# facebook/winterfell

Measured on NVIDIA H100. Metric: prover_ms, lower is better.
Workload: dtype u64

## Files before the change

### winterfell_b200/csrc/capi.cu

```cuda
#include <cuda_runtime.h>
#include <stdarg.h>
#include <stdio.h>

#include <algorithm>
#include <map>
#include <set>
#include <string>
#include <thread>
#include <utility>
#include <vector>

#include "internal.hpp"
#include "alg_hash.cuh"

void wf_mark(wf_ctx* ctx, const char* name) {
    if (!ctx->profiling) return;
    cudaEvent_t e;
    if (cudaEventCreate(&e) != cudaSuccess) return;
    cudaEventRecord(e, ctx->st);
    ctx->marks.push_back({name, e});
}
int wf_fail(wf_ctx* ctx, int code, const char* fmt, ...) {
    char buf[512];
    va_list ap;
    va_start(ap, fmt);
    vsnprintf(buf, sizeof(buf), fmt, ap);
    va_end(ap);
    if (ctx) ctx->err = buf;
    return code;
}
static inline void wf_use_device(wf_ctx* ctx) {
    int cur = -1;
    if (cudaGetDevice(&cur) != cudaSuccess || cur != ctx->device) cudaSetDevice(ctx->device);
}
int wf_dev_alloc(wf_ctx* ctx, size_t bytes, void** out) {
    wf_use_device(ctx);
    bytes = (bytes + 255) & ~(size_t)255;
    if (bytes == 0) bytes = 256;
    auto it = ctx->pool.find(bytes);
    if (it != ctx->pool.end()) {
        *out = it->second;
        ctx->pool.erase(it);
        ctx->live[*out] = bytes;
        return WF_OK;
    }
    void* p = nullptr;
    cudaError_t e = cudaMalloc(&p, bytes);
    if (e != cudaSuccess) {
        for (auto& kv : ctx->pool) cudaFree(kv.second);
        ctx->pool.clear();
        e = cudaMalloc(&p, bytes);
        if (e != cudaSuccess) return wf_fail(ctx, WF_ERR_CUDA, "cudaMalloc(%zu): %s", bytes, cudaGetErrorString(e));
    }
    ctx->live[p] = bytes;
    *out = p;
    return WF_OK;
}
void wf_dev_free(wf_ctx* ctx, void* p) {
    if (!p) return;
    auto it = ctx->live.find(p);
    if (it == ctx->live.end()) return;
    ctx->pool.insert({it->second, p});
    ctx->live.erase(it);
}
int wf_mat_alloc(wf_ctx* ctx, size_t rows, u32 cols, wf_mat** out) { return wf_mat_alloc_w(ctx, rows, cols, seg_width_for(cols), out); }
int wf_mat_alloc_w(wf_ctx* ctx, size_t rows, u32 cols, int W, wf_mat** out) {
    wf_mat* m = new wf_mat();
    m->m.rows = rows;
    m->m.cols = cols;
    m->m.W = W;
    m->m.seg_stride = rows * m->m.W;
    void* p;
    int r = wf_dev_alloc(ctx, m->m.words() * 8, &p);
    if (r != WF_OK) { delete m; return r; }
    m->m.base = (u64*)p;
    *out = m;
    return WF_OK;
}

__global__ void pow_table_kernel(u64* out, u64 base, u64 scale, size_t count) {
    size_t i = (size_t)blockIdx.x * blockDim.x + threadIdx.x;
    if (i < count) out[i] = gl_mul(scale, gl_pow(base, i));
}
__global__ void pow_table2_kernel(u64* out, const u64* bases, size_t count, size_t nbases) {
    size_t i = (size_t)blockIdx.x * blockDim.x + threadIdx.x;
    if (i < count * nbases) out[i] = gl_pow(bases[i / count], i % count);
}

int wf_get_twiddles(wf_ctx* ctx, u32 log_n, const u64** out) {
    auto it = ctx->tw.find(log_n);
    if (it != ctx->tw.end()) { *out = it->second; return WF_OK; }
    if (log_n < 1 || log_n > 32) return wf_fail(ctx, WF_ERR_INVALID, "no 2^%u-th root of unity", log_n);
    size_t half = log_n >= 1 ? ((size_t)1 << (log_n - 1)) : 1;
    void* p;
    cudaError_t e = cudaMalloc(&p, std::max(half * 8, (size_t)16));
    if (e != cudaSuccess) return wf_fail(ctx, WF_ERR_CUDA, "cudaMalloc twiddles: %s", cudaGetErrorString(e));
    pow_table_kernel<<<(unsigned)((half + 255) / 256), 256, 0, ctx->st>>>((u64*)p, gl_root_of_unity(log_n), 1, half);
    ctx->launches++;
    CK(cudaGetLastError());
    ctx->tw[log_n] = (u64*)p;
    *out = (u64*)p;
    return WF_OK;
}

static int get_pow_table(wf_ctx* ctx, u32 log_order, u32 log_count, const u64** out) {
    auto key = std::make_pair(log_order, log_count);
    auto it = ctx->pow_tab.find(key);
    if (it != ctx->pow_tab.end()) { *out = it->second; return WF_OK; }
    size_t cnt = (size_t)1 << log_count;
    void* p;
    cudaError_t e = cudaMalloc(&p, std::max(cnt * 8, (size_t)16));
    if (e != cudaSuccess) return wf_fail(ctx, WF_ERR_CUDA, "cudaMalloc power table: %s", cudaGetErrorString(e));
    pow_table_kernel<<<(unsigned)((cnt + 255) / 256), 256, 0, ctx->st>>>((u64*)p, log_order ? gl_root_of_unity(log_order) : 1, 1, cnt);
    ctx->launches++;
    CK(cudaGetLastError());
    ctx->pow_tab[key] = (u64*)p;
    *out = (u64*)p;
    return WF_OK;
}
static int get_round_tw(wf_ctx* ctx, u32 logS, const u64** out) {
    auto it = ctx->round_tw.find(logS);
    if (it != ctx->round_tw.end()) { *out = it->second; return WF_OK; }
    void* p;
    cudaError_t e = cudaMalloc(&p, ntt2_tw_entries((int)logS) * 8);
    if (e != cudaSuccess) return wf_fail(ctx, WF_ERR_CUDA, "cudaMalloc round twiddles: %s", cudaGetErrorString(e));
    CK(ntt2_build_tw((int)logS, (u64*)p, ctx->st));
    ctx->launches++;
    ctx->round_tw[logS] = (u64*)p;
    *out = (u64*)p;
    return WF_OK;
}
static int launch_pass(wf_ctx* ctx, int mode, NttPassParams& p, u32 n_segments, u32 n_batch) {
    wf_use_device(ctx);
    if (p.logS >= NTT2_MIN_LOGS) {
        CKI(get_round_tw(ctx, (u32)p.logS, &p.sub_tw));
        if (p.has_post) {
            p.tw_split = p.logM / 2;
            CKI(get_pow_table(ctx, p.logM, p.tw_split, &p.tw_lo));
            CKI(get_pow_table(ctx, p.logM - p.tw_split, p.logM - p.tw_split, &p.tw_hi));
        }
        p.vec_in = (p.W >= 2 || mode == NTT_STRIDED) ? 1 : 0;
        p.vec_out = (p.W >= 2 || (mode == NTT_STRIDED && !p.y_in_out)) ? 1 : 0;
        CK(ntt2_launch_pass(mode, p, n_segments, n_batch, ctx->st));
    } else {
        CKI(wf_get_twiddles(ctx, std::max((u32)p.logS, 1u), &p.sub_tw));
        if (p.has_post) CKI(wf_get_twiddles(ctx, p.logM, &p.master));
        CK(ntt_launch_pass(mode, p, n_segments, n_batch, ctx->st));
    }
    ctx->launches++;
    return WF_OK;
}

static void split_log(u32 log_n, u32* logR, u32* logC) {
    if (log_n <= NTT_MAX_LOGS) { *logR = 0; *logC = log_n; return; }
    u32 r = (log_n + 1) / 2;
    if (r > NTT_MAX_LOGS) r = NTT_MAX_LOGS;
    *logR = r;
    *logC = log_n - r;
}

static int get_lde_tables(wf_ctx* ctx, u32 log_n, u32 log_b, u32 logR, LdeTables* out) {
    auto key = std::make_pair(log_n | (logR << 8), log_b);
    auto it = ctx->lde_tabs.find(key);
    if (it != ctx->lde_tabs.end()) { *out = it->second; return WF_OK; }
    const u32 logC = log_n - logR;
    size_t b = (size_t)1 << log_b, R = (size_t)1 << logR, C = (size_t)1 << logC;
    u64 g = gl_root_of_unity(log_n + log_b);
    std::vector<u64> bases(b);
    size_t cnt = logR == 0 ? C : R;
    for (size_t k = 0; k < b; k++) {
        u64 sk = gl_mul(GL_GENERATOR, gl_pow(g, k));
        bases[k] = logR == 0 ? sk : gl_pow(sk, C);
    }
    LdeTables t{nullptr, nullptr};
    void *p, *pb;
    CK(cudaMalloc(&p, b * cnt * 8));
    CK(cudaMalloc(&pb, b * 8));
    CK(cudaMemcpyAsync(pb, bases.data(), b * 8, cudaMemcpyHostToDevice, ctx->st));
    pow_table2_kernel<<<(unsigned)((b * cnt + 255) / 256), 256, 0, ctx->st>>>((u64*)p, (u64*)pb, cnt, b);
    ctx->launches++;
    CK(cudaGetLastError());
    CK(cudaStreamSynchronize(ctx->st));
    cudaFree(pb);
    t.pre = (u64*)p;
    if (logR != 0) {
        void* q;
        CK(cudaMalloc(&q, C * 8));
        pow_table_kernel<<<(unsigned)((C + 255) / 256), 256, 0, ctx->st>>>((u64*)q, GL_GENERATOR, 1, C);
        ctx->launches++;
        CK(cudaGetLastError());
        t.pow7 = (u64*)q;
    }
    ctx->lde_tabs[key] = t;
    *out = t;
    return WF_OK;
}

static void pass_defaults(NttPassParams& p, const SegMatrix& in, const SegMatrix& out) {
    memset(&p, 0, sizeof(p));
    p.in = in.base;
    p.out = out.base;
    p.in_seg_stride = in.seg_stride;
    p.out_seg_stride = out.seg_stride;
    p.W = in.W;
    p.out_W = (u32)out.W;
    p.out_row_mul = 1;
    p.cconst = 1;
}
static int split3(wf_ctx* ctx, u32 log_n, u32* lr, u32* lc, u32* lr2, u32* lc2) {
    *lr = (log_n + 2) / 3;
    *lc = log_n - *lr;
    split_log(*lc, lr2, lc2);
    if (*lr2 == 0 || *lc2 > NTT_MAX_LOGS || *lr > NTT_MAX_LOGS)
        return wf_fail(ctx, WF_ERR_UNSUPPORTED, "transform of 2^%u points exceeds the three-pass limit", log_n);
    return WF_OK;
}

static int run_ntt(wf_ctx* ctx, const SegMatrix& in, SegMatrix& out, const SegMatrix* tmp, u32 log_n, int inverse) {
    u32 logR, logC;
    split_log(log_n, &logR, &logC);
    u64 inv_n = gl_inv(((u64)1 << log_n) % GL_P);
    NttPassParams p;
    if (logC > NTT_MAX_LOGS) {
        if (!tmp) return wf_fail(ctx, WF_ERR_STATE, "run_ntt: scratch matrix required");
        u32 lr, lc, lr2, lc2;
        CKI(split3(ctx, log_n, &lr, &lc, &lr2, &lc2));
        pass_defaults(p, in, *tmp);
        p.logS = (int)lr; p.logR = lr; p.logC = lc; p.inverse = inverse;
        p.has_post = 1; p.logM = log_n; p.a_mul = 1; p.b_mul = 0; p.cconst = inverse ? inv_n : 1;
        CKI(launch_pass(ctx, NTT_STRIDED, p, in.nseg(), 1));
        pass_defaults(p, *tmp, *tmp);
        p.in_batch_stride = p.out_batch_stride = ((size_t)1 << lc) * in.W;
        p.logS = (int)lr2; p.logR = lr2; p.logC = lc2; p.inverse = inverse;
        p.has_post = 1; p.logM = lc; p.a_mul = 1; p.b_mul = 0;
        CKI(launch_pass(ctx, NTT_STRIDED, p, in.nseg(), 1u << lr));
        pass_defaults(p, *tmp, out);
        p.in_batch_stride = ((size_t)1 << lc) * in.W;
        p.logS = (int)lc2; p.logR = lr2; p.logC = lc2; p.inverse = inverse;
        p.out_row_mul = 1u << lr; p.out_row_add = 1;
        CKI(launch_pass(ctx, NTT_CONTIG, p, in.nseg(), 1u << lr));
        return WF_OK;
    }
    if (logR == 0) {
        pass_defaults(p, in, out);
        p.logS = (int)logC; p.logR = 0; p.logC = logC; p.inverse = inverse;
        if (inverse) p.cconst = inv_n;
        return launch_pass(ctx, NTT_CONTIG, p, in.nseg(), 1);
    }
    if (!tmp) return wf_fail(ctx, WF_ERR_STATE, "run_ntt: scratch matrix required");
    pass_defaults(p, in, *tmp);
    p.logS = (int)logR; p.logR = logR; p.logC = logC; p.inverse = inverse;
    p.has_post = 1; p.logM = log_n; p.a_mul = 1; p.b_mul = 0; p.cconst = inverse ? inv_n : 1;
    CKI(launch_pass(ctx, NTT_STRIDED, p, in.nseg(), 1));
    pass_defaults(p, *tmp, out);
    p.logS = (int)logC; p.logR = logR; p.logC = logC; p.inverse = inverse;
    return launch_pass(ctx, NTT_CONTIG, p, in.nseg(), 1);
}

static int run_lde(wf_ctx* ctx, const SegMatrix& polys, SegMatrix& out, u32 log_n, u32 log_b, u32 out_col0 = 0, u32 k0 = 0, u32 k1 = 0,
                   u32 row_mul = 0, u32 row_add = 1) {
    u32 logR, logC;
    split_log(log_n, &logR, &logC);
    u32 b = 1u << log_b;
    if (k1 == 0) k1 = b;
    if (row_mul == 0) { row_mul = b; row_add = 1; }
    LdeTables tabs;
    NttPassParams p;
    if (logC > NTT_MAX_LOGS) {
        u32 lr, lc, lr2, lc2;
        CKI(split3(ctx, log_n, &lr, &lc, &lr2, &lc2));
        CKI(get_lde_tables(ctx, log_n, log_b, lr, &tabs));
        SegMatrix y = polys;
        void* yp;
        CKI(wf_dev_alloc(ctx, polys.words() * 8, &yp));
        y.base = (u64*)yp;
        int rc = WF_OK;
        for (u32 k = k0; k < k1 && rc == WF_OK; k++) {
            pass_defaults(p, polys, y);
            p.logS = (int)lr; p.logR = lr; p.logC = lc;
            p.pre_tab = tabs.pre + ((size_t)k << lr); p.pre_batch_stride = 0;
            p.has_post = 1; p.logM = log_n + log_b; p.a_mul = b; p.b_mul = 1; p.batch0 = k;
            p.ctab = tabs.pow7;
            rc = launch_pass(ctx, NTT_STRIDED, p, polys.nseg(), 1);
            if (rc != WF_OK) break;
            pass_defaults(p, y, y);
            p.in_batch_stride = p.out_batch_stride = ((size_t)1 << lc) * polys.W;
            p.logS = (int)lr2; p.logR = lr2; p.logC = lc2;
            p.has_post = 1; p.logM = lc; p.a_mul = 1; p.b_mul = 0;
            rc = launch_pass(ctx, NTT_STRIDED, p, polys.nseg(), 1u << lr);
            if (rc != WF_OK) break;
            pass_defaults(p, y, out);
            p.in_batch_stride = ((size_t)1 << lc) * polys.W;
            p.logS = (int)lc2; p.logR = lr2; p.logC = lc2;
            p.out_row_mul = row_mul << lr; p.out_row_add = row_mul; p.out_col0 = out_col0;
            p.out = out.base + (size_t)(k - k0) * row_add * out.W;
            rc = launch_pass(ctx, NTT_CONTIG, p, polys.nseg(), 1u << lr);
        }
        wf_dev_free(ctx, yp);
        return rc;
    }
    CKI(get_lde_tables(ctx, log_n, log_b, logR, &tabs));
    if (logR == 0) {
        pass_defaults(p, polys, out);
        p.logS = (int)logC; p.logR = 0; p.logC = logC;
        p.pre_tab = tabs.pre + ((size_t)k0 << log_n); p.pre_batch_stride = (size_t)1 << log_n;
        p.out_row_mul = row_mul; p.out_row_add = row_add; p.out_col0 = out_col0;
        return launch_pass(ctx, NTT_CONTIG, p, polys.nseg(), k1 - k0);
    }
    pass_defaults(p, polys, out);
    p.logS = (int)logR; p.logR = logR; p.logC = logC;
    p.pre_tab = tabs.pre + ((size_t)k0 << logR); p.pre_batch_stride = (size_t)1 << logR;
    p.has_post = 1; p.logM = log_n + log_b; p.a_mul = b; p.b_mul = 1; p.batch0 = k0;
    p.ctab = tabs.pow7;
    p.y_in_out = 1; p.out_row_mul = row_mul; p.out_row_add = row_add; p.out_col0 = out_col0;
    CKI(launch_pass(ctx, NTT_STRIDED, p, polys.nseg(), k1 - k0));
    pass_defaults(p, polys, out);
    p.in = out.base;
    p.in_seg_stride = out.seg_stride;
    p.logS = (int)logC; p.logR = logR; p.logC = logC;
    p.y_in_out = 1; p.out_row_mul = row_mul; p.out_row_add = row_add; p.out_col0 = out_col0;
    return launch_pass(ctx, NTT_CONTIG, p, polys.nseg(), k1 - k0);
}

template <int K>
__device__ __forceinline__ void field_shift_store(u64 a, u64* out, size_t n, size_t i, int slot) { out[(4 + slot) * n + i] = gl_mul_2exp<K>(a); }
__global__ void field_ops_kernel(const u64* a, const u64* b, size_t n, u64* out) {
    size_t i = (size_t)blockIdx.x * blockDim.x + threadIdx.x;
    if (i >= n) return;
    u64 x = a[i], y = b[i];
    out[i] = gl_mul(x, y);
    out[n + i] = gl_add(x, y);
    out[2 * n + i] = gl_sub(x, y);
    out[3 * n + i] = x ? gl_inv(x) : 0;
    u64 s = x, d = y;
    gl_butterfly(s, d);
    if (s != out[n + i] || d != out[2 * n + i]) out[n + i] = ~0ULL;
    field_shift_store<1>(x, out, n, i, 0);   field_shift_store<3>(x, out, n, i, 1);   field_shift_store<6>(x, out, n, i, 2);
    field_shift_store<12>(x, out, n, i, 3);  field_shift_store<24>(x, out, n, i, 4);  field_shift_store<31>(x, out, n, i, 5);
    field_shift_store<32>(x, out, n, i, 6);  field_shift_store<33>(x, out, n, i, 7);  field_shift_store<48>(x, out, n, i, 8);
    field_shift_store<63>(x, out, n, i, 9);  field_shift_store<64>(x, out, n, i, 10); field_shift_store<65>(x, out, n, i, 11);
    field_shift_store<72>(x, out, n, i, 12); field_shift_store<80>(x, out, n, i, 13); field_shift_store<84>(x, out, n, i, 14);
    field_shift_store<90>(x, out, n, i, 15); field_shift_store<95>(x, out, n, i, 16); field_shift_store<96>(x, out, n, i, 17);
}
template <int... K>
__device__ __forceinline__ void field_shifts_all(u64 x, u64* out, size_t n, size_t i, std::integer_sequence<int, K...>) {
    ((out[(size_t)K * n + i] = gl_mul_2exp<K>(x)), ...);
}
__global__ void field_shifts_kernel(const u64* a, size_t n, u64* out) {
    size_t i = (size_t)blockIdx.x * blockDim.x + threadIdx.x;
    if (i >= n) return;
    field_shifts_all(a[i], out, n, i, std::make_integer_sequence<int, 97>{});
}

__global__ void rescue_weak_kernel(const u64* a, const u64* b, size_t n, u64* out) {
    size_t i = (size_t)blockIdx.x * blockDim.x + threadIdx.x;
    if (i >= n) return;
    out[i] = gl_mul_weak(a[i], b[i]);
    out[n + i] = gl_sqr_weak(a[i]);
    out[2 * n + i] = rp64_exp7(a[i]);
}
template <int G>
__global__ void rescue_inv7_kernel(const u64* a, size_t n, u64* out) {
    size_t t = (size_t)blockIdx.x * blockDim.x + threadIdx.x;
    if (t >= n / G) return;
    u64 s[G];
#pragma unroll
    for (int e = 0; e < G; e++) s[e] = a[t * G + e];
    rp64_inv7_group<G>(s);
#pragma unroll
    for (int e = 0; e < G; e++) out[t * G + e] = s[e];
}
__global__ void rescue_mds_kernel(const u64* a, size_t n, u64* out12, u64* out8) {
    size_t t = (size_t)blockIdx.x * blockDim.x + threadIdx.x;
    if (t < n / 12) {
        u64 s[12];
        for (int e = 0; e < 12; e++) s[e] = a[t * 12 + e];
        rp64_mds(s);
        for (int e = 0; e < 12; e++) out12[t * 12 + e] = s[e];
    }
    if (t < n / 8) {
        u64 s[8];
        for (int e = 0; e < 8; e++) s[e] = a[t * 8 + e];
        rpj_mds(s);
        for (int e = 0; e < 8; e++) out8[t * 8 + e] = s[e];
    }
}
template <int HASH, int W>
__global__ void rescue_permute_kernel(const u64* in, const u64* values, size_t n, u64* out) {
    size_t i = (size_t)blockIdx.x * blockDim.x + threadIdx.x;
    if (i >= n) return;
    u64 s[W];
#pragma unroll
    for (int e = 0; e < W; e++) s[e] = in[i * W + e];
    u64 m[4], mi[4];
    alg_merge<HASH>(s, m);
    alg_merge_with_int<HASH>(s, values[i], mi);
    if (HASH == WF_HASH_RP64_256) rp64_permute(s);
    else rpj_permute(s);
#pragma unroll
    for (int e = 0; e < W; e++) out[i * W + e] = s[e];
#pragma unroll
    for (int e = 0; e < 4; e++) { out[n * W + i * 4 + e] = m[e]; out[n * (W + 4) + i * 4 + e] = mi[e]; }
}

template <int D>
__global__ void ext_ops_kernel(const u64* a, const u64* b, size_t n, u64* out) {
    size_t i = (size_t)blockIdx.x * blockDim.x + threadIdx.x;
    if (i >= n) return;
    GlExt<D> x, y;
#pragma unroll
    for (int q = 0; q < D; q++) { x.v[q] = a[i * D + q]; y.v[q] = b[i * D + q]; }
    const GlExt<D> r[6] = {ext_mul(x, y), ext_inv(x), ext_frobenius(x), ext_mul_base(x, y.v[0]), ext_add(x, y), ext_sub(x, y)};
#pragma unroll
    for (int k = 0; k < 6; k++)
#pragma unroll
        for (int q = 0; q < D; q++) out[((size_t)k * n + i) * D + q] = r[k].v[q];
}

__global__ void acc_ops_kernel(const u64* x, const u64* y, u32 k, size_t n, u64* out) {
    size_t i = (size_t)blockIdx.x * blockDim.x + threadIdx.x;
    if (i >= n) return;
    GlAcc a = acc_zero();
    for (u32 j = 0; j < k; j++) acc_mad(a, x[i * k + j], y[i * k + j]);
    u64* o = out + i * 6;
    o[0] = a.w0; o[1] = a.w1; o[2] = a.w2; o[3] = a.w3; o[4] = a.w4;
    o[5] = acc_reduce(a);
}

template <int K>
static u64 m2e(u64 x) { return gl_mul_2exp<K>(x); }

extern "C" {

const char* wf_version(void) { return "winterfell_b200 0.1 (sm_90a)"; }

int wf_ctx_create(wf_ctx** out, int device, void* stream) {
    if (!out) return WF_ERR_INVALID;
    *out = nullptr;
    int n = 0;
    cudaError_t e = cudaGetDeviceCount(&n);
    if (e != cudaSuccess || n == 0) return WF_ERR_CUDA;
    if (device < 0 || device >= n) return WF_ERR_INVALID;
    if (cudaSetDevice(device) != cudaSuccess) return WF_ERR_CUDA;
    wf_ctx* ctx = new wf_ctx();
    ctx->device = device;
    ctx->st = (cudaStream_t)stream;
    ctx->launches = 0;
    ctx->pinned = nullptr;
    ctx->pinned_bytes = 0;
    ctx->profiling = false;
    *out = ctx;
    return WF_OK;
}
void wf_ctx_destroy(wf_ctx* ctx) {
    if (!ctx) return;
    cudaSetDevice(ctx->device);
    cudaStreamSynchronize(ctx->st);
    for (auto& kv : ctx->pool) cudaFree(kv.second);
    for (auto& kv : ctx->live) cudaFree(kv.first);
    for (auto& kv : ctx->tw) cudaFree(kv.second);
    for (auto& kv : ctx->lde_tabs) { cudaFree(kv.second.pre); if (kv.second.pow7) cudaFree(kv.second.pow7); }
    if (ctx->pinned) cudaFreeHost(ctx->pinned);
    for (auto& kv : ctx->ipc_opened) cudaIpcCloseMemHandle(kv.second);
    for (auto& kv : ctx->jit_cache) if (kv.second.first) cudaLibraryUnload((cudaLibrary_t)kv.second.first);
    for (int i = 0; i < 4; i++) if (ctx->push_st[i]) { cudaStreamSynchronize(ctx->push_st[i]); cudaStreamDestroy(ctx->push_st[i]); }
    for (int i = 0; i < 16; i++) if (ctx->push_ev[i]) cudaEventDestroy(ctx->push_ev[i]);
    if (ctx->copy_st) {
        cudaStreamSynchronize(ctx->copy_st);
        for (int i = 0; i < 2; i++) { cudaEventDestroy(ctx->ev_up[i]); cudaEventDestroy(ctx->ev_used[i]); }
        cudaEventDestroy(ctx->ev_start);
        cudaStreamDestroy(ctx->copy_st);
    }
    delete ctx;
}
int wf_ctx_set_profiling(wf_ctx* ctx, int on) {
    if (!ctx) return WF_ERR_INVALID;
    ctx->profiling = on != 0;
    for (auto& m : ctx->marks) cudaEventDestroy(m.second);
    ctx->marks.clear();
    return WF_OK;
}
int wf_ctx_stage_times(wf_ctx* ctx, char* names, size_t names_cap, float* ms, size_t* count) {
    if (!ctx || !names || !ms || !count) return WF_ERR_INVALID;
    CK(cudaStreamSynchronize(ctx->st));
    size_t n = ctx->marks.size() > 0 ? ctx->marks.size() - 1 : 0, used = 0;
    if (n > *count) n = *count;
    names[0] = 0;
    for (size_t i = 0; i < n; i++) {
        CK(cudaEventElapsedTime(&ms[i], ctx->marks[i].second, ctx->marks[i + 1].second));
        const std::string& nm = ctx->marks[i + 1].first;
        if (used + nm.size() + 2 < names_cap) { memcpy(names + used, nm.c_str(), nm.size()); used += nm.size(); names[used++] = ','; names[used] = 0; }
    }
    *count = n;
    for (auto& m : ctx->marks) cudaEventDestroy(m.second);
    ctx->marks.clear();
    return WF_OK;
}
const char* wf_last_error(const wf_ctx* ctx) { return ctx ? ctx->err.c_str() : "no context (is a CUDA device present?)"; }
int wf_ctx_sync(wf_ctx* ctx) { wf_use_device(ctx); CK(cudaStreamSynchronize(ctx->st)); return WF_OK; }
uint64_t wf_ctx_launch_count(const wf_ctx* ctx) { return ctx->launches; }
int wf_ctx_mem_stats(const wf_ctx* ctx, uint64_t* live_buffers, uint64_t* live_bytes, uint64_t* pooled_bytes) {
    if (!ctx) return WF_ERR_INVALID;
    uint64_t lb = 0, pb = 0;
    for (auto& kv : ctx->live) lb += kv.second;
    for (auto& kv : ctx->pool) pb += kv.first;
    if (live_buffers) *live_buffers = ctx->live.size();
    if (live_bytes) *live_bytes = lb;
    if (pooled_bytes) *pooled_bytes = pb;
    return WF_OK;
}
// ... 261 lines not shown
            ctx->launches++;
            SegMatrix pv = polys->m;
            pv.base = polys->m.base + (size_t)k * polys->m.seg_stride;
            pv.cols = cw;
            SegMatrix tv = trv;
            tv.base = (u64*)tmp;
            CKI(run_ntt(ctx, trv, pv, &tv, log_n, 1));
            SegMatrix ov = lde->m;
            ov.base = lde->m.base + (size_t)(c0 / Wout) * lde->m.seg_stride;
            ov.cols = cw;
            CKI(extend(pv, ov, c0 % Wout, k + 1 == nchunks));
        }
        return WF_OK;
    };
    int rc = body();
    if (rc != WF_OK) {
        cudaStreamSynchronize(ctx->copy_st);
        release(true);
        return rc;
    }
    release(false);
    *polys_out = polys;
    *lde_out = lde;
    return WF_OK;
}

int wf_mat_interpolate_with_offset(wf_ctx* ctx, const wf_mat* evals, uint64_t domain_offset, wf_mat** polys) {
    if (domain_offset == 0 || domain_offset >= GL_P) return wf_fail(ctx, WF_ERR_INVALID, "bad domain offset");
    wf_mat* p;
    CKI(mat_transform(ctx, evals, 1, &p));
    CK(layout_scale_rows_by_powers(p->m, gl_inv(domain_offset), ctx->st));
    ctx->launches++;
    *polys = p;
    return WF_OK;
}

static int tree_alloc(wf_ctx* ctx, int hash_id, size_t nleaves, wf_tree** out) {
    if (nleaves < 2 || (nleaves & (nleaves - 1))) return wf_fail(ctx, WF_ERR_INVALID, "number of leaves must be a power of two >= 2");
    wf_tree* t = new wf_tree();
    t->hash_id = hash_id;
    t->nleaves = nleaves;
    void *a, *b;
    int r = wf_dev_alloc(ctx, nleaves * 32, &a);
    if (r != WF_OK) { delete t; return r; }
    r = wf_dev_alloc(ctx, nleaves * 32, &b);
    if (r != WF_OK) { wf_dev_free(ctx, a); delete t; return r; }
    t->leaves = (u64*)a;
    t->nodes = (u64*)b;
    *out = t;
    return WF_OK;
}
static u32 merkle_launches(size_t nleaves) {
    u32 l = 0;
    size_t m = nleaves / 2;
    while (m > (1u << 13)) { l++; m >>= 1; }
    for (;;) {
        l++;
        if (m <= 256) break;
        m = (m >> 8) >> 1;
        if (m == 0) break;
    }
    return l;
}
int wf_commit_rows_partitioned(wf_ctx* ctx, int hash_id, const wf_mat* m, uint32_t partition_size, wf_tree** out) {
    if (!ctx || !m || !out) return wf_fail(ctx, WF_ERR_INVALID, "bad arguments");
    if (!WF_HASH_IS_KNOWN(hash_id)) return wf_fail(ctx, WF_ERR_UNSUPPORTED, "unknown hash %d", hash_id);
    if (partition_size != 0 && partition_size != m->m.cols && (m->m.cols + partition_size - 1) / partition_size > 16)
        return wf_fail(ctx, WF_ERR_INVALID, "more than 16 partitions");
    wf_tree* t;
    CKI(tree_alloc(ctx, hash_id, m->m.rows, &t));
    CK(commit_hash_rows(hash_id, m->m, t->leaves, ctx->st, partition_size));
    CK(commit_merkle_nodes(hash_id, t->leaves, t->nleaves, t->nodes, ctx->st));
    ctx->launches += 1 + merkle_launches(t->nleaves);
    *out = t;
    return WF_OK;
}
int wf_commit_rows(wf_ctx* ctx, int hash_id, const wf_mat* m, wf_tree** out) {
    if (!ctx || !m || !out) return wf_fail(ctx, WF_ERR_INVALID, "bad arguments");
    if (!WF_HASH_IS_KNOWN(hash_id)) return wf_fail(ctx, WF_ERR_UNSUPPORTED, "unknown hash %d", hash_id);
    wf_tree* t;
    CKI(tree_alloc(ctx, hash_id, m->m.rows, &t));
    CK(commit_hash_rows(hash_id, m->m, t->leaves, ctx->st));
    CK(commit_merkle_nodes(hash_id, t->leaves, t->nleaves, t->nodes, ctx->st));
    ctx->launches += 1 + merkle_launches(t->nleaves);
    *out = t;
    return WF_OK;
}
int wf_tree_from_leaves(wf_ctx* ctx, int hash_id, const uint8_t* leaves, size_t nleaves, int on_device, wf_tree** out) {
    if (!ctx || !leaves || !out) return wf_fail(ctx, WF_ERR_INVALID, "bad arguments");
    wf_tree* t;
    CKI(tree_alloc(ctx, hash_id, nleaves, &t));
    CK(cudaMemcpyAsync(t->leaves, leaves, nleaves * 32, on_device ? cudaMemcpyDeviceToDevice : cudaMemcpyHostToDevice, ctx->st));
    CK(commit_merkle_nodes(hash_id, t->leaves, nleaves, t->nodes, ctx->st));
    ctx->launches += merkle_launches(nleaves);
    if (!on_device) CK(cudaStreamSynchronize(ctx->st));
    *out = t;
    return WF_OK;
}
int wf_tree_free(wf_ctx* ctx, wf_tree* t) {
    if (!t) return WF_OK;
    wf_dev_free(ctx, t->leaves);
    wf_dev_free(ctx, t->nodes);
    delete t;
    return WF_OK;
}
size_t wf_tree_num_leaves(const wf_tree* t) { return t->nleaves; }
int wf_tree_root(wf_ctx* ctx, const wf_tree* t, uint8_t root[32]) {
    if (!ctx || !t || !root) return wf_fail(ctx, WF_ERR_INVALID, "bad arguments");
    CK(cudaMemcpyAsync(root, t->nodes + 4, 32, cudaMemcpyDeviceToHost, ctx->st));
    CK(cudaStreamSynchronize(ctx->st));
    return WF_OK;
}
int wf_tree_to_host(wf_ctx* ctx, const wf_tree* t, uint8_t* leaves, uint8_t* nodes) {
    if (!ctx || !t) return wf_fail(ctx, WF_ERR_INVALID, "bad arguments");
    if (leaves) CK(cudaMemcpyAsync(leaves, t->leaves, t->nleaves * 32, cudaMemcpyDeviceToHost, ctx->st));
    if (nodes) CK(cudaMemcpyAsync(nodes, t->nodes, t->nleaves * 32, cudaMemcpyDeviceToHost, ctx->st));
    CK(cudaStreamSynchronize(ctx->st));
    return WF_OK;
}

}

int wf_open_plan(wf_ctx* ctx, size_t n, const uint64_t* positions, size_t k, OpenPlan& pl) {
    pl.depth = log2_ceil(n);
    if (k == 0) return wf_fail(ctx, WF_ERR_INVALID, "no positions");
    std::map<size_t, size_t> index_map;
    for (size_t i = 0; i < k; i++) {
        if (positions[i] >= n) return wf_fail(ctx, WF_ERR_INVALID, "leaf index out of bounds");
        index_map[positions[i]] = i;
    }
    if (index_map.size() != k) return wf_fail(ctx, WF_ERR_INVALID, "duplicate leaf index");
    std::set<size_t> norm;
    for (size_t i = 0; i < k; i++) norm.insert(positions[i] & ~(size_t)1);
    pl.want.clear();
    pl.vec_slots.clear();
    pl.leaf_slot.assign(k, 0);
    std::vector<size_t> next;
    for (size_t index : norm) {
        std::vector<size_t> slots;
        for (size_t i = index; i < index + 2; i++) {
            auto it = index_map.find(i);
            pl.want.push_back(n + i);
            if (it != index_map.end()) pl.leaf_slot[it->second] = pl.want.size() - 1;
            else slots.push_back(pl.want.size() - 1);
        }
        pl.vec_slots.push_back(slots);
        next.push_back((index + n) >> 1);
    }
    for (u32 lvl = 1; lvl < pl.depth; lvl++) {
        std::vector<size_t> idx = next;
        next.clear();
        size_t i = 0;
        while (i < idx.size()) {
            size_t sib = idx[i] ^ 1;
            if (i + 1 < idx.size() && idx[i + 1] == sib) i += 1;
            else { pl.want.push_back(sib); pl.vec_slots[i].push_back(pl.want.size() - 1); }
            next.push_back(sib >> 1);
            i += 1;
        }
    }
    return WF_OK;
}
void wf_open_finish(const OpenPlan& pl, const uint8_t* got, uint8_t* leaves_out, ByteVec& proof) {
    if (leaves_out)
        for (size_t i = 0; i < pl.leaf_slot.size(); i++) memcpy(leaves_out + i * 32, got + pl.leaf_slot[i] * 32, 32);
    proof.u8_((u8)pl.depth);
    proof.usize(pl.vec_slots.size());
    for (auto& v : pl.vec_slots) {
        proof.usize(v.size());
        for (size_t s : v) proof.bytes(got + s * 32, pl.digest_bytes);
    }
}

int pinned_reserve(wf_ctx* ctx, size_t bytes) {
    if (ctx->pinned_bytes >= bytes) return WF_OK;
    if (ctx->pinned) cudaFreeHost(ctx->pinned);
    ctx->pinned = nullptr;
    ctx->pinned_bytes = 0;
    bytes = std::max(bytes * 2, (size_t)1 << 20);
    CK(cudaMallocHost(&ctx->pinned, bytes));
    ctx->pinned_bytes = bytes;
    return WF_OK;
}

size_t GatherBatch::add_rows(const SegMatrix& m, const std::vector<u64>& pos) {
    rows.push_back({m, pos, 0, 0});
    return rows.size() - 1;
}
int GatherBatch::add_opening(wf_ctx* ctx, const wf_tree* t, const std::vector<u64>& pos, size_t* id) {
    digs.emplace_back();
    digs.back().t = t;
    CKI(wf_open_plan(ctx, t->nleaves, pos.data(), pos.size(), digs.back().plan));
    digs.back().plan.digest_bytes = WF_DIGEST_BYTES(t->hash_id);
    digs.back().idx = digs.back().plan.want;
    *id = digs.size() - 1;
    return WF_OK;
}
int GatherBatch::add_opening_sharded(wf_ctx* ctx, const wf_tree* t, size_t n_global, int world, int rank, const std::vector<u64>& pos,
                                     size_t* id, std::vector<std::pair<size_t, u64>>* top_slots) {
    digs.emplace_back();
    DigJob& j = digs.back();
    j.t = t;
    CKI(wf_open_plan(ctx, n_global, pos.data(), pos.size(), j.plan));
    if (t) j.plan.digest_bytes = WF_DIGEST_BYTES(t->hash_id);
    const size_t n_local = n_global / (size_t)world;
    const u32 log_w = log2_ceil((size_t)world);
    j.idx.assign(j.plan.want.size(), ~(u64)0);
    for (size_t s = 0; s < j.plan.want.size(); s++) {
        const u64 e = j.plan.want[s];
        if (e >= n_global) {
            const u64 leaf = e - n_global;
            if ((int)(leaf / n_local) == rank) j.idx[s] = n_local + leaf % n_local;
        } else if (e < (u64)world) {
            if (top_slots) top_slots->push_back({s, e});
        } else {
            u32 depth = 63 - (u32)__builtin_clzll(e);
            const u32 rel = depth - log_w;
            const u64 owner = (e >> rel) - (u64)world;
            if ((int)owner == rank) j.idx[s] = ((u64)1 << rel) | (e & (((u64)1 << rel) - 1));
        }
    }
    *id = digs.size() - 1;
    return WF_OK;
}
int GatherBatch::run(wf_ctx* ctx) {
    wf_use_device(ctx);
    size_t idx_words = 0, out_words = 0;
    for (auto& j : rows) { j.idx_off = idx_words; j.out_off = out_words; idx_words += j.pos.size(); out_words += j.pos.size() * j.m.cols; }
    for (auto& j : digs) { j.idx_off = idx_words; j.out_off = out_words; idx_words += j.plan.want.size(); out_words += j.plan.want.size() * 4; }
    if (idx_words == 0) return WF_OK;
    CKI(pinned_reserve(ctx, (idx_words + out_words) * 8));
    u64* h_idx = (u64*)ctx->pinned;
    u64* h_out = h_idx + idx_words;
    for (auto& j : rows) memcpy(h_idx + j.idx_off, j.pos.data(), j.pos.size() * 8);
    for (auto& j : digs) memcpy(h_idx + j.idx_off, j.idx.data(), j.idx.size() * 8);
    void *d_idx, *d_out;
    CKI(wf_dev_alloc(ctx, idx_words * 8, &d_idx));
    CKI(wf_dev_alloc(ctx, out_words * 8, &d_out));
    CK(cudaMemcpyAsync(d_idx, h_idx, idx_words * 8, cudaMemcpyHostToDevice, ctx->st));
    for (auto& j : rows) {
        CK(layout_gather_rows(j.m, (const u64*)d_idx + j.idx_off, j.pos.size(), (u64*)d_out + j.out_off, 0, ctx->st));
        ctx->launches++;
    }
    for (auto& j : digs) {
        CK(layout_gather_digests(j.t->nodes, j.t->leaves, j.t->nleaves, (const u64*)d_idx + j.idx_off, j.plan.want.size(),
                                 (u64*)d_out + j.out_off, ctx->st));
        ctx->launches++;
    }
    if (comm && comm->world > 1 && comm->all_reduce_sum(comm->user, d_out, out_words) != 0)
        return wf_fail(ctx, WF_ERR_STATE, "all_reduce_sum callback failed");
    CK(cudaMemcpyAsync(h_out, d_out, out_words * 8, cudaMemcpyDeviceToHost, ctx->st));
    CK(cudaStreamSynchronize(ctx->st));
    wf_dev_free(ctx, d_idx);
    wf_dev_free(ctx, d_out);
    result = h_out;
    return WF_OK;
}

int wf_tree_open_many_bytes(wf_ctx* ctx, const wf_tree* t, const uint64_t* positions, size_t k, uint8_t* leaves_out,
                            ByteVec& proof) {
    GatherBatch gb;
    size_t id;
    CKI(gb.add_opening(ctx, t, std::vector<u64>(positions, positions + k), &id));
    CKI(gb.run(ctx));
    wf_open_finish(gb.digs[id].plan, gb.digest_result(id), leaves_out, proof);
    return WF_OK;
}
extern "C" {
int wf_tree_open_many(wf_ctx* ctx, const wf_tree* t, const uint64_t* positions, size_t k, uint8_t* leaves_out,
                      uint8_t* proof, size_t* proof_len) {
    if (!ctx || !t || !positions || !leaves_out || !proof || !proof_len) return wf_fail(ctx, WF_ERR_INVALID, "bad arguments");
    ByteVec bv;
    CKI(wf_tree_open_many_bytes(ctx, t, positions, k, leaves_out, bv));
    if (bv.v.size() > *proof_len) return wf_fail(ctx, WF_ERR_INVALID, "proof buffer too small (%zu needed)", bv.v.size());
    memcpy(proof, bv.v.data(), bv.v.size());
    *proof_len = bv.v.size();
    return WF_OK;
}

}
int wf_fri_layer_tree(wf_ctx* ctx, int hash_id, const u64* vals, size_t len, int d, int ld, int nf, wf_tree** out) {
    const size_t m = len / (size_t)nf;
    wf_tree* t;
    CKI(tree_alloc(ctx, hash_id, m, &t));
    CK(fri_hash_layer(hash_id, vals, len, d, ld, nf, t->leaves, ctx->st));
    CK(commit_merkle_nodes(hash_id, t->leaves, m, t->nodes, ctx->st));
    ctx->launches += 1 + merkle_launches(m);
    *out = t;
    return WF_OK;
}
extern "C" {
int wf_fri_free(wf_ctx* ctx, wf_fri* f) {
    if (!f) return WF_OK;
    for (auto& l : f->layers) { wf_dev_free(ctx, l.evals); wf_tree_free(ctx, l.tree); }
    delete f;
    return WF_OK;
}

}
struct FriBuild {
    wf_ctx* ctx;
    wf_fri* f;
    wf_tree* t = nullptr;
    DevScratch tmp;
    FriBuild(wf_ctx* c, wf_fri* fr) : ctx(c), f(fr), tmp(c) {}
    ~FriBuild() { if (t) wf_tree_free(ctx, t); if (f) wf_fri_free(ctx, f); }
};
extern "C" {
int wf_fri_build_layers(wf_ctx* ctx, int hash_id, const wf_mat* evals, int d, uint32_t folding, uint32_t rem_max_deg,
                        uint32_t blowup, wf_fri_commit_fn commit, wf_fri_draw_fn draw_alpha, void* user, wf_fri** out) {
    if (!ctx || !evals || !commit || !draw_alpha || !out) return wf_fail(ctx, WF_ERR_INVALID, "bad arguments");
    if (d < 1 || d > 3 || (int)evals->m.cols != d) return wf_fail(ctx, WF_ERR_INVALID, "evaluations must have ext_degree base columns");
    if (folding != 2 && folding != 4 && folding != 8 && folding != 16) return wf_fail(ctx, WF_ERR_UNSUPPORTED, "folding factor %u", folding);
    size_t len = evals->m.rows;
    u32 logL;
    if (log2_exact(len, &logL)) return wf_fail(ctx, WF_ERR_INVALID, "domain size must be a power of two");
    wf_fri* f = new wf_fri();
    FriBuild g(ctx, f);
    f->hash_id = hash_id; f->d = d; f->folding = folding; f->blowup = blowup;
    f->ld = evals->m.W;
    const int ld = f->ld;
    void* cur;
    CKI(g.tmp.alloc(len * ld * 8, &cur));
    CK(cudaMemcpyAsync(cur, evals->m.base, len * ld * 8, cudaMemcpyDeviceToDevice, ctx->st));
    size_t max_rem = (size_t)(rem_max_deg + 1) * blowup;
    while (len > max_rem) {
        size_t m = len / folding;
        wf_tree* t;
        CKI(tree_alloc(ctx, hash_id, m, &t));
        g.t = t;
        CK(fri_hash_layer(hash_id, (u64*)cur, len, d, ld, (int)folding, t->leaves, ctx->st));
        CK(commit_merkle_nodes(hash_id, t->leaves, m, t->nodes, ctx->st));
        ctx->launches += 1 + merkle_launches(m);
        uint8_t root[32];
        CK(cudaMemcpyAsync(root, t->nodes + 4, 32, cudaMemcpyDeviceToHost, ctx->st));
        CK(cudaStreamSynchronize(ctx->st));
        commit(user, root);
        u64 alpha[3] = {0, 0, 0};
        draw_alpha(user, alpha);
        const u64* master;
        CKI(wf_get_twiddles(ctx, log2_ceil(len), &master));
        void* nxt;
        CKI(g.tmp.alloc(m * ld * 8, &nxt));
        if (ld > d) CK(cudaMemsetAsync(nxt, 0, m * ld * 8, ctx->st));
        CK(fri_fold_layer((u64*)cur, len, d, ld, (int)folding, alpha, master, (u64*)nxt, ld, ctx->st));
        ctx->launches++;
        f->layers.push_back(FriLayer{(u64*)g.tmp.keep(cur), len, t});
        g.t = nullptr;
        cur = nxt;
        len = m;
    }
    std::vector<u64> raw(len * ld), v(len * d);
    CK(cudaMemcpyAsync(raw.data(), cur, len * ld * 8, cudaMemcpyDeviceToHost, ctx->st));
    CK(cudaStreamSynchronize(ctx->st));
    g.tmp.free(cur);
    for (size_t i = 0; i < len; i++)
        for (int c = 0; c < d; c++) v[i * d + c] = raw[i * ld + c];
    wf_host_dft(v, len, d, true, GL_GENERATOR);
    size_t rsize = len / blowup;
    f->remainder.resize(rsize * d);
    for (size_t i = 0; i < rsize; i++)
        for (int c = 0; c < d; c++) f->remainder[i * d + c] = v[(rsize - 1 - i) * d + c];
    Digest rc = hh_hash_elements(hash_id, f->remainder.data(), f->remainder.size());
    commit(user, rc.b);
    g.f = nullptr;
    *out = f;
    return WF_OK;
}

}
int wf_fri_build_layers_coin(wf_ctx* ctx, int hash_id, const wf_mat* evals, int d, uint32_t folding, uint32_t rem_max_deg,
                             uint32_t blowup, PublicCoin& coin, std::vector<Digest>& commitments, wf_fri** out) {
    if (!ctx || !evals || !out) return wf_fail(ctx, WF_ERR_INVALID, "bad arguments");
    if (d < 1 || d > 3 || (int)evals->m.cols != d) return wf_fail(ctx, WF_ERR_INVALID, "evaluations must have ext_degree base columns");
    if (folding != 2 && folding != 4 && folding != 8 && folding != 16) return wf_fail(ctx, WF_ERR_UNSUPPORTED, "folding factor %u", folding);
    size_t len = evals->m.rows;
    u32 logL;
    if (log2_exact(len, &logL)) return wf_fail(ctx, WF_ERR_INVALID, "domain size must be a power of two");
    wf_fri* f = new wf_fri();
    FriBuild g(ctx, f);
    f->hash_id = hash_id; f->d = d; f->folding = folding; f->blowup = blowup;
    f->ld = evals->m.W;
    const int ld = f->ld;
    const size_t max_rem = (size_t)(rem_max_deg + 1) * blowup;
    size_t nlayers = 0;
    for (size_t l = len; l > max_rem; l /= folding) nlayers++;
    void *cur, *dstate, *dalpha, *dlog;
    CKI(g.tmp.alloc(len * ld * 8, &cur));
    CK(cudaMemcpyAsync(cur, evals->m.base, len * ld * 8, cudaMemcpyDeviceToDevice, ctx->st));
    CKI(g.tmp.alloc(8 * 8, &dstate));
    CKI(g.tmp.alloc(8 * 8, &dalpha));
    CKI(g.tmp.alloc(std::max<size_t>(nlayers, 1) * 8 * 8, &dlog));
    u64 seed_words[4];
    memcpy(seed_words, coin.seed.b, 32);
    CK(cudaMemcpyAsync(dstate, seed_words, 32, cudaMemcpyHostToDevice, ctx->st));
    size_t layer = 0;
    while (len > max_rem) {
        size_t m = len / folding;
        wf_tree* t;
        CKI(tree_alloc(ctx, hash_id, m, &t));
        g.t = t;
        CK(fri_hash_layer(hash_id, (u64*)cur, len, d, ld, (int)folding, t->leaves, ctx->st));
        CK(commit_merkle_nodes(hash_id, t->leaves, m, t->nodes, ctx->st));
        CK(fri_coin_step(hash_id, (u64*)dstate, t->nodes + 4, d, (u64*)dalpha, (u64*)dlog + 8 * layer, ctx->st));
        ctx->launches += 2 + merkle_launches(m);
        const u64* master;
        CKI(wf_get_twiddles(ctx, log2_ceil(len), &master));
        void* nxt;
        CKI(g.tmp.alloc(m * ld * 8, &nxt));
        if (ld > d) CK(cudaMemsetAsync(nxt, 0, m * ld * 8, ctx->st));
        CK(fri_fold_layer((u64*)cur, len, d, ld, (int)folding, nullptr, master, (u64*)nxt, ld, ctx->st, (const u64*)dalpha));
        ctx->launches++;
        f->layers.push_back(FriLayer{(u64*)g.tmp.keep(cur), len, t});
        g.t = nullptr;
        cur = nxt;
        len = m;
        layer++;
    }
    std::vector<u64> raw(len * ld), v(len * d), log(std::max<size_t>(nlayers, 1) * 8);
    CK(cudaMemcpyAsync(raw.data(), cur, len * ld * 8, cudaMemcpyDeviceToHost, ctx->st));
    if (nlayers) CK(cudaMemcpyAsync(log.data(), dlog, nlayers * 8 * 8, cudaMemcpyDeviceToHost, ctx->st));
    CK(cudaStreamSynchronize(ctx->st));
    g.tmp.free(cur);
    g.tmp.free(dstate); g.tmp.free(dalpha); g.tmp.free(dlog);
    for (size_t l = 0; l < nlayers; l++) {
        Digest root;
        memcpy(root.b, &log[8 * l], 32);
        commitments.push_back(root);
        coin.reseed(root);
        u64 alpha[3] = {0, 0, 0};
        bool ok = coin.draw(d, alpha) && log[8 * l + 7] == 1;
        for (int k = 0; k < d; k++) ok = ok && alpha[k] == log[8 * l + 4 + k];
        if (!ok) return wf_fail(ctx, WF_ERR_STATE, "device and host FRI transcripts diverged at layer %zu", l);
    }
    for (size_t i = 0; i < len; i++)
        for (int c = 0; c < d; c++) v[i * d + c] = raw[i * ld + c];
    wf_host_dft(v, len, d, true, GL_GENERATOR);
    size_t rsize = len / blowup;
    f->remainder.resize(rsize * d);
    for (size_t i = 0; i < rsize; i++)
        for (int c = 0; c < d; c++) f->remainder[i * d + c] = v[(rsize - 1 - i) * d + c];
    Digest rc = hh_hash_elements(hash_id, f->remainder.data(), f->remainder.size());
    commitments.push_back(rc);
    coin.reseed(rc);
    g.f = nullptr;
    *out = f;
    return WF_OK;
}
extern "C" {

struct DefaultChannel {
    PublicCoin coin;
    int d;
    std::vector<Digest> commitments;
};
int wf_fri_build_layers_default_channel(wf_ctx* ctx, int hash_id, const wf_mat* evals, int d, uint32_t folding,
                                        uint32_t rem_max_deg, uint32_t blowup, uint8_t* roots_out, size_t roots_cap,
                                        wf_fri** out) {
    DefaultChannel ch{PublicCoin(hash_id, nullptr, 0), d, {}};
    CKI(wf_fri_build_layers_coin(ctx, hash_id, evals, d, folding, rem_max_deg, blowup, ch.coin, ch.commitments, out));
    if (roots_out) {
        if (roots_cap < ch.commitments.size() * 32) return wf_fail(ctx, WF_ERR_INVALID, "roots buffer too small");
        for (size_t i = 0; i < ch.commitments.size(); i++) memcpy(roots_out + 32 * i, ch.commitments[i].b, 32);
    }
    return WF_OK;
}
uint32_t wf_fri_num_layers(const wf_fri* f) { return (uint32_t)f->layers.size(); }
size_t wf_fri_remainder(const wf_fri* f, uint64_t* coeffs, size_t cap_words) {
    if (coeffs && cap_words >= f->remainder.size()) memcpy(coeffs, f->remainder.data(), f->remainder.size() * 8);
    return f->remainder.size() / f->d;
}

}
int wf_fri_queue_proof(wf_ctx* ctx, wf_fri* f, const std::vector<u64>& positions, GatherBatch& gb, FriProofPlan& plan) {
    std::vector<u64> pos = positions;
    for (auto& L : f->layers) {
        size_t m = L.len / f->folding;
        pos = fold_positions(pos, m);
        std::vector<u64> gpos(pos.size() * f->folding);
        for (size_t i = 0; i < pos.size(); i++)
            for (u32 j = 0; j < f->folding; j++) gpos[i * f->folding + j] = pos[i] + (u64)j * m;
        SegMatrix lm;
        lm.base = L.evals; lm.rows = L.len; lm.cols = (u32)f->d; lm.W = f->ld; lm.seg_stride = L.len * f->ld;
        plan.row_ids.push_back(gb.add_rows(lm, gpos));
        size_t id;
        CKI(gb.add_opening(ctx, L.tree, pos, &id));
        plan.dig_ids.push_back(id);
        plan.nq.push_back(pos.size());
    }
    return WF_OK;
}
void wf_fri_finish_proof(const wf_fri* f, const GatherBatch& gb, const FriProofPlan& plan, ByteVec& bv, const FriProofPlan* before) {
    auto layer = [&](const FriProofPlan& p, size_t l) {
        const size_t nvals = p.nq[l] * f->folding * f->d;
        ByteVec paths;
        wf_open_finish(gb.digs[p.dig_ids[l]].plan, gb.digest_result(p.dig_ids[l]), nullptr, paths);
        bv.u32_((u32)(nvals * 8));
        bv.bytes(gb.row_result(p.row_ids[l]), nvals * 8);
        bv.u32_((u32)paths.v.size());
        bv.bytes(paths.v.data(), paths.v.size());
    };
    const size_t nb = before ? before->nq.size() : 0;
    bv.u8_((u8)(nb + f->layers.size()));
    for (size_t l = 0; l < nb; l++) layer(*before, l);
    for (size_t l = 0; l < f->layers.size(); l++) layer(plan, l);
    bv.u16_((uint16_t)(f->remainder.size() * 8));
    bv.bytes(f->remainder.data(), f->remainder.size() * 8);
    bv.u8_(0);
}
extern "C" {
int wf_fri_build_proof(wf_ctx* ctx, wf_fri* f, const uint64_t* positions, size_t k, uint8_t* out, size_t* len) {
    if (!ctx || !f || !positions || !out || !len) return wf_fail(ctx, WF_ERR_INVALID, "bad arguments");
    GatherBatch gb;
    FriProofPlan plan;
    CKI(wf_fri_queue_proof(ctx, f, std::vector<u64>(positions, positions + k), gb, plan));
    CKI(gb.run(ctx));
    ByteVec bv;
    wf_fri_finish_proof(f, gb, plan, bv);
    if (bv.v.size() > *len) return wf_fail(ctx, WF_ERR_INVALID, "proof buffer too small (%zu needed)", bv.v.size());
    memcpy(out, bv.v.data(), bv.v.size());
    *len = bv.v.size();
    return WF_OK;
}

int wf_ntt_dev(wf_ctx* ctx, uint64_t* d_data, uint32_t log_n, uint32_t cols, int inverse) {
    if (!ctx || !d_data || cols == 0 || log_n < 1) return wf_fail(ctx, WF_ERR_INVALID, "bad arguments");
    wf_mat *m, *o;
    CKI(wf_mat_from_device_columns(ctx, d_data, cols, (size_t)1 << log_n, &m));
    int r = mat_transform(ctx, m, inverse, &o);
    wf_mat_free(ctx, m);
    if (r != WF_OK) return r;
    r = wf_mat_to_columns(ctx, o, d_data, 0, 0);
    wf_mat_free(ctx, o);
    return r;
}
int wf_hash_rows_dev(wf_ctx* ctx, int hash_id, const uint64_t* d_rows, size_t nrows, uint32_t cols, uint8_t* d_digests) {
    if (!ctx || !d_rows || !d_digests || cols == 0) return wf_fail(ctx, WF_ERR_INVALID, "bad arguments");
    wf_mat* m;
    CKI(wf_mat_alloc(ctx, nrows, cols, &m));
    CK(layout_rows_to_seg(d_rows, m->m, ctx->st));
    CK(commit_hash_rows(hash_id, m->m, (u64*)d_digests, ctx->st));
    ctx->launches += 2;
    wf_mat_free(ctx, m);
    return WF_OK;
}
int wf_merkle_dev(wf_ctx* ctx, int hash_id, const uint8_t* d_leaves, size_t nleaves, uint8_t* d_nodes) {
    if (!ctx || !d_leaves || !d_nodes) return wf_fail(ctx, WF_ERR_INVALID, "bad arguments");
    if (nleaves < 2 || (nleaves & (nleaves - 1))) return wf_fail(ctx, WF_ERR_INVALID, "number of leaves must be a power of two >= 2");
    CK(commit_merkle_nodes(hash_id, (const u64*)d_leaves, nleaves, (u64*)d_nodes, ctx->st));
    ctx->launches += merkle_launches(nleaves);
    return WF_OK;
}
int wf_field_ops_dev(wf_ctx* ctx, const uint64_t* d_a, const uint64_t* d_b, size_t n, uint64_t* d_out) {
    if (!ctx || !d_a || !d_b || !d_out || n == 0) return wf_fail(ctx, WF_ERR_INVALID, "bad arguments");
    field_ops_kernel<<<(unsigned)((n + 127) / 128), 128, 0, ctx->st>>>(d_a, d_b, n, d_out);
    ctx->launches++;
    CK(cudaGetLastError());
    return WF_OK;
}
int wf_field_shifts_dev(wf_ctx* ctx, const uint64_t* d_a, size_t n, uint64_t* d_out) {
    if (!ctx || !d_a || !d_out || n == 0) return wf_fail(ctx, WF_ERR_INVALID, "bad arguments");
    field_shifts_kernel<<<(unsigned)((n + 127) / 128), 128, 0, ctx->st>>>(d_a, n, d_out);
    ctx->launches++;
    CK(cudaGetLastError());
    return WF_OK;
}
int wf_rescue_ops_dev(wf_ctx* ctx, const uint64_t* d_a, const uint64_t* d_b, size_t n, uint64_t* d_out) {
    if (!ctx || !d_a || !d_b || !d_out || n == 0 || n % 24) return wf_fail(ctx, WF_ERR_INVALID, "bad arguments");
    const unsigned blocks = (unsigned)((n + 127) / 128);
    rescue_weak_kernel<<<blocks, 128, 0, ctx->st>>>(d_a, d_b, n, d_out);
    rescue_inv7_kernel<1><<<blocks, 128, 0, ctx->st>>>(d_a, n, d_out + 3 * n);
    rescue_inv7_kernel<2><<<blocks, 128, 0, ctx->st>>>(d_a, n, d_out + 4 * n);
    rescue_inv7_kernel<3><<<blocks, 128, 0, ctx->st>>>(d_a, n, d_out + 5 * n);
    rescue_inv7_kernel<4><<<blocks, 128, 0, ctx->st>>>(d_a, n, d_out + 6 * n);
    rescue_inv7_kernel<6><<<blocks, 128, 0, ctx->st>>>(d_a, n, d_out + 7 * n);
    rescue_mds_kernel<<<blocks, 128, 0, ctx->st>>>(d_a, n, d_out + 8 * n, d_out + 9 * n);
    ctx->launches += 7;
    CK(cudaGetLastError());
    return WF_OK;
}
int wf_rescue_permute_dev(wf_ctx* ctx, int hash_id, const uint64_t* d_states, const uint64_t* d_values, size_t n, uint64_t* d_out) {
    if (!ctx || !d_states || !d_values || !d_out || n == 0) return wf_fail(ctx, WF_ERR_INVALID, "bad arguments");
    const unsigned blocks = (unsigned)((n + 127) / 128);
    if (hash_id == WF_HASH_RP64_256) rescue_permute_kernel<WF_HASH_RP64_256, 12><<<blocks, 128, 0, ctx->st>>>(d_states, d_values, n, d_out);
    else if (hash_id == WF_HASH_RPJIVE64_256) rescue_permute_kernel<WF_HASH_RPJIVE64_256, 8><<<blocks, 128, 0, ctx->st>>>(d_states, d_values, n, d_out);
    else return wf_fail(ctx, WF_ERR_INVALID, "hash %d has no Rescue permutation", hash_id);
    ctx->launches++;
    CK(cudaGetLastError());
    return WF_OK;
}
int wf_ext_ops_dev(wf_ctx* ctx, uint32_t ext, const uint64_t* d_a, const uint64_t* d_b, size_t n, uint64_t* d_out) {
    if (!ctx || !d_a || !d_b || !d_out || n == 0 || (ext != 2 && ext != 3)) return wf_fail(ctx, WF_ERR_INVALID, "bad arguments");
    const unsigned blocks = (unsigned)((n + 127) / 128);
    if (ext == 2) ext_ops_kernel<2><<<blocks, 128, 0, ctx->st>>>(d_a, d_b, n, d_out);
    else ext_ops_kernel<3><<<blocks, 128, 0, ctx->st>>>(d_a, d_b, n, d_out);
    ctx->launches++;
    CK(cudaGetLastError());
    return WF_OK;
}
int wf_acc_ops_dev(wf_ctx* ctx, const uint64_t* d_x, const uint64_t* d_y, uint32_t k, size_t n, uint64_t* d_out) {
    if (!ctx || !d_x || !d_y || !d_out || n == 0 || k == 0 || k >= (1u << 31)) return wf_fail(ctx, WF_ERR_INVALID, "bad arguments");
    acc_ops_kernel<<<(unsigned)((n + 127) / 128), 128, 0, ctx->st>>>(d_x, d_y, k, n, d_out);
    ctx->launches++;
    CK(cudaGetLastError());
    return WF_OK;
}
int wf_fri_fold_dev(wf_ctx* ctx, const uint64_t* d_evals, size_t len, int d, uint32_t folding, const uint64_t* alpha,
                    uint64_t* d_next) {
    if (!ctx || !d_evals || !alpha || !d_next || d < 1 || d > 3) return wf_fail(ctx, WF_ERR_INVALID, "bad arguments");
    u32 ll;
    if (log2_exact(len, &ll) || len < folding) return wf_fail(ctx, WF_ERR_INVALID, "bad length");
    const u64* master;
    CKI(wf_get_twiddles(ctx, std::max(ll, 1u), &master));
    CK(fri_fold_layer(d_evals, len, d, d, (int)folding, alpha, master, d_next, d, ctx->st));
    ctx->launches++;
    return WF_OK;
}

int wf_host_hash_elements(int hash_id, const uint64_t* elems, size_t n, uint8_t out[32]) {
    Digest d = hh_hash_elements(hash_id, elems, n);
    memcpy(out, d.b, 32);
    return WF_OK;
}
int wf_host_merge(int hash_id, const uint8_t two[64], uint8_t out[32]) {
    Digest a, b;
    memcpy(a.b, two, 32);
    memcpy(b.b, two + 32, 32);
    Digest d = hh_merge(hash_id, a, b);
    memcpy(out, d.b, 32);
    return WF_OK;
}
int wf_host_merge_with_int(int hash_id, const uint8_t seed[32], uint64_t value, uint8_t out[32]) {
    Digest s;
    memcpy(s.b, seed, 32);
    Digest d = hh_merge_with_int(hash_id, s, value);
    memcpy(out, d.b, 32);
    return WF_OK;
}
uint64_t wf_host_mul(uint64_t a, uint64_t b) { return gl_mul(a, b); }
uint64_t wf_host_mul_2exp(uint64_t x, uint32_t k) {
    switch (k) {
        case 0: return m2e<0>(x); case 3: return m2e<3>(x); case 6: return m2e<6>(x); case 12: return m2e<12>(x);
        case 24: return m2e<24>(x); case 36: return m2e<36>(x); case 48: return m2e<48>(x); case 60: return m2e<60>(x);
        case 63: return m2e<63>(x); case 64: return m2e<64>(x); case 65: return m2e<65>(x); case 72: return m2e<72>(x);
        case 84: return m2e<84>(x); case 95: return m2e<95>(x); case 96: return m2e<96>(x);
        default: return gl_mul(x, gl_pow(2, k));
    }
}
uint64_t wf_host_mont_to_canonical(uint64_t m) { return gl_from_mont(m); }
uint64_t wf_host_canonical_to_mont(uint64_t x) { return gl_to_mont(x); }
size_t wf_host_write_usize(uint64_t value, uint8_t out[9]) {
    ByteVec b;
    b.usize(value);
    memcpy(out, b.v.data(), b.v.size());
    return b.v.size();
}
int wf_host_build_fib_trace(uint32_t k, size_t n, uint64_t* cols, uint64_t* results) {
    if (!cols || !results || k == 0 || n == 0) return WF_ERR_INVALID;
    auto pair = [&](uint32_t j) {
        u64 a = j + 1, b = j + 1;
        u64 *ca = cols + (size_t)(2 * j) * n, *cb = ca + n;
        for (size_t i = 0; i < n; i++) {
            ca[i] = a;
            cb[i] = b;
            a = gl_add_host(a, b);
            b = gl_add_host(b, a);
        }
        results[j] = cb[n - 1];
    };
    const unsigned nt = std::max(1u, std::min(std::min(k, 16u), std::thread::hardware_concurrency()));
    std::vector<std::thread> th;
    for (unsigned t = 0; t < nt; t++) th.emplace_back([&, t]() { for (uint32_t j = t; j < k; j += nt) pair(j); });
    for (auto& x : th) x.join();
    return WF_OK;
}
long wf_host_sharded_opening_plan(size_t n_global, int world, int rank, const uint64_t* positions, size_t k, uint64_t* want,
                                  uint64_t* idx, size_t cap) {
    if (!positions || !want || !idx || world < 1 || (world & (world - 1)) || n_global % (size_t)world) return -1;
    GatherBatch gb;
    size_t id;
    std::vector<std::pair<size_t, u64>> top;
    if (gb.add_opening_sharded(nullptr, nullptr, n_global, world, rank, std::vector<u64>(positions, positions + k), &id, &top) != WF_OK) return -1;
    const auto& j = gb.digs[id];
    if (j.idx.size() > cap) return -1;
    for (size_t i = 0; i < j.idx.size(); i++) { want[i] = j.plan.want[i]; idx[i] = j.idx[i]; }
    for (auto& t : top) idx[t.first] = ~(u64)0 - 1;
    return (long)j.idx.size();
}
int wf_host_coin_draw(int hash_id, const uint64_t* seed_elems, size_t n_seed, const uint8_t* reseed32, int d, size_t count,
                      uint64_t* out) {
    if (d < 1 || d > 3 || !out) return -1;
    PublicCoin coin(hash_id, seed_elems, n_seed);
    if (reseed32) { Digest dg; memcpy(dg.b, reseed32, 32); coin.reseed(dg); }
    for (size_t i = 0; i < count; i++) if (!coin.draw(d, out + i * d)) return -1;
    return 0;
}

}
```

### winterfell_b200/csrc/fri.cu

```cuda
#include "fri.cuh"
#include "internal.hpp"

#include "blake3.cuh"
#include "commit.cuh"
#include "minidft.cuh"
#include "alg_hash.cuh"

__global__ void __launch_bounds__(256) fri_hash_blake3_kernel(const u64* __restrict__ ev, size_t m, int d, int ld, int nf,
                                                              uint4* __restrict__ digests, u32 dw) {
    size_t i = (size_t)blockIdx.x * blockDim.x + threadIdx.x;
    if (i >= m) return;
    const u32 ne = (u32)(nf * d);
    const u32 nblk = (ne + 7) / 8;
    u32 cv[8];
    b3_iv(cv);
    for (u32 b = 0; b < nblk; b++) {
        u32 msg[16];
#pragma unroll
        for (int k = 0; k < 8; k++) {
            u32 e = b * 8 + k;
            u64 v = 0;
            if (e < ne) {
                u32 kk = e / d, comp = e % d;
                v = ev[(i + (size_t)kk * m) * ld + comp];
            }
            msg[2 * k] = (u32)v;
            msg[2 * k + 1] = (u32)(v >> 32);
        }
        u32 bl = min(64u, (ne - b * 8) * 8);
        u32 fl = (b == 0 ? B3_CHUNK_START : 0) | (b == nblk - 1 ? (B3_CHUNK_END | B3_ROOT) : 0);
        b3_compress(cv, msg, 0, bl, fl, b3_runtime_one());
    }
    if (dw == 6) { cv[6] = 0; cv[7] = 0; }
    digests[2 * i] = make_uint4(cv[0], cv[1], cv[2], cv[3]);
    digests[2 * i + 1] = make_uint4(cv[4], cv[5], cv[6], cv[7]);
}

template <int HASH>
__global__ void __launch_bounds__(128) fri_hash_alg_kernel(const u64* __restrict__ ev, size_t m, int d, int ld, int nf,
                                                           u64* __restrict__ digests) {
    size_t i = (size_t)blockIdx.x * blockDim.x + threadIdx.x;
    if (i >= m) return;
    const u32 ne = (u32)(nf * d);
    AlgSponge<HASH> sp;
    sp.init(ne);
    for (u32 e = 0; e < ne; e++) {
        u32 kk = e / d, comp = e % d;
        sp.absorb(ev[(i + (size_t)kk * m) * ld + comp]);
    }
    u64 o[4];
    sp.finish(o);
#pragma unroll
    for (int k = 0; k < 4; k++) digests[i * 4 + k] = o[k];
}

__host__ __device__ constexpr u32 cbrev(u32 v, int bits) {
    u32 r = 0;
    for (int i = 0; i < bits; i++) r |= ((v >> i) & 1u) << (bits - 1 - i);
    return r;
}

template <int D, int LOGNF>
__global__ void __launch_bounds__(256) fri_fold_kernel(const u64* __restrict__ ev, size_t m, int ld, GlExt<D> alpha,
                                                       const u64* __restrict__ d_alpha, const u64* __restrict__ master,
                                                       u32 logL, u64* __restrict__ next, int next_ld, size_t i0) {
    constexpr int NF = 1 << LOGNF;
    size_t i = (size_t)blockIdx.x * blockDim.x + threadIdx.x;
    if (i >= m) return;
    if (d_alpha) {
#pragma unroll
        for (int c = 0; c < D; c++) alpha.v[c] = d_alpha[c];
    }
    u64 x[D][NF];
#pragma unroll
    for (int k = 0; k < NF; k++)
#pragma unroll
        for (int c = 0; c < D; c++) x[c][k] = ev[(i + (size_t)k * m) * ld + c];
#pragma unroll
    for (int c = 0; c < D; c++) mini_dft<LOGNF>(x[c]);
    const u32 L = 1u << logL;
    u32 e = (L - (u32)(i + i0)) & (L - 1);
    u64 winv = (e & (L >> 1)) ? gl_neg(master[e & ((L >> 1) - 1)]) : master[e & ((L >> 1) - 1)];
    u64 xinv = gl_mul(winv, 2635249152773512046ULL);
    GlExt<D> beta = ext_mul_base(alpha, xinv);
    GlExt<D> acc;
    {
        constexpr u32 pos = cbrev(1u, LOGNF);
#pragma unroll
        for (int c = 0; c < D; c++) acc.v[c] = x[c][pos];
    }
#pragma unroll
    for (int j = NF - 2; j >= 0; j--) {
        const u32 pos = cbrev((u32)((NF - j) % NF), LOGNF);
        GlExt<D> cj;
#pragma unroll
        for (int c = 0; c < D; c++) cj.v[c] = x[c][pos];
        acc = ext_add(ext_mul(acc, beta), cj);
    }
    const u64 inv_nf = GL_P - ((GL_P - 1) >> LOGNF);
    acc = ext_mul_base(acc, inv_nf);
#pragma unroll
    for (int c = 0; c < D; c++) next[i * next_ld + c] = acc.v[c];
}

cudaError_t fri_hash_layer(int hash_id, const u64* evals, size_t len, int d, int ld, int nf, u64* digests,
                           cudaStream_t st) {
    size_t m = len / nf;
    if (WF_HASH_IS_BLAKE3(hash_id))
        fri_hash_blake3_kernel<<<(unsigned)((m + 255) / 256), 256, 0, st>>>(evals, m, d, ld, nf,
                                                                            reinterpret_cast<uint4*>(digests), WF_DIGEST_WORDS32(hash_id));
    else if (hash_id == WF_HASH_RP64_256)
        fri_hash_alg_kernel<WF_HASH_RP64_256><<<(unsigned)((m + 127) / 128), 128, 0, st>>>(evals, m, d, ld, nf, digests);
    else if (hash_id == WF_HASH_SHA3_256)
        fri_hash_alg_kernel<WF_HASH_SHA3_256><<<(unsigned)((m + 127) / 128), 128, 0, st>>>(evals, m, d, ld, nf, digests);
    else
        fri_hash_alg_kernel<WF_HASH_RPJIVE64_256><<<(unsigned)((m + 127) / 128), 128, 0, st>>>(evals, m, d, ld, nf, digests);
    return cudaGetLastError();
}

template <int D>
static cudaError_t fold_dispatch(const u64* evals, size_t len, int ld, int nf, const u64* alpha, const u64* d_alpha,
                                 const u64* master, u64* next, int next_ld, cudaStream_t st, size_t i0, u32 logL_global) {
    size_t m = len / nf;
    const u32 logL = logL_global ? logL_global : log2_ceil(len);
    GlExt<D> a;
    for (int c = 0; c < D; c++) a.v[c] = alpha ? alpha[c] : 0;
    unsigned blocks = (unsigned)((m + 255) / 256);
    switch (nf) {
        case 2: fri_fold_kernel<D, 1><<<blocks, 256, 0, st>>>(evals, m, ld, a, d_alpha, master, logL, next, next_ld, i0); break;
        case 4: fri_fold_kernel<D, 2><<<blocks, 256, 0, st>>>(evals, m, ld, a, d_alpha, master, logL, next, next_ld, i0); break;
        case 8: fri_fold_kernel<D, 3><<<blocks, 256, 0, st>>>(evals, m, ld, a, d_alpha, master, logL, next, next_ld, i0); break;
        case 16: fri_fold_kernel<D, 4><<<blocks, 256, 0, st>>>(evals, m, ld, a, d_alpha, master, logL, next, next_ld, i0); break;
        default: return cudaErrorInvalidValue;
    }
    return cudaGetLastError();
}

cudaError_t fri_fold_layer(const u64* evals, size_t len, int d, int ld, int nf, const u64* alpha, const u64* master,
                           u64* next, int next_ld, cudaStream_t st, const u64* d_alpha, size_t i0, u32 logL_global) {
    switch (d) {
        case 1: return fold_dispatch<1>(evals, len, ld, nf, alpha, d_alpha, master, next, next_ld, st, i0, logL_global);
        case 2: return fold_dispatch<2>(evals, len, ld, nf, alpha, d_alpha, master, next, next_ld, st, i0, logL_global);
        case 3: return fold_dispatch<3>(evals, len, ld, nf, alpha, d_alpha, master, next, next_ld, st, i0, logL_global);
        default: return cudaErrorInvalidValue;
    }
}

template <int HASH>
__device__ __forceinline__ void coin_merge(const u64 a[4], const u64 b[4], u64 out[4]) {
    if (WF_HASH_IS_BLAKE3(HASH)) {
        u32 wa[8], wb[8], cv[8];
#pragma unroll
        for (int i = 0; i < 4; i++) { wa[2 * i] = (u32)a[i]; wa[2 * i + 1] = (u32)(a[i] >> 32); wb[2 * i] = (u32)b[i]; wb[2 * i + 1] = (u32)(b[i] >> 32); }
        b3_merge_words<WF_DIGEST_WORDS32(HASH)>(wa, wb, cv);
#pragma unroll
        for (int i = 0; i < 4; i++) out[i] = (u64)cv[2 * i] | ((u64)cv[2 * i + 1] << 32);
    } else {
        u64 in[8];
#pragma unroll
        for (int i = 0; i < 4; i++) { in[i] = a[i]; in[4 + i] = b[i]; }
        alg_merge<HASH>(in, out);
    }
}
template <int HASH>
__device__ __forceinline__ void coin_merge_with_int(const u64 seed[4], u64 value, u64 out[4]) {
    if (WF_HASH_IS_BLAKE3(HASH)) {
        u32 ws[8], cv[8];
#pragma unroll
        for (int i = 0; i < 4; i++) { ws[2 * i] = (u32)seed[i]; ws[2 * i + 1] = (u32)(seed[i] >> 32); }
        b3_merge_with_int_words<WF_DIGEST_WORDS32(HASH)>(ws, value, cv);
#pragma unroll
        for (int i = 0; i < 4; i++) out[i] = (u64)cv[2 * i] | ((u64)cv[2 * i + 1] << 32);
    } else {
        alg_merge_with_int<HASH>(seed, value, out);
    }
}
template <int HASH>
__global__ void fri_coin_kernel(u64* state, const u64* root, int d, u64* alpha_out, u64* log_entry) {
    if (threadIdx.x != 0 || blockIdx.x != 0) return;
    u64 seed[4], r[4], v[4];
    for (int i = 0; i < 4; i++) { seed[i] = state[i]; r[i] = root[i]; }
    coin_merge<HASH>(seed, r, seed);
    u64 counter = 0;
    bool ok = false;
    for (int t = 0; t < 1000 && !ok; t++) {
        counter += 1;
        coin_merge_with_int<HASH>(seed, counter, v);
        ok = true;
        for (int k = 0; k < d; k++) ok = ok && v[k] < GL_P;
    }
    for (int i = 0; i < 4; i++) { state[i] = seed[i]; log_entry[i] = r[i]; }
    state[4] = counter;
    for (int k = 0; k < 3; k++) { u64 a = (ok && k < d) ? v[k] : 0; alpha_out[k] = a; log_entry[4 + k] = a; }
    log_entry[7] = ok ? 1 : 0;
}
cudaError_t fri_coin_step(int hash_id, u64* state, const u64* root, int d, u64* alpha_out, u64* log_entry, cudaStream_t st) {
    if (hash_id == WF_HASH_BLAKE3_256) fri_coin_kernel<WF_HASH_BLAKE3_256><<<1, 32, 0, st>>>(state, root, d, alpha_out, log_entry);
    else if (hash_id == WF_HASH_BLAKE3_192) fri_coin_kernel<WF_HASH_BLAKE3_192><<<1, 32, 0, st>>>(state, root, d, alpha_out, log_entry);
    else if (hash_id == WF_HASH_RP64_256) fri_coin_kernel<WF_HASH_RP64_256><<<1, 32, 0, st>>>(state, root, d, alpha_out, log_entry);
    else if (hash_id == WF_HASH_SHA3_256) fri_coin_kernel<WF_HASH_SHA3_256><<<1, 32, 0, st>>>(state, root, d, alpha_out, log_entry);
    else fri_coin_kernel<WF_HASH_RPJIVE64_256><<<1, 32, 0, st>>>(state, root, d, alpha_out, log_entry);
    return cudaGetLastError();
}
```

### winterfell_b200/csrc/fri.cuh

```cuda
#pragma once
#include <cuda_runtime.h>

#include "gl64.cuh"

cudaError_t fri_hash_layer(int hash_id, const u64* evals, size_t len, int d, int ld, int nf, u64* digests,
                           cudaStream_t st);
cudaError_t fri_fold_layer(const u64* evals, size_t len, int d, int ld, int nf, const u64* alpha,
                           const u64* master, u64* next, int next_ld, cudaStream_t st, const u64* d_alpha = nullptr,
                           size_t i0 = 0, u32 logL_global = 0);
cudaError_t fri_coin_step(int hash_id, u64* state, const u64* root, int d, u64* alpha_out, u64* log_entry, cudaStream_t st);
```

### winterfell_b200/csrc/internal.hpp

```cpp
#pragma once
#include <cuda_runtime.h>

#include <algorithm>
#include <map>
#include <set>
#include <string>
#include <functional>
#include <vector>

#include "../../include/winterfell_b200.h"
#include "commit.cuh"
#include "fri.cuh"
#include "host_transcript.hpp"
#include "layout.cuh"
#include "ntt.cuh"

struct LdeTables {
    u64* pre;
    u64* pow7;
};

struct wf_ctx {
    int device;
    cudaStream_t st;
    std::string err;
    uint64_t launches;
    std::multimap<size_t, void*> pool;
    std::map<void*, size_t> live;
    std::map<u32, u64*> tw;
    std::map<u32, u64*> round_tw;
    std::map<std::pair<u32, u32>, u64*> pow_tab;
    std::map<std::pair<u32, u32>, LdeTables> lde_tabs;
    void* pinned;
    size_t pinned_bytes;
    cudaStream_t copy_st = nullptr;
    cudaEvent_t ev_up[2], ev_used[2], ev_start;
    std::map<std::string, void*> ipc_opened;
    cudaStream_t push_st[4] = {nullptr, nullptr, nullptr, nullptr};
    cudaEvent_t push_ev[16] = {};
    std::map<std::string, std::pair<void*, void*>> jit_cache;
    bool jit_enabled = true;
    bool validate = false;
    uint64_t jit_compiled = 0, jit_hits = 0, jit_fallbacks = 0;
    bool profiling;
    std::vector<std::pair<std::string, cudaEvent_t>> marks;
};
void wf_mark(wf_ctx* ctx, const char* name);

struct wf_mat {
    SegMatrix m;
};
struct wf_tree {
    int hash_id;
    size_t nleaves;
    u64* leaves;
    u64* nodes;
};

static inline u32 log2_ceil(size_t n) { return n <= 1 ? 0 : 64 - (u32)__builtin_clzll((unsigned long long)(n - 1)); }

static inline void wf_host_dft(std::vector<u64>& v, size_t n, int d, bool inverse, u64 offset) {
    const u32 log_n = log2_ceil(n);
    u64 w0 = n > 1 ? gl_root_of_unity(log_n) : 1;
    if (inverse) w0 = gl_inv(w0);
    if (!inverse && offset != 1) {
        u64 f = 1;
        for (size_t i = 0; i < n; i++) { for (int c = 0; c < d; c++) v[i * d + c] = gl_mul(v[i * d + c], f); f = gl_mul(f, offset); }
    }
    for (size_t i = 0; i < n; i++) {
        size_t j = 0;
        for (u32 b = 0; b < log_n; b++) j |= ((i >> b) & 1) << (log_n - 1 - b);
        if (j > i) for (int c = 0; c < d; c++) std::swap(v[i * d + c], v[j * d + c]);
    }
    for (size_t len = 2; len <= n; len <<= 1) {
        u64 wl = gl_pow(w0, n / len);
        for (size_t s = 0; s < n; s += len) {
            u64 w = 1;
            for (size_t i = 0; i < len / 2; i++) {
                for (int c = 0; c < d; c++) {
                    u64 a = v[(s + i) * d + c], b = gl_mul(v[(s + i + len / 2) * d + c], w);
                    v[(s + i) * d + c] = gl_add(a, b);
                    v[(s + i + len / 2) * d + c] = gl_sub(a, b);
                }
                w = gl_mul(w, wl);
            }
        }
    }
    if (inverse) {
        u64 scale = gl_inv((u64)n % GL_P), oinv = gl_inv(offset);
        for (size_t i = 0; i < n; i++) {
            for (int c = 0; c < d; c++) v[i * d + c] = gl_mul(v[i * d + c], scale);
            scale = gl_mul(scale, oinv);
        }
    }
}

int wf_fail(wf_ctx* ctx, int code, const char* fmt, ...);
int pinned_reserve(wf_ctx* ctx, size_t bytes);
std::string wf_jit_source(int D, u32 w, u32 nper, u32 nregs, const std::vector<u32>& prog, const std::vector<u64>& consts, u32 aw, u32 nr,
                          u32 naregs, const std::vector<u32>& aprog);
int wf_jit_compile(const std::string& src, std::vector<char>& cubin, std::string& log);
int wf_jit_get_kernel(wf_ctx* ctx, const std::string& src, cudaKernel_t* kernel);
int wf_dev_alloc(wf_ctx* ctx, size_t bytes, void** out);
void wf_dev_free(wf_ctx* ctx, void* p);
struct AuxBuildCol {
    u32 kind = 0;
    u64 init[3] = {0, 0, 0};
    u32 num_regs = 0;
    std::vector<u32> prog;
};
struct AuxBuildHost {
    u32 aw = 0;
    std::vector<u64> consts;
    std::vector<AuxBuildCol> cols;
};
const char* wf_aux_build_parse(const u64* d, size_t len, u32 w, u32 aw, u32 np, u32 nr, AuxBuildHost& out);
int wf_aux_build_run(wf_ctx* ctx, const AuxBuildHost& b, const wf_mat* main, u32 w, const std::vector<std::vector<u64>>& periodic,
                     const u64* rnd, u32 nr, int D, wf_mat** out);
struct DevScratch {
    wf_ctx* ctx;
    std::vector<void*> bufs;
    explicit DevScratch(wf_ctx* c) : ctx(c) {}
    DevScratch(const DevScratch&) = delete;
    DevScratch& operator=(const DevScratch&) = delete;
    ~DevScratch() { for (void* p : bufs) if (p) wf_dev_free(ctx, p); }
    int alloc(size_t bytes, void** out) {
        int r = wf_dev_alloc(ctx, bytes, out);
        if (r == WF_OK) bufs.push_back(*out);
        return r;
    }
    void forget(void* p) { for (void*& q : bufs) if (q == p) { q = nullptr; return; } }
    void free(void* p) { if (!p) return; forget(p); wf_dev_free(ctx, p); }
    void* keep(void* p) { forget(p); return p; }
};
int wf_mat_alloc(wf_ctx* ctx, size_t rows, u32 cols, wf_mat** out);
int wf_mat_alloc_w(wf_ctx* ctx, size_t rows, u32 cols, int W, wf_mat** out);
extern "C" int wf_trace_lde_cosetwise(wf_ctx* ctx, const uint64_t* const* cols, const uint64_t* d_cols, uint32_t ncols, size_t nrows, int mont,
                           uint32_t log_blowup, wf_mat** polys_out, wf_mat** lde_out, bool coset_major,
                           const std::function<int(u32)>* after_coset);
extern "C" int wf_mat_lde_cosets(wf_ctx* ctx, const wf_mat* polys, uint32_t log_blowup, uint32_t k0, uint32_t k1, wf_mat* lde);
extern "C" int wf_mat_lde_from_coset(wf_ctx* ctx, const wf_mat* polys, uint32_t log_blowup, uint32_t k0, wf_mat* lde);
struct PublicCoin;
struct Digest;
struct wf_fri;
int wf_fri_build_layers_coin(wf_ctx* ctx, int hash_id, const wf_mat* evals, int d, uint32_t folding, uint32_t rem_max_deg,
                             uint32_t blowup, PublicCoin& coin, std::vector<Digest>& commitments, wf_fri** out);
int wf_get_twiddles(wf_ctx* ctx, u32 log_n, const u64** out);
struct wf_tree;
int wf_fri_layer_tree(wf_ctx* ctx, int hash_id, const u64* vals, size_t len, int d, int ld, int nf, wf_tree** out);
struct OpenPlan {
    u32 depth;
    u32 digest_bytes = 32;
    std::vector<u64> want;
    std::vector<std::vector<size_t>> vec_slots;
    std::vector<size_t> leaf_slot;
};
int wf_open_plan(wf_ctx* ctx, size_t n, const uint64_t* positions, size_t k, OpenPlan& pl);
void wf_open_finish(const OpenPlan& pl, const uint8_t* got, uint8_t* leaves_out, ByteVec& proof);
struct GatherBatch {
    struct RowJob { SegMatrix m; std::vector<u64> pos; size_t idx_off, out_off; };
    struct DigJob { const wf_tree* t; OpenPlan plan; std::vector<u64> idx; size_t idx_off, out_off; };
    std::vector<RowJob> rows;
    std::vector<DigJob> digs;
    const wf_comm* comm = nullptr;
    u64* result = nullptr;
    size_t add_rows(const SegMatrix& m, const std::vector<u64>& pos);
    int add_opening(wf_ctx* ctx, const wf_tree* t, const std::vector<u64>& pos, size_t* id);
    int add_opening_sharded(wf_ctx* ctx, const wf_tree* t, size_t n_global, int world, int rank, const std::vector<u64>& pos,
                            size_t* id, std::vector<std::pair<size_t, u64>>* top_slots);
    int run(wf_ctx* ctx);
    const u64* row_result(size_t id) const { return result + rows[id].out_off; }
    const u8* digest_result(size_t id) const { return (const u8*)(result + digs[id].out_off); }
    u64* digest_words(size_t id) { return result + digs[id].out_off; }
};
struct FriLayer {
    u64* evals;
    size_t len;
    wf_tree* tree;
};
struct wf_fri {
    int hash_id, d, ld;
    u32 folding, blowup;
    std::vector<FriLayer> layers;
    std::vector<u64> remainder;
};

struct FriProofPlan { std::vector<size_t> row_ids, dig_ids; std::vector<size_t> nq; };
int wf_fri_queue_proof(wf_ctx* ctx, wf_fri* f, const std::vector<u64>& positions, GatherBatch& gb, FriProofPlan& plan);
void wf_fri_finish_proof(const wf_fri* f, const GatherBatch& gb, const FriProofPlan& plan, ByteVec& out,
                         const FriProofPlan* before = nullptr);
int wf_tree_open_many_bytes(wf_ctx* ctx, const wf_tree* t, const uint64_t* positions, size_t k, uint8_t* leaves_out,
                            ByteVec& proof);

#define CK(call)                                                                                          \
    do {                                                                                                  \
        cudaError_t _e = (call);                                                                          \
        if (_e != cudaSuccess)                                                                            \
            return wf_fail(ctx, WF_ERR_CUDA, "%s:%d %s: %s", __FILE__, __LINE__, #call, cudaGetErrorString(_e)); \
    } while (0)
#define CKI(call)                   \
    do {                            \
        int _r = (call);            \
        if (_r != WF_OK) return _r; \
    } while (0)
```

### winterfell_b200/csrc/ntt.cuh

```cuda
#pragma once
#include <cuda_runtime.h>
#include <stdint.h>

#include "gl64.cuh"

#define NTT_LANES 8
#ifndef NTT_THREADS
#define NTT_THREADS 512
#endif
#ifndef NTT_LD_BATCH
#define NTT_LD_BATCH 8
#endif
#ifndef NTT_MIN_BLOCKS
#define NTT_MIN_BLOCKS 2
#endif
#define NTT_MAX_LOGS 11

struct NttPassParams {
    const u64* in;
    u64* out;
    size_t in_seg_stride, out_seg_stride;
    size_t in_batch_stride, out_batch_stride;
    int W;
    int logS;
    u32 logR, logC;
    int inverse;
    u32 out_row_mul, out_row_add;
    int y_in_out;
    u32 out_W, out_col0;
    const u64* sub_tw;
    const u64* pre_tab;
    size_t pre_batch_stride;
    int has_post;
    const u64* master;
    u32 logM;
    u32 a_mul, b_mul;
    u32 batch0;
    const u64 *tw_hi, *tw_lo;
    u32 tw_split;
    int vec_in, vec_out;
    const u64* ctab;
    u64 cconst;
};

enum { NTT_STRIDED = 0, NTT_CONTIG = 1 };

size_t ntt_pass_smem_bytes(const NttPassParams& p);
cudaError_t ntt_launch_pass(int mode, const NttPassParams& p, u32 n_segments, u32 n_batch, cudaStream_t st);
#define NTT2_MIN_LOGS 6
cudaError_t ntt2_launch_pass(int mode, const NttPassParams& p, u32 n_segments, u32 n_batch, cudaStream_t st);
size_t ntt2_tw_entries(int logS);
cudaError_t ntt2_build_tw(int logS, u64* d_out, cudaStream_t st);
```

### winterfell_b200/csrc/ntt2.cu

```cuda
#include "minidft.cuh"
#include "ntt.cuh"

#ifndef NTT2_THREADS
#define NTT2_THREADS 256
#endif
#ifndef NTT2_MINB
#define NTT2_MINB 2
#endif
#define NTT2_TILE_ELEMS 8192

template <int LOGS>
struct Plan {
    static constexpr int rounds = LOGS >= 9 ? 3 : 2;
    static constexpr int r0 = (LOGS == 8) ? 4 : 3;
    static constexpr int r1 = (LOGS == 11 || LOGS == 8 || LOGS == 7) ? 4 : 3;
    static constexpr int r2 = LOGS >= 9 ? LOGS - r0 - r1 : 0;
    static_assert(LOGS >= 6 && LOGS <= 11, "plan covers 2^6 .. 2^11");
    static_assert(r0 + r1 + r2 == LOGS && (rounds == 2 || (r2 == 3 || r2 == 4)), "radices must add up");
    static constexpr int lanes = LOGS == 11 ? 4 : 8;
    static constexpr int tw0_entries = 1 << LOGS;
    static constexpr int tw1_entries = rounds == 3 ? (1 << (LOGS - r0)) : 0;
    static constexpr int tw_entries = tw0_entries + tw1_entries;
};
template <int LOGS> __host__ __device__ constexpr int plan_radix(int k) { return k == 0 ? Plan<LOGS>::r0 : (k == 1 ? Plan<LOGS>::r1 : Plan<LOGS>::r2); }
template <int LOGS> __host__ __device__ constexpr int plan_stage(int k) { return k == 0 ? 0 : (k == 1 ? Plan<LOGS>::r0 : Plan<LOGS>::r0 + Plan<LOGS>::r1); }

template <int LK>
__host__ __device__ constexpr u32 swz_const(u32 r) {
    u32 x = r >> LK, h = 0;
    while (x) { h ^= x & ((1u << LK) - 1); x >>= LK; }
    return h;
}
template <int LK>
__host__ __device__ constexpr u32 swz_lo(u32 Q) { return swz_const<LK>(Q) ^ (Q & ((1u << LK) - 1)); }
template <int LK>
__host__ __device__ constexpr u32 swz_hi(u32 Q) { return Q & ~((1u << LK) - 1); }
__host__ __device__ constexpr u32 brev_const(u32 v, int bits) {
    u32 r = 0;
    for (int i = 0; i < bits; i++) r |= ((v >> i) & 1u) << (bits - 1 - i);
    return r;
}
template <int LOGS, int LK, u32 STEP, u32 N, u32 IT = 0, class F>
__device__ __forceinline__ void for_brev_rows(F&& f) {
    if constexpr (IT < N) {
        constexpr u32 c = brev_const(IT * STEP, LOGS);
        f(IT, swz_lo<LK>(c), swz_hi<LK>(c));
        for_brev_rows<LOGS, LK, STEP, N, IT + 1>(f);
    }
}
template <int LK>
__device__ __forceinline__ u32 swz_hash(u32 r) {
    if (LK == 1) return __popc(r >> 1) & 1;
    u32 x = r >> 2;
    x ^= x >> 4;
    x ^= x >> 8;
    x ^= x >> 2;
    return x & 3;
}
template <int LK>
__device__ __forceinline__ u32 prow(u32 r) { return r ^ swz_hash<LK>(r); }

__device__ __forceinline__ void bulk_init(u64* mbar, int tid) {
    if (tid == 0) {
        u32 mb = (u32)__cvta_generic_to_shared(mbar);
        asm volatile("mbarrier.init.shared::cta.b64 [%0], 1;" ::"r"(mb));
        asm volatile("fence.mbarrier_init.release.cluster;" ::: "memory");
    }
}
__device__ __forceinline__ void bulk_expect(u64* mbar, u32 bytes) {
    u32 mb = (u32)__cvta_generic_to_shared(mbar);
    asm volatile("mbarrier.arrive.expect_tx.shared::cta.b64 _, [%0], %1;" ::"r"(mb), "r"(bytes) : "memory");
}
__device__ __forceinline__ void bulk_copy(void* smem_dst, const void* gsrc, u32 bytes, u64* mbar) {
    u32 mb = (u32)__cvta_generic_to_shared(mbar), dst = (u32)__cvta_generic_to_shared(smem_dst);
    asm volatile("cp.async.bulk.shared::cluster.global.mbarrier::complete_tx::bytes [%0], [%1], %2, [%3];" ::"r"(dst), "l"(gsrc), "r"(bytes),
                 "r"(mb)
                 : "memory");
}
__device__ __forceinline__ void bulk_wait(u64* mbar) {
    u32 mb = (u32)__cvta_generic_to_shared(mbar), done = 0;
    while (!done)
        asm volatile("{\n\t.reg .pred p;\n\tmbarrier.try_wait.parity.shared::cta.b64 p, [%1], 0;\n\tselp.u32 %0, 1, 0, p;\n\t}" : "=r"(done) : "r"(mb) : "memory");
}

__device__ __forceinline__ void cp_async16(void* smem_dst, const void* gsrc, bool ok) {
    const u32 dst = (u32)__cvta_generic_to_shared(smem_dst);
    asm volatile("cp.async.cg.shared.global [%0], [%1], 16, %2;" ::"r"(dst), "l"(gsrc), "r"(ok ? 16 : 0) : "memory");
}
__device__ __forceinline__ void cp_async8(void* smem_dst, const void* gsrc, bool ok) {
    const u32 dst = (u32)__cvta_generic_to_shared(smem_dst);
    asm volatile("cp.async.ca.shared.global [%0], [%1], 8, %2;" ::"r"(dst), "l"(gsrc), "r"(ok ? 8 : 0) : "memory");
}
__device__ __forceinline__ void cp_async_commit() { asm volatile("cp.async.commit_group;" ::: "memory"); }
__device__ __forceinline__ void cp_async_wait_all() { asm volatile("cp.async.wait_group 0;" ::: "memory"); }

template <int LOGS, int K>
__device__ __forceinline__ void tile_round(u64* __restrict__ s, const u64* __restrict__ tw, const u64* __restrict__ pre, int tid) {
    constexpr int LANES = Plan<LOGS>::lanes, LK = LANES == 8 ? 1 : 2;
    constexpr int R = plan_radix<LOGS>(K), ST = plan_stage<LOGS>(K);
    constexpr int LOGSPAN = LOGS - ST - R;
    constexpr u32 SPAN = 1u << LOGSPAN;
    constexpr bool LAST = LOGSPAN == 0;
    constexpr u32 TASKS = (1u << LOGS) * LANES / 16;
    if (R == 4) {
#pragma unroll 1
        for (u32 task = tid; task < TASKS; task += NTT2_THREADS) {
            const u32 lane = task % LANES, bf = task / LANES;
            const u32 lo = bf & (SPAN - 1), base = ((bf >> LOGSPAN) << (LOGSPAN + 4)) + lo;
            const u32 bh = base ^ swz_hash<LK>(base);
            u64* pr[1 << LK];
#pragma unroll
            for (int v = 0; v < (1 << LK); v++) pr[v] = s + ((bh ^ v) * LANES + lane);
            u64 x[16];
#pragma unroll
            for (int q = 0; q < 16; q++) x[q] = pr[swz_lo<LK>((u32)q << LOGSPAN)][swz_hi<LK>((u32)q << LOGSPAN) * LANES];
            if (K == 0 && pre) {
#pragma unroll
                for (int q = 0; q < 16; q++) x[q] = gl_mul(x[q], __ldg(pre + base + ((u32)q << LOGSPAN)));
            }
            mini_dft<4>(x);
            if (!LAST) {
                const ulonglong2* t2 = reinterpret_cast<const ulonglong2*>(tw + (size_t)lo * 16);
#pragma unroll
                for (int h = 0; h < 8; h++) {
                    const ulonglong2 w = t2[h];
                    if (h > 0) x[2 * h] = gl_mul(x[2 * h], w.x);
                    x[2 * h + 1] = gl_mul(x[2 * h + 1], w.y);
                }
            }
#pragma unroll
            for (int q = 0; q < 16; q++) pr[swz_lo<LK>((u32)q << LOGSPAN)][swz_hi<LK>((u32)q << LOGSPAN) * LANES] = x[q];
        }
    } else {
        constexpr int LP = LANES / 2;
#pragma unroll 1
        for (u32 task = tid; task < TASKS; task += NTT2_THREADS) {
            const u32 lp = task % LP, bf = task / LP;
            const u32 lo = bf & (SPAN - 1), base = ((bf >> LOGSPAN) << (LOGSPAN + 3)) + lo;
            const u32 bh = base ^ swz_hash<LK>(base);
            ulonglong2* pr[1 << LK];
#pragma unroll
            for (int v = 0; v < (1 << LK); v++) pr[v] = reinterpret_cast<ulonglong2*>(s + ((bh ^ v) * LANES + 2 * lp));
            u64 xa[8], xb[8];
#pragma unroll
            for (int q = 0; q < 8; q++) {
                const ulonglong2 v = pr[swz_lo<LK>((u32)q << LOGSPAN)][swz_hi<LK>((u32)q << LOGSPAN) * (LANES / 2)];
                xa[q] = v.x;
                xb[q] = v.y;
            }
            if (K == 0 && pre) {
#pragma unroll
                for (int q = 0; q < 8; q++) {
                    const u64 f = __ldg(pre + base + ((u32)q << LOGSPAN));
                    xa[q] = gl_mul(xa[q], f);
                    xb[q] = gl_mul(xb[q], f);
                }
            }
            mini_dft<3>(xa);
            mini_dft<3>(xb);
            if (!LAST) {
                const ulonglong2* t2 = reinterpret_cast<const ulonglong2*>(tw + (size_t)lo * 8);
#pragma unroll
                for (int h = 0; h < 4; h++) {
                    const ulonglong2 w = t2[h];
                    if (h > 0) { xa[2 * h] = gl_mul(xa[2 * h], w.x); xb[2 * h] = gl_mul(xb[2 * h], w.x); }
                    xa[2 * h + 1] = gl_mul(xa[2 * h + 1], w.y);
                    xb[2 * h + 1] = gl_mul(xb[2 * h + 1], w.y);
                }
            }
#pragma unroll
            for (int q = 0; q < 8; q++) pr[swz_lo<LK>((u32)q << LOGSPAN)][swz_hi<LK>((u32)q << LOGSPAN) * (LANES / 2)] = make_ulonglong2(xa[q], xb[q]);
        }
    }
}

template <int MODE, int LOGS>
__global__ void __launch_bounds__(NTT2_THREADS, NTT2_MINB) ntt2_pass_kernel(const NttPassParams p) {
    extern __shared__ __align__(16) u64 smem[];
    constexpr int LANES = Plan<LOGS>::lanes, LK = LANES == 8 ? 1 : 2, LP = LANES / 2;
    constexpr u32 S = 1u << LOGS;
    const int tid = threadIdx.x;
    const int W = p.W, logW = 31 - __clz(W);
    const int T = W >= LANES ? 1 : (LANES >> logW);
    const int chunks = W >= LANES ? W / LANES : 1;
    u64* s = smem;
    u64* rtw = s + (size_t)S * LANES;
    u64* ctw = rtw + Plan<LOGS>::tw_entries;
    u64* mbar = ctw + (p.has_post ? (size_t)S * T : 0);

    const bool ymap = p.y_in_out;
    const u32 tc = ymap ? blockIdx.y : blockIdx.x;
    const u32 tile = tc / chunks, q0 = (tc % chunks) * LANES;
    const u32 g = ymap ? blockIdx.z : blockIdx.y, b = ymap ? blockIdx.x : blockIdx.z;
    const u32 R = 1u << p.logR, C = 1u << p.logC;
    const u32 ncols = MODE == NTT_STRIDED ? C : R;

    {
        const u64* in = p.in + (size_t)g * p.in_seg_stride + (size_t)b * p.in_batch_stride;
        const u32 lp = tid % LP;
        const u32 l0 = 2 * lp;
        const u32 t0 = W >= LANES ? 0 : (l0 >> logW), t1 = W >= LANES ? 0 : ((l0 + 1) >> logW);
        const u32 w0 = W >= LANES ? q0 + l0 : (l0 & (W - 1)), w1 = W >= LANES ? q0 + l0 + 1 : ((l0 + 1) & (W - 1));
        const u32 c0 = tile * T + t0, c1 = tile * T + t1;
        const bool ok0 = c0 < ncols, ok1 = c1 < ncols;
        const bool yin = MODE == NTT_CONTIG && ymap;
        const u64 istride = MODE == NTT_STRIDED ? ((u64)W << p.logC) : (yin ? ((u64)p.out_row_mul << p.logR) * p.out_W : (u64)W);
        const u64* a0 = MODE == NTT_STRIDED ? in + (size_t)c0 * W + w0
                        : yin ? in + ((size_t)c0 * p.out_row_mul + (size_t)b * p.out_row_add) * p.out_W + p.out_col0 + w0
                              : in + (((size_t)c0 << p.logC) * W + w0);
        const u64* a1 = MODE == NTT_STRIDED ? in + (size_t)c1 * W + w1
                        : yin ? in + ((size_t)c1 * p.out_row_mul + (size_t)b * p.out_row_add) * p.out_W + p.out_col0 + w1
                              : in + (((size_t)c1 << p.logC) * W + w1);
        if (!ok0) a0 = p.in;
        if (!ok1) a1 = p.in;
        const u64 s0 = ok0 ? istride : 0, s1 = ok1 ? istride : 0;
        const bool vec = p.vec_in;
        constexpr u32 ROWS_PER_IT = NTT2_THREADS / LP;
#pragma unroll 4
        for (u32 i = tid / LP; i < S; i += ROWS_PER_IT) {
            u64* dst = s + prow<LK>(i) * LANES + l0;
            if (vec) {
                cp_async16(dst, a0 + i * s0, ok0);
            } else {
                cp_async8(dst, a0 + i * s0, ok0);
                cp_async8(dst + 1, a1 + i * s1, ok1);
            }
        }
        cp_async_commit();
    }

    bulk_init(mbar, tid);
    __syncthreads();
    if (tid == 0) {
        bulk_expect(mbar, Plan<LOGS>::tw_entries * 8);
        bulk_copy(rtw, p.sub_tw, Plan<LOGS>::tw_entries * 8, mbar);
    }

    if (p.has_post && T == 1) {
        const u32 M = 1u << p.logM, lo_mask = (1u << p.tw_split) - 1, c = tile;
        auto wpow = [&](u64 e64) {
            u32 e = (u32)(e64 & (M - 1));
            if (p.inverse && e) e = M - e;
            return gl_mul(p.tw_hi[e >> p.tw_split], p.tw_lo[e & lo_mask]);
        };
        u64 K = wpow((u64)(p.batch0 + b) * p.b_mul * c);
        if (p.ctab) K = gl_mul(K, p.ctab[c < ncols ? c : 0]);
        if (p.cconst != 1) K = gl_mul(K, p.cconst);
        const u64 step = wpow((u64)NTT2_THREADS * p.a_mul * c);
        u64 x = gl_mul(K, wpow((u64)tid * p.a_mul * c));
        for (u32 j = tid; j < S; j += NTT2_THREADS) {
            ctw[j] = x;
            x = gl_mul(x, step);
        }
    } else if (p.has_post) {
        const u32 M = 1u << p.logM, lo_mask = (1u << p.tw_split) - 1;
        for (u32 idx = tid; idx < S * (u32)T; idx += NTT2_THREADS) {
            const u32 j = idx / T, tt = idx % T, c = tile * T + tt;
            u64 e64 = ((u64)j * p.a_mul + (u64)(p.batch0 + b) * p.b_mul) * c;
            u32 e = (u32)(e64 & (M - 1));
            if (p.inverse && e) e = M - e;
            u64 x = gl_mul(p.tw_hi[e >> p.tw_split], p.tw_lo[e & lo_mask]);
            if (p.ctab) x = gl_mul(x, p.ctab[c < ncols ? c : 0]);
            if (p.cconst != 1) x = gl_mul(x, p.cconst);
            ctw[idx] = x;
        }
    }

    cp_async_wait_all();
    bulk_wait(mbar);
    __syncthreads();

    tile_round<LOGS, 0>(s, rtw, p.pre_tab ? p.pre_tab + (size_t)b * p.pre_batch_stride : nullptr, tid);
    __syncthreads();
    if (Plan<LOGS>::rounds == 3) {
        tile_round<LOGS, 1>(s, rtw + Plan<LOGS>::tw0_entries, nullptr, tid);
        __syncthreads();
        tile_round<LOGS, 2>(s, nullptr, nullptr, tid);
    } else {
        tile_round<LOGS, 1>(s, nullptr, nullptr, tid);
    }
    __syncthreads();

    u64* out = p.out + (size_t)g * p.out_seg_stride + (size_t)b * p.out_batch_stride;
    {
        const u32 lp = tid % LP, l0 = 2 * lp;
        const u32 t0 = W >= LANES ? 0 : (l0 >> logW), t1 = W >= LANES ? 0 : ((l0 + 1) >> logW);
        const u32 w0 = W >= LANES ? q0 + l0 : (l0 & (W - 1)), w1 = W >= LANES ? q0 + l0 + 1 : ((l0 + 1) & (W - 1));
        const u32 c0 = tile * T + t0, c1 = tile * T + t1;
        const bool ok0 = c0 < ncols, ok1 = c1 < ncols;
        u64 *o0, *o1, jstride;
        if (MODE == NTT_STRIDED && ymap) {
            o0 = out + (((size_t)c0 << p.logR) * p.out_row_mul + (size_t)b * p.out_row_add) * p.out_W + p.out_col0 + w0;
            o1 = out + (((size_t)c1 << p.logR) * p.out_row_mul + (size_t)b * p.out_row_add) * p.out_W + p.out_col0 + w1;
            jstride = (u64)p.out_row_mul * p.out_W;
        } else if (MODE == NTT_STRIDED) {
            o0 = out + (size_t)c0 * W + w0;
            o1 = out + (size_t)c1 * W + w1;
            jstride = (u64)W << p.logC;
        } else {
            o0 = out + ((size_t)c0 * p.out_row_mul + (size_t)b * p.out_row_add) * p.out_W + p.out_col0 + w0;
            o1 = out + ((size_t)c1 * p.out_row_mul + (size_t)b * p.out_row_add) * p.out_W + p.out_col0 + w1;
            jstride = ((u64)p.out_row_mul << p.logR) * p.out_W;
        }
        const bool post = p.has_post, scale = !p.has_post && p.cconst != 1, vec = p.vec_out;
        const u32 inv_mask = p.inverse ? (S - 1) : 0;
        constexpr u32 ROWS_PER_IT = NTT2_THREADS / LP;
        if (!p.inverse && vec && T == 1) {
            const u32 j0 = tid / LP, r0 = __brev(j0) >> (32 - LOGS), rh = r0 ^ swz_hash<LK>(r0);
            const ulonglong2* pr[1 << LK];
#pragma unroll
            for (int v = 0; v < (1 << LK); v++) pr[v] = reinterpret_cast<const ulonglong2*>(s + ((rh ^ v) * LANES + l0));
            const u64* cj = ctw + j0;
            u64* oj = o0 + (u64)j0 * jstride;
            const u64 ostep = (u64)ROWS_PER_IT * jstride;
            for_brev_rows<LOGS, LK, ROWS_PER_IT, S / ROWS_PER_IT>([&](u32 it, u32 lo, u32 hi) {
                ulonglong2 v = pr[lo][hi * (LANES / 2)];
                if (post) {
                    const u64 f = cj[it * ROWS_PER_IT];
                    v.x = gl_mul(v.x, f);
                    v.y = gl_mul(v.y, f);
                } else if (scale) {
                    v.x = gl_mul(v.x, p.cconst);
                    v.y = gl_mul(v.y, p.cconst);
                }
                if (ok0) *reinterpret_cast<ulonglong2*>(oj + it * ostep) = v;
            });
            return;
        }
#pragma unroll 4
        for (u32 j = tid / LP; j < S; j += ROWS_PER_IT) {
            const u32 jf = inv_mask ? ((S - j) & inv_mask) : j;
            const u32 r = __brev(jf) >> (32 - LOGS);
            ulonglong2 v = *reinterpret_cast<const ulonglong2*>(s + prow<LK>(r) * LANES + l0);
            if (post) {
                const u64 f0 = ctw[j * T + t0];
                v.x = gl_mul(v.x, f0);
                v.y = gl_mul(v.y, t1 == t0 ? f0 : ctw[j * T + t1]);
            } else if (scale) {
                v.x = gl_mul(v.x, p.cconst);
                v.y = gl_mul(v.y, p.cconst);
            }
            if (vec) {
                if (ok0) *reinterpret_cast<ulonglong2*>(o0 + (u64)j * jstride) = v;
            } else {
                if (ok0) o0[(u64)j * jstride] = v.x;
                if (ok1) o1[(u64)j * jstride] = v.y;
            }
        }
    }
}

template <int LOGS>
__global__ void ntt2_build_tw_kernel(u64* out, u64 w_s) {
    const u32 idx = blockIdx.x * blockDim.x + threadIdx.x;
    if (idx >= (u32)Plan<LOGS>::tw_entries) return;
    int k = idx < (u32)Plan<LOGS>::tw0_entries ? 0 : 1;
    const u32 li = k == 0 ? idx : idx - Plan<LOGS>::tw0_entries;
    const int r = plan_radix<LOGS>(k), st = plan_stage<LOGS>(k);
    const u32 lo = li >> r, qo = li & ((1u << r) - 1);
    const u32 e = (lo * (__brev(qo) >> (32 - r))) << st;
    out[idx] = gl_pow(w_s, e);
}

template <int LOGS>
static size_t smem_bytes_t(const NttPassParams& p) {
    const int lanes = Plan<LOGS>::lanes;
    const size_t S = (size_t)1 << LOGS, T = p.W >= lanes ? 1 : lanes / p.W;
    return (S * lanes + Plan<LOGS>::tw_entries + (p.has_post ? S * T : 0) + 2) * 8;
}
template <int MODE, int LOGS>
static cudaError_t launch_t(const NttPassParams& p, u32 n_segments, u32 n_batch, cudaStream_t st) {
    const int lanes = Plan<LOGS>::lanes;
    const u32 T = p.W >= lanes ? 1 : lanes / p.W, chunks = p.W >= lanes ? p.W / lanes : 1;
    const u32 ncols = MODE == NTT_STRIDED ? (1u << p.logC) : (1u << p.logR);
    const size_t smem = smem_bytes_t<LOGS>(p);
    const u32 tiles = ((ncols + T - 1) / T) * chunks;
    const dim3 grid = p.y_in_out ? dim3(n_batch, tiles, n_segments) : dim3(tiles, n_segments, n_batch);
    cudaError_t e = cudaFuncSetAttribute(ntt2_pass_kernel<MODE, LOGS>, cudaFuncAttributeMaxDynamicSharedMemorySize, (int)smem);
    if (e != cudaSuccess) return e;
    ntt2_pass_kernel<MODE, LOGS><<<grid, NTT2_THREADS, smem, st>>>(p);
    return cudaGetLastError();
}
template <int MODE>
static cudaError_t launch_m(const NttPassParams& p, u32 n_segments, u32 n_batch, cudaStream_t st) {
    switch (p.logS) {
        case 6: return launch_t<MODE, 6>(p, n_segments, n_batch, st);
        case 7: return launch_t<MODE, 7>(p, n_segments, n_batch, st);
        case 8: return launch_t<MODE, 8>(p, n_segments, n_batch, st);
        case 9: return launch_t<MODE, 9>(p, n_segments, n_batch, st);
        case 10: return launch_t<MODE, 10>(p, n_segments, n_batch, st);
        case 11: return launch_t<MODE, 11>(p, n_segments, n_batch, st);
    }
    return cudaErrorInvalidValue;
}
cudaError_t ntt2_launch_pass(int mode, const NttPassParams& p, u32 n_segments, u32 n_batch, cudaStream_t st) {
    return mode == NTT_STRIDED ? launch_m<NTT_STRIDED>(p, n_segments, n_batch, st) : launch_m<NTT_CONTIG>(p, n_segments, n_batch, st);
}
size_t ntt2_tw_entries(int logS) {
    switch (logS) {
        case 6: return Plan<6>::tw_entries; case 7: return Plan<7>::tw_entries; case 8: return Plan<8>::tw_entries;
        case 9: return Plan<9>::tw_entries; case 10: return Plan<10>::tw_entries; case 11: return Plan<11>::tw_entries;
    }
    return 0;
}
cudaError_t ntt2_build_tw(int logS, u64* d_out, cudaStream_t st) {
    const u64 w = gl_root_of_unity((u32)logS);
    const unsigned nb = (unsigned)((ntt2_tw_entries(logS) + 255) / 256);
    switch (logS) {
        case 6: ntt2_build_tw_kernel<6><<<nb, 256, 0, st>>>(d_out, w); break;
        case 7: ntt2_build_tw_kernel<7><<<nb, 256, 0, st>>>(d_out, w); break;
        case 8: ntt2_build_tw_kernel<8><<<nb, 256, 0, st>>>(d_out, w); break;
        case 9: ntt2_build_tw_kernel<9><<<nb, 256, 0, st>>>(d_out, w); break;
        case 10: ntt2_build_tw_kernel<10><<<nb, 256, 0, st>>>(d_out, w); break;
        case 11: ntt2_build_tw_kernel<11><<<nb, 256, 0, st>>>(d_out, w); break;
        default: return cudaErrorInvalidValue;
    }
    return cudaGetLastError();
}
```

### winterfell_b200/csrc/prover.cu

```cuda
#include <algorithm>
#include <chrono>

#include "internal.hpp"
#include "air_host.hpp"
#include "blake3.cuh"
#include "alg_hash.cuh"

#include "constraints_generic.cuh"

#ifndef FIB_ROWS_D3
#define FIB_ROWS_D3 2
#endif
struct FibEvalParams {
    SegMatrix lde;
    SegMatrix out;
    u32 k, log_n, log_blowup, log_ce_blowup;
    const u64* coef;
    u64 K0[3], K1[3];
    const u64* tw_ce;
    u64 zt[8];
    u64 last;
    size_t row0, ce_rows;
    u32 log_step;
};
// ... 896 lines not shown
        } else if (aw) {
            generic_constraints_kernel<D, true><<<blocks, 128, 0, ctx->st>>>(p);
        } else {
            generic_constraints_kernel<D, false><<<blocks, 128, 0, ctx->st>>>(p);
        }
        ctx->launches++;
        CK(cudaGetLastError());
    }
    CK(cudaStreamSynchronize(ctx->st));
    stage.comp = nullptr;
    *out = comp;
    return WF_OK;
}

static size_t comp_subcoset_rows(size_t n, u32 kc) {
    size_t m = n;
    while (m < n * kc) m <<= 1;
    return m;
}
int composition_polys(wf_ctx* ctx, const wf_mat* comp, u32 log_n, int D, u32 kc, wf_mat** polys_out) {
    const size_t n = (size_t)1 << log_n;
    if (comp->m.rows < n * kc || (int)comp->m.cols != D) return wf_fail(ctx, WF_ERR_INVALID, "composition trace shape");
    wf_mat *ccoefs, *cpolys;
    const size_t m = comp_subcoset_rows(n, kc);
    if (m < comp->m.rows && comp->m.nseg() == 1) {
        wf_mat* sub;
        CKI(wf_mat_alloc_w(ctx, m, comp->m.cols, comp->m.W, &sub));
        const size_t rb = (size_t)comp->m.W * 8, stride = comp->m.rows / m;
        cudaError_t e = cudaMemcpy2DAsync(sub->m.base, rb, comp->m.base, stride * rb, rb, m, cudaMemcpyDeviceToDevice, ctx->st);
        int rc = e == cudaSuccess ? wf_mat_interpolate_with_offset(ctx, sub, GL_GENERATOR, &ccoefs)
                                  : wf_fail(ctx, WF_ERR_CUDA, "composition sub-coset copy: %s", cudaGetErrorString(e));
        wf_mat_free(ctx, sub);
        if (rc != WF_OK) return rc;
    } else {
        CKI(wf_mat_interpolate_with_offset(ctx, comp, GL_GENERATOR, &ccoefs));
    }
    if (kc == 1 && ccoefs->m.rows == n) {
        wf_mark(ctx, "composition_interpolate");
        *polys_out = ccoefs;
        return WF_OK;
    }
    CKI(wf_mat_alloc(ctx, n, kc * D, &cpolys));
    if (cpolys->m.W > (int)(kc * D)) CK(cudaMemsetAsync(cpolys->m.base, 0, cpolys->m.words() * 8, ctx->st));
    comp_split_kernel<<<(unsigned)((n * kc * D + 255) / 256), 256, 0, ctx->st>>>(ccoefs->m, n, kc, D, cpolys->m);
    ctx->launches++;
    CK(cudaGetLastError());
    wf_mat_free(ctx, ccoefs);
    wf_mark(ctx, "composition_interpolate");
    *polys_out = cpolys;
    return WF_OK;
}
static int composition_lde(wf_ctx* ctx, const wf_mat* comp, const wf_mat* cpolys, u32 log_n, u32 log_b, u32 kc, wf_mat** lde_out) {
    const size_t n = (size_t)1 << log_n;
    if (kc != 1 || comp->m.rows != n || comp->m.nseg() != 1 || comp->m.W != cpolys->m.W || cpolys->m.nseg() != 1)
        return wf_mat_lde(ctx, cpolys, log_b, lde_out);
    if (log_b > 7 || log_n + log_b > 32) return wf_fail(ctx, WF_ERR_INVALID, "bad blowup");
    const u32 b = 1u << log_b;
    wf_mat* clde;
    CKI(wf_mat_alloc(ctx, n << log_b, cpolys->m.cols, &clde));
    coset0_rows_kernel<<<(unsigned)((n * comp->m.W + 255) / 256), 256, 0, ctx->st>>>(comp->m.base, n, comp->m.W, b, clde->m.base);
    ctx->launches++;
    const cudaError_t e = cudaGetLastError();
    int r = e == cudaSuccess ? wf_mat_lde_from_coset(ctx, cpolys, log_b, 1, clde)
                             : wf_fail(ctx, WF_ERR_CUDA, "composition coset 0 copy: %s", cudaGetErrorString(e));
    if (r != WF_OK) { wf_mat_free(ctx, clde); return r; }
    *lde_out = clde;
    return WF_OK;
}
int composition_commit(wf_ctx* ctx, int h, const wf_mat* comp, u32 log_n, u32 log_b, int D, u32 kc, wf_mat** polys_out,
                       wf_mat** lde_out, wf_tree** tree_out, u32 partition_words = 0) {
    wf_mat *cpolys = nullptr, *clde = nullptr;
    CKI(composition_polys(ctx, comp, log_n, D, kc, &cpolys));
    int r = composition_lde(ctx, comp, cpolys, log_n, log_b, kc, &clde);
    if (r == WF_OK) {
        wf_mark(ctx, "composition_lde");
        if (tree_out) r = wf_commit_rows_partitioned(ctx, h, clde, partition_words, tree_out);
    }
    if (r != WF_OK) { wf_mat_free(ctx, cpolys); wf_mat_free(ctx, clde); return r; }
    *polys_out = cpolys;
    *lde_out = clde;
    return WF_OK;
}

template <int D>
int deep_compose(wf_ctx* ctx, const wf_mat* lde, const wf_mat* alde, const wf_mat* clde, u32 kc, u32 log_N,
                 const std::vector<GlExt<D>>& dc, const GlExt<D>& z, const GlExt<D>& zg, const GlExt<D>& Sz, const GlExt<D>& Szg,
                 wf_mat** out, size_t row0 = 0, size_t nrows = 0) {
    const u32 c = lde->m.cols, aw = alde ? alde->m.cols / D : 0, ct = c + aw;
    const size_t N = nrows ? nrows : ((size_t)1 << log_N);
    for (const GlExt<D>* w : {&z, &zg}) {
        bool base = true;
        for (int q = 1; q < D; q++) base = base && w->v[q] == 0;
        if (base && gl_sqr_n(gl_mul(w->v[0], 2635249152773512046ULL), (int)log_N) == 1)
            return wf_fail(ctx, WF_ERR_INVALID, "DEEP point %s lies on the LDE domain: its denominators vanish", w == &z ? "z" : "z*g");
    }
    DeepPoint<D> pz, pzg;
    if (!deep_point<D>(z, pz) || !deep_point<D>(zg, pzg)) return wf_fail(ctx, WF_ERR_STATE, "conjugates of the out-of-domain point are inconsistent");
    u64 *d_dt, *d_dq, *d_da;
    CKI(upload_ext<D>(ctx, dc, 0, ct + kc, &d_dt));
    d_da = d_dt + (size_t)c * D;
    d_dq = d_dt + (size_t)ct * D;
    wf_mat* deep;
    CKI(wf_mat_alloc(ctx, N, D, &deep));
    DeepParams p;
    p.trace = lde->m; p.cons = clde->m; p.out = deep->m; p.c = c; p.kc = kc; p.log_N = log_N;
    p.row0 = row0; p.nrows = nrows;
    p.tcc = d_dt; p.ccc = d_dq; p.acc = d_da; p.aw = aw;
    p.aux = aw ? alde->m : lde->m;
    CKI(wf_get_twiddles(ctx, log_N, &p.tw_N));
    const size_t coef_bytes = (size_t)(c + aw + kc) * D * 8;
    deep_sum_kernel<D><<<(unsigned)((N + DEEP_SUM_THREADS - 1) / DEEP_SUM_THREADS), DEEP_SUM_THREADS, coef_bytes, ctx->st>>>(p);
    const size_t rows_per_thread = DEEP_ROWS;
    size_t threads = (N + rows_per_thread - 1) / rows_per_thread;
    deep_div_kernel<D><<<(unsigned)((threads + 255) / 256), 256, 0, ctx->st>>>(p, pz, pzg, Sz, Szg);
    ctx->launches += 2;
    CK(cudaGetLastError());
    wf_dev_free(ctx, d_dt);
    *out = deep;
    return WF_OK;
}

template <int D>
int deep_compose_polys(wf_ctx* ctx, const wf_mat* polys, const wf_mat* apolys, const wf_mat* cpolys, u32 kc, u32 log_b,
                       const std::vector<GlExt<D>>& dc, const GlExt<D>& z, const GlExt<D>& zg, wf_mat** out) {
    const u32 c = polys->m.cols, aw = apolys ? apolys->m.cols / D : 0, ct = c + aw;
    const size_t n = polys->m.rows, ntiles = (n + SYN_TILE - 1) / SYN_TILE;
    const u32 log_n = log2_ceil(n);
    DevScratch tmp(ctx);
    u64* d_dt;
    CKI(upload_ext<D>(ctx, dc, 0, ct + kc, &d_dt));
    tmp.bufs.push_back(d_dt);
    void* d_agg;
    CKI(tmp.alloc(ntiles * 2 * D * 8, &d_agg));
    wf_mat* quot;
    CKI(wf_mat_alloc(ctx, n, D, &quot));
    DeepParams p{};
    p.trace = polys->m; p.cons = cpolys->m; p.out = quot->m; p.c = c; p.kc = kc; p.log_N = log_n;
    p.tcc = d_dt; p.acc = d_dt + (size_t)c * D; p.ccc = d_dt + (size_t)ct * D; p.aw = aw;
    p.aux = aw ? apolys->m : polys->m;
    deep_sum_kernel<D><<<(unsigned)((n + DEEP_SUM_THREADS - 1) / DEEP_SUM_THREADS), DEEP_SUM_THREADS, (size_t)(ct + kc) * D * 8, ctx->st>>>(p);
    SynDivParams<D> sp;
    sp.b[0] = z; sp.b[1] = zg;
    for (int pt = 0; pt < 2; pt++) { sp.b_items[pt] = ext_pow(sp.b[pt], SYN_ITEMS); sp.b_tile[pt] = ext_pow(sp.b[pt], SYN_TILE); }
    syn_div_reduce<D><<<(unsigned)ntiles, SYN_THREADS, 0, ctx->st>>>(quot->m.base, n, sp, (u64*)d_agg);
    syn_div_carry<D><<<1, SYN_THREADS, 0, ctx->st>>>((u64*)d_agg, ntiles, sp);
    syn_div_apply<D><<<(unsigned)ntiles, SYN_THREADS, 0, ctx->st>>>(quot->m.base, n, sp, (const u64*)d_agg);
    ctx->launches += 4;
    const cudaError_t e = cudaGetLastError();
    const int r = e == cudaSuccess ? wf_mat_lde(ctx, quot, log_b, out) : wf_fail(ctx, WF_ERR_CUDA, "DEEP quotient launch: %s", cudaGetErrorString(e));
    wf_mat_free(ctx, quot);
    return r;
}

static int validation_result(wf_ctx* ctx, int r, const TraceReport& rep) {
    if (r != WF_OK) return r;
    return rep.kind == WF_VALID ? WF_OK : wf_fail(ctx, WF_ERR_INVALID, "%s", rep.msg.c_str());
}

struct ProofScope {
    wf_ctx* ctx;
    std::vector<wf_mat**> mats;
    std::vector<wf_tree**> trees;
    wf_fri** fri = nullptr;
    explicit ProofScope(wf_ctx* c) : ctx(c) {}
    void own(std::initializer_list<wf_mat**> l) { mats.insert(mats.end(), l); }
    void own(std::initializer_list<wf_tree**> l) { trees.insert(trees.end(), l); }
    void drop(wf_mat*& m) { wf_mat_free(ctx, m); m = nullptr; }
    ~ProofScope() {
        if (fri && *fri) wf_fri_free(ctx, *fri);
        for (wf_mat** m : mats) if (*m) wf_mat_free(ctx, *m);
        for (wf_tree** t : trees) if (*t) wf_tree_free(ctx, *t);
    }
};

template <int D>
int prove_air(wf_ctx* ctx, const AirHost& air_in, const uint64_t* const* trace_cols, const uint64_t* d_trace, int mont, u32 log_n,
              const Options& o, wf_aux_builder_fn aux_builder, void* aux_user, std::vector<u8>& proof_out,
              wf_aux_assertions_fn aux_assertions = nullptr, const AuxBuildHost* aux_build = nullptr) {
    AirHost air_dyn;
    if (aux_assertions) air_dyn = air_in;
    const AirHost& air = aux_assertions ? air_dyn : air_in;
    const int h = o.hash_id;
    const size_t n = (size_t)1 << log_n;
    const u32 log_b = log2_ceil(o.blowup);
    const size_t N = n << log_b;
    const u32 c = air.w, kc = air.num_comp_cols(n), log_ceb = air.log_ce_blowup();
    const u32 aw = air.aw;
    if (aw && !aux_builder && !aux_build) return wf_fail(ctx, WF_ERR_INVALID, "multi-segment AIR needs an aux trace builder");
    const bool validate = ctx->validate && !air.is_fib;
    if (log_ceb > log_b) return wf_fail(ctx, WF_ERR_INVALID, "blowup factor too small for the constraint degrees");
    for (auto& col : air.periodic) if (col.size() > n) return wf_fail(ctx, WF_ERR_INVALID, "periodic column longer than the trace");
    CKI(validate_degrees(ctx, air.all_degrees(), n));
    CKI(validate_assertions(ctx, air.aux_asserts, n, 3, "aux assertion"));
    CKI(validate_assertions(ctx, air.asserts, n, 1, "assertion"));
    Channel ch(h, context_seed(air, n, o));

    wf_mat *trace = nullptr, *polys = nullptr, *lde = nullptr, *atrace = nullptr, *apolys = nullptr, *alde = nullptr, *comp = nullptr,
           *cpolys = nullptr, *clde = nullptr, *deep = nullptr;
    wf_tree *ttree = nullptr, *atree = nullptr, *ctree = nullptr;
    wf_fri* fri = nullptr;
    ProofScope scope(ctx);
    scope.own({&trace, &polys, &lde, &atrace, &apolys, &alde, &comp, &cpolys, &clde, &deep});
    scope.own({&ttree, &atree, &ctree});
    scope.fri = &fri;
    wf_mark(ctx, "start");
    if (d_trace) {
        CKI(wf_mat_from_device_columns(ctx, d_trace, c, n, &trace));
        wf_mark(ctx, "trace_upload_layout");
        CKI(wf_mat_interpolate(ctx, trace, &polys));
        if (!aux_build && !validate) scope.drop(trace);
        wf_mark(ctx, "trace_interpolate");
        CKI(wf_mat_lde(ctx, polys, log_b, &lde));
    } else {
        CKI(wf_trace_lde_from_host(ctx, trace_cols, c, n, mont, log_b, &polys, &lde));
    }
    wf_mark(ctx, "trace_lde");
    CKI(wf_commit_rows_partitioned(ctx, h, lde, o.part_words(c, 1), &ttree));
    u8 root[32];
    CKI(wf_tree_root(ctx, ttree, root));
    wf_mark(ctx, "trace_commit");
    ch.commit(root);

    std::vector<u64> rnd_flat;
    if (aw) {
        for (u32 i = 0; i < air.nr; i++) { GlExt<D> e = draw_ext<D>(ch.coin); for (int q = 0; q < D; q++) rnd_flat.push_back(e.v[q]); }
        std::vector<u64> rnd_user = rnd_flat;
        if (mont) for (u64& v : rnd_user) v = gl_mul(v, 0xFFFFFFFFULL);
        std::vector<u64> aux_host;
        if (aux_build) {
            if (!trace) CKI(wf_mat_evaluate(ctx, polys, &trace));
            CKI(wf_aux_build_run(ctx, *aux_build, trace, c, air.periodic, rnd_flat.data(), air.nr, D, &atrace));
            if (!validate) scope.drop(trace);
            wf_mark(ctx, "aux_build");
        } else {
            aux_host.resize((size_t)aw * n * D);
            if (aux_builder(aux_user, rnd_user.data(), aux_host.data()) != 0) return wf_fail(ctx, WF_ERR_INVALID, "aux trace builder failed");
        }
        if (aux_assertions) {
            std::vector<u64> vals = get_aux_assertion_words(air_dyn, D, mont);
            if (aux_assertions(aux_user, rnd_user.data(), vals.data()) != 0) return wf_fail(ctx, WF_ERR_INVALID, "aux assertion callback failed");
            if (!set_aux_assertion_words(air_dyn, vals.data(), D, mont))
                return wf_fail(ctx, WF_ERR_INVALID, "aux assertion value is not a canonical field element");
        }
        if (!aux_build) {
            std::vector<const u64*> cols(aw);
            for (u32 j = 0; j < aw; j++) cols[j] = &aux_host[(size_t)j * n * D];
            CKI(wf_mat_from_host_columns(ctx, cols.data(), aw, n, D, mont, &atrace));
        }
        CKI(wf_mat_interpolate(ctx, atrace, &apolys));
        if (!validate) scope.drop(atrace);
        CKI(wf_mat_lde(ctx, apolys, log_b, &alde));
        CKI(wf_commit_rows_partitioned(ctx, h, alde, o.part_words(aw, D), &atree));
        CKI(wf_tree_root(ctx, atree, root));
        wf_mark(ctx, "aux_commit");
        ch.commit(root);
    }
    if (validate) {
        if (!trace) CKI(wf_mat_evaluate(ctx, polys, &trace));
        TraceReport rep;
        CKI(validation_result(ctx, wf_check_trace(ctx, air, trace, atrace, rnd_flat.data(), log_n, D, rep), rep));
        scope.drop(trace);
        scope.drop(atrace);
    }

    std::vector<GlExt<D>> cc = draw_coeffs<D>(ch.coin, o.batch_c, air.num_constraints());
    const size_t m = comp_subcoset_rows(n, kc);
    const u32 log_step = m < (n << log_ceb) ? log_n + log_ceb - log2_ceil(m) : 0;
    CKI(eval_constraints<D>(ctx, air, lde, alde, cc, rnd_flat, log_n, log_b, &comp, 0, 0, log_step));
    if (validate) {
        TraceReport rep;
        CKI(validation_result(ctx, wf_check_degrees(ctx, air, lde, alde, rnd_flat.data(), log_n, log_b, D, rep), rep));
    }
    wf_mark(ctx, "constraint_eval");
    CKI(composition_commit(ctx, h, comp, log_n, log_b, D, kc, &cpolys, &clde, &ctree, o.part_words(kc, D)));
    scope.drop(comp);
    CKI(wf_tree_root(ctx, ctree, root));
    wf_mark(ctx, "composition_commit");
    ch.commit(root);

    GlExt<D> z = draw_ext<D>(ch.coin);
    GlExt<D> zg = ext_mul_base(z, gl_root_of_unity(log_n));
    std::vector<std::vector<GlExt<D>>> ood;
    {
        std::vector<const wf_mat*> mats = {polys, cpolys};
        if (aw) mats.push_back(apolys);
        CKI(ood_eval<D>(ctx, mats, z, zg, ood));
    }
    std::vector<GlExt<D>>&t_cur = ood[0], &t_nxt = ood[1];
    std::vector<GlExt<D>> q_cur = ext_from_components<D>(ood[2]), q_nxt = ext_from_components<D>(ood[3]);
    if (aw) {
        auto a_cur = ext_from_components<D>(ood[4]), a_nxt = ext_from_components<D>(ood[5]);
        t_cur.insert(t_cur.end(), a_cur.begin(), a_cur.end());
        t_nxt.insert(t_nxt.end(), a_nxt.begin(), a_nxt.end());
    }
    const u32 ct = c + aw;
    ByteVec ood_t, ood_q;
    ch.coin.reseed(ood_frames<D>(h, t_cur, t_nxt, q_cur, q_nxt, &ood_t, &ood_q));
    wf_mark(ctx, "ood_frames");
    std::vector<GlExt<D>> dc = draw_coeffs<D>(ch.coin, o.batch_d, ct + kc);
    CKI(deep_compose_polys<D>(ctx, polys, apolys, cpolys, kc, log_b, dc, z, zg, &deep));
    wf_mark(ctx, "deep_composition");
    {
        std::vector<Digest> fri_roots;
        CKI(wf_fri_build_layers_coin(ctx, h, deep, D, o.folding, o.rem_max_deg, o.blowup, ch.coin, fri_roots, &fri));
        for (auto& r : fri_roots) ch.commitments.bytes(r.b, WF_DIGEST_BYTES(h));
    }
    scope.drop(deep);
    wf_mark(ctx, "fri_layers");
    u64 nonce;
    CKI(grind_on_device(ctx, h, ch.coin.seed, o.grinding, &nonce));
    if (ch.coin.check_leading_zeros(nonce) < o.grinding) return wf_fail(ctx, WF_ERR_STATE, "grinding self-check failed");
    std::vector<u64> pos;
    if (!query_positions(ch.coin, o.num_queries, N, nonce, pos)) return wf_fail(ctx, WF_ERR_STATE, "failed to draw query positions");
    wf_mark(ctx, "grinding");
    ByteVec w;
    write_context(w, air, log_n, o);
    w.u8_((u8)pos.size());
    w.u16_((uint16_t)ch.commitments.v.size());
    w.bytes(ch.commitments.v.data(), ch.commitments.v.size());
    GatherBatch gb;
    FriProofPlan fplan;
    size_t tr_rows = gb.add_rows(lde->m, pos), cr_rows = gb.add_rows(clde->m, pos), tr_dig, cr_dig;
    size_t ar_rows = 0, ar_dig = 0;
    if (aw) ar_rows = gb.add_rows(alde->m, pos);
    CKI(gb.add_opening(ctx, ttree, pos, &tr_dig));
    CKI(gb.add_opening(ctx, ctree, pos, &cr_dig));
    if (aw) CKI(gb.add_opening(ctx, atree, pos, &ar_dig));
    CKI(wf_fri_queue_proof(ctx, fri, pos, gb, fplan));
    CKI(gb.run(ctx));
    write_queries(gb, tr_rows, tr_dig, pos.size() * c, w);
    if (aw) write_queries(gb, ar_rows, ar_dig, pos.size() * aw * D, w);
    write_queries(gb, cr_rows, cr_dig, pos.size() * kc * D, w);
    w.u16_((uint16_t)ood_t.v.size()); w.bytes(ood_t.v.data(), ood_t.v.size());
    w.u16_((uint16_t)ood_q.v.size()); w.bytes(ood_q.v.data(), ood_q.v.size());
    wf_fri_finish_proof(fri, gb, fplan, w);
    w.u64_(nonce);
    wf_mark(ctx, "queries_and_proof");
    proof_out.swap(w.v);
    return WF_OK;
}

__global__ void __launch_bounds__(256) coset_interleave_kernel(SegMatrix src, SegMatrix dst, size_t rows_j, u32 b) {
    const size_t idx = (size_t)blockIdx.x * blockDim.x + threadIdx.x;
    const int W = dst.W;
    if (idx >= dst.rows * (size_t)W) return;
    const size_t row = idx / W;
    const u32 w = (u32)(idx % W), g = blockIdx.y;
    const size_t j = row / b, k = row % b;
    dst.base[(size_t)g * dst.seg_stride + idx] = src.base[(size_t)g * src.seg_stride + (k * rows_j + j) * W + w];
}

struct ShardCtx {
    wf_ctx* ctx;
    const wf_comm* cm;
    int G, r;
    double bytes_sent = 0, bytes_overlapped = 0, ncoll = 0, ms_small = 0;
    bool forked = false;
    int fork() {
        if (cm->fork) { if (cm->fork(cm->user) != 0) return wf_fail(ctx, WF_ERR_STATE, "fork callback failed"); forked = true; }
        return WF_OK;
    }
    int join() {
        if (forked) { forked = false; if (cm->join(cm->user) != 0) return wf_fail(ctx, WF_ERR_STATE, "join callback failed"); }
        return WF_OK;
    }
    std::vector<std::pair<cudaEvent_t, cudaEvent_t>> ev;
    ~ShardCtx() { for (auto& e : ev) { cudaEventDestroy(e.first); cudaEventDestroy(e.second); } }
    int exchange(const std::vector<int>& sp, const std::vector<const void*>& sv, const std::vector<int>& rp, const std::vector<void*>& rv,
                 size_t bytes) {
        cudaEvent_t a = nullptr, b = nullptr;
        if (!forked) {
            CK(cudaEventCreate(&a));
            CK(cudaEventCreate(&b));
            ev.push_back({a, b});
            CK(cudaEventRecord(a, ctx->st));
        }
        if (cm->exchange(cm->user, sp.size(), sp.data(), sv.data(), rp.size(), rp.data(), rv.data(), bytes) != 0)
            return wf_fail(ctx, WF_ERR_STATE, "exchange callback failed");
        if (!forked) CK(cudaEventRecord(b, ctx->st));
        (forked ? bytes_overlapped : bytes_sent) += (double)bytes * (double)sp.size();
        ncoll += 1;
        return WF_OK;
    }
    int all_gather_dev(const void* mine, void* all, size_t bytes) {
        std::vector<int> sp, rp;
        std::vector<const void*> sv;
        std::vector<void*> rv;
        for (int q = 0; q < G; q++) {
            if (q == r) continue;
            sp.push_back(q); sv.push_back(mine);
            rp.push_back(q); rv.push_back((u8*)all + (size_t)q * bytes);
        }
        if ((const u8*)mine != (u8*)all + (size_t)r * bytes)
            CK(cudaMemcpyAsync((u8*)all + (size_t)r * bytes, mine, bytes, cudaMemcpyDeviceToDevice, ctx->st));
        return exchange(sp, sv, rp, rv, bytes);
    }
    int gather_host(const void* send, void* recv, size_t bytes) {
        cudaEvent_t a, b;
        (void)a; (void)b;
        const auto t0 = std::chrono::steady_clock::now();
        if (cm->all_gather_host(cm->user, send, recv, bytes) != 0) return wf_fail(ctx, WF_ERR_STATE, "all_gather_host callback failed");
        ms_small += std::chrono::duration<double, std::milli>(std::chrono::steady_clock::now() - t0).count();
        ncoll += 1;
        return WF_OK;
    }
    int map_peers(void* local_base, std::vector<void*>& out) {
        out.assign(G, nullptr);
        if (const char* e = getenv("WF_PEER_PUSH")) if (atoi(e) == 0) return WF_ERR_UNSUPPORTED;
        cudaIpcMemHandle_t h;
        memset(&h, 0, sizeof(h));
        int ok = cudaIpcGetMemHandle(&h, local_base) == cudaSuccess ? 1 : 0;
        if (!ok) cudaGetLastError();
        struct Msg { cudaIpcMemHandle_t h; int ok; int pad; } mine{h, ok, 0};
        std::vector<Msg> all(G);
        CKI(gather_host(&mine, all.data(), sizeof(Msg)));
        for (int q = 0; q < G; q++) ok &= all[q].ok;
        if (!ok) return WF_ERR_UNSUPPORTED;
        int opened = 1;
        for (int q = 0; q < G; q++) {
            if (q == r) { out[q] = local_base; continue; }
            std::string key((const char*)&all[q].h, sizeof(cudaIpcMemHandle_t));
            auto it = ctx->ipc_opened.find(key);
            if (it != ctx->ipc_opened.end()) { out[q] = it->second; continue; }
            void* pp = nullptr;
            if (cudaIpcOpenMemHandle(&pp, all[q].h, cudaIpcMemLazyEnablePeerAccess) != cudaSuccess) { cudaGetLastError(); opened = 0; continue; }
            ctx->ipc_opened[key] = pp;
            out[q] = pp;
        }
        std::vector<int> flags(G);
        CKI(gather_host(&opened, flags.data(), sizeof(int)));
        for (int q = 0; q < G; q++) if (!flags[q]) return WF_ERR_UNSUPPORTED;
        return WF_OK;
    }
    int host_barrier() {
        int one = 1;
        std::vector<int> all(G);
        return gather_host(&one, all.data(), sizeof(int));
    }
    double exchange_ms() {
        double t = 0;
        for (auto& e : ev) { float ms = 0; if (cudaEventElapsedTime(&ms, e.first, e.second) == cudaSuccess) t += ms; }
        return t;
    }
};

struct ShardTree {
    wf_tree* local = nullptr;
    size_t n_global = 0;
    std::vector<Digest> top;
};
static int shard_tree_finish(ShardCtx& sc, int h, ShardTree& t, Digest* root) {
    wf_ctx* ctx = sc.ctx;
    Digest mine;
    CKI(wf_tree_root(ctx, t.local, mine.b));
    std::vector<Digest> all(sc.G);
    CKI(sc.gather_host(mine.b, all.data(), 32));
    t.top.assign(2 * sc.G, Digest{});
    for (int q = 0; q < sc.G; q++) t.top[sc.G + q] = all[q];
    for (int i = sc.G - 1; i >= 1; i--) t.top[i] = hh_merge(h, t.top[2 * i], t.top[2 * i + 1]);
    *root = t.top[1];
    return WF_OK;
}

static void shard_segments(u32 w, u32 G, u32 r, u32& seg0, u32& nseg) {
    const u32 S = (w + 7) / 8, base = S / G, extra = S % G;
    seg0 = r * base + std::min(r, extra);
    nseg = base + (r < extra ? 1u : 0u);
}
static void shard_columns(u32 w, u32 G, u32 r, u32& first, u32& count) {
    u32 s0, ns;
    shard_segments(w, G, r, s0, ns);
    first = std::min(w, s0 * 8);
    count = std::min(w, (s0 + ns) * 8) - first;
}

static int exchange_halo(ShardCtx& sc, const SegMatrix& m, size_t b) {
    wf_ctx* ctx = sc.ctx;
    DevScratch tmp(ctx);
    void *pk, *pk2;
    const size_t hb = b * m.W * 8;
    const u32 nsg = m.nseg();
    CKI(tmp.alloc(hb * nsg, &pk));
    CKI(tmp.alloc(hb * nsg, &pk2));
    CK(cudaMemcpy2DAsync(pk, hb, m.base, m.seg_stride * 8, hb, nsg, cudaMemcpyDeviceToDevice, ctx->st));
    CKI(sc.exchange({(sc.r + sc.G - 1) % sc.G}, {pk}, {(sc.r + 1) % sc.G}, {pk2}, hb * nsg));
    CK(cudaMemcpy2DAsync(m.base + m.rows * m.W, m.seg_stride * 8, pk2, hb, hb, nsg, cudaMemcpyDeviceToDevice, ctx->st));
    return WF_OK;
}

static int shard_lde_rows(ShardCtx& sc, const wf_mat* polys, u32 log_b, bool halo, wf_mat** out, wf_mat& view) {
    wf_ctx* ctx = sc.ctx;
    const int G = sc.G, r = sc.r;
    const size_t n = polys->m.rows, b = (size_t)1 << log_b, rows_per = (n << log_b) / (size_t)G;
    const int W = polys->m.W;
    const u32 cols = polys->m.cols;
    if (b % (size_t)G != 0) {
        wf_mat *full = nullptr, *rows = nullptr;
        CKI(wf_mat_lde(ctx, polys, log_b, &full));
        if (!halo) {
            *out = full;
            view.m = full->m;
            view.m.base += (size_t)r * rows_per * full->m.W;
            view.m.rows = rows_per;
            return WF_OK;
        }
        int rc = wf_mat_alloc_w(ctx, rows_per + b, cols, full->m.W, &rows);
        if (rc == WF_OK) {
            rows->m.rows = rows_per;
            const size_t rb = (size_t)full->m.W * 8, sp = full->m.seg_stride * 8, dp = rows->m.seg_stride * 8;
            const u32 nsg = full->m.nseg();
            cudaError_t e = cudaMemcpy2DAsync(rows->m.base, dp, full->m.base + (size_t)r * rows_per * full->m.W, sp, rows_per * rb, nsg,
                                              cudaMemcpyDeviceToDevice, ctx->st);
            if (e == cudaSuccess)
                e = cudaMemcpy2DAsync(rows->m.base + rows_per * full->m.W, dp, full->m.base + (size_t)((r + 1) % G) * rows_per * full->m.W, sp,
                                      b * rb, nsg, cudaMemcpyDeviceToDevice, ctx->st);
            if (e != cudaSuccess) rc = wf_fail(ctx, WF_ERR_CUDA, "row shard copy: %s", cudaGetErrorString(e));
        }
        wf_mat_free(ctx, full);
        if (rc != WF_OK) { wf_mat_free(ctx, rows); return rc; }
        *out = rows;
        view.m = rows->m;
        return WF_OK;
    }
    const u32 kpr = (u32)(b / (size_t)G);
    const size_t nj = n / (size_t)G;
    wf_mat *ccos = nullptr, *stage = nullptr, *lde = nullptr;
    int rc = wf_mat_alloc_w(ctx, (size_t)kpr * n, cols, W, &ccos);
    if (rc == WF_OK) rc = wf_mat_lde_cosets(ctx, polys, log_b, (u32)r * kpr, (u32)(r + 1) * kpr, ccos);
    if (rc == WF_OK) rc = wf_mat_alloc_w(ctx, rows_per, cols, W, &stage);
    if (rc == WF_OK) rc = wf_mat_alloc_w(ctx, rows_per + (halo ? b : 0), cols, W, &lde);
    if (rc == WF_OK) {
        lde->m.rows = rows_per;
        const size_t blk = nj * W;
        std::vector<int> sp, rp;
        std::vector<const void*> sv;
        std::vector<void*> rv;
        for (u32 sg = 0; sg < ccos->m.nseg(); sg++) {
            const u64* cb = ccos->m.base + (size_t)sg * ccos->m.seg_stride;
            u64* sb = stage->m.base + (size_t)sg * stage->m.seg_stride;
            for (u32 kl = 0; kl < kpr; kl++)
                for (int q = 0; q < G; q++) {
                    const u64* src = cb + ((size_t)kl * n + (size_t)q * nj) * W;
                    if (q == r) CK(cudaMemcpyAsync(sb + ((size_t)r * kpr + kl) * blk, src, blk * 8, cudaMemcpyDeviceToDevice, ctx->st));
                    else { sp.push_back(q); sv.push_back(src); }
                }
            for (u32 k = 0; k < (u32)b; k++) {
                const int owner = (int)(k / kpr);
                if (owner != r) { rp.push_back(owner); rv.push_back(sb + (size_t)k * blk); }
            }
        }
        rc = sc.exchange(sp, sv, rp, rv, blk * 8);
        if (rc == WF_OK) {
            dim3 grid((unsigned)((rows_per * W + 255) / 256), lde->m.nseg());
            coset_interleave_kernel<<<grid, 256, 0, ctx->st>>>(stage->m, lde->m, nj, (u32)b);
            ctx->launches++;
            if (cudaGetLastError() != cudaSuccess) rc = wf_fail(ctx, WF_ERR_CUDA, "coset_interleave_kernel launch failed");
        }
    }
    wf_mat_free(ctx, ccos);
    wf_mat_free(ctx, stage);
    if (rc == WF_OK && halo) rc = exchange_halo(sc, lde->m, b);
    if (rc != WF_OK) { wf_mat_free(ctx, lde); return rc; }
    *out = lde;
    view.m = lde->m;
    return WF_OK;
}


template <int D>
static int sharded_check_trace(ShardCtx& sc, const AirHost& air, const wf_mat* polys, const wf_mat* mtrace, const wf_mat* atrace,
                               const std::vector<u64>& rnd, u32 log_n, const std::vector<u32>& seg0, const std::vector<u32>& segs) {
    wf_ctx* ctx = sc.ctx;
    const int G = sc.G, r = sc.r;
    const size_t n = (size_t)1 << log_n, nt = n / (size_t)G;
    const u32 fs = seg0[r], nsl = segs[r];
    const u32 col0 = std::min(air.w, fs * 8), cl = std::min(air.w, (fs + nsl) * 8) - col0;
    wf_mat *own = nullptr, *rows = nullptr;
    struct Free { wf_ctx* c; wf_mat** a; wf_mat** b; ~Free() { wf_mat_free(c, *a); wf_mat_free(c, *b); } } fr{ctx, &own, &rows};
    TraceCheckPart part;
    part.acol0 = col0;
    part.s0 = (size_t)r * nt;
    part.s1 = std::min((size_t)(r + 1) * nt, n - air.exemptions);
    if (mtrace) {
        part.amain = mtrace->m;
        part.amain.base += (size_t)fs * mtrace->m.seg_stride;
        part.amain.cols = cl;
        part.main = mtrace;
        part.aux = atrace;
    } else {
        CKI(wf_mat_alloc_w(ctx, n, cl, 8, &own));
        if (cl) {
            wf_mat* ev;
            CKI(wf_mat_evaluate(ctx, polys, &ev));
            const cudaError_t e = layout_select_cols(ev->m, 0, own->m, ctx->st);
            ctx->launches++;
            wf_mat_free(ctx, ev);
            CK(e);
        }
        part.amain = own->m;
        CKI(wf_mat_alloc_w(ctx, nt + 1, air.w, 8, &rows));
        rows->m.rows = nt;
        std::vector<int> sp, rp;
        std::vector<const void*> sv;
        std::vector<void*> rv;
        for (int q = 0; q < G; q++) {
            for (u32 sg = 0; sg < nsl; sg++) {
                const u64* src = own->m.base + (size_t)sg * own->m.seg_stride + (size_t)q * nt * 8;
// ... 45 lines not shown
                const u64* src = loc->m.base + (size_t)(cs0[q] + sg) * loc->m.seg_stride;
                if (q == r) CK(cudaMemcpyAsync(mine->m.base + (size_t)sg * mine->m.seg_stride + (size_t)r * ce_per * 8, src, ce_per * 64,
                                               cudaMemcpyDeviceToDevice, ctx->st));
                else { sp.push_back(q); sv.push_back(src); }
            }
            for (u32 sg = 0; q != r && sg < cns[r]; sg++) { rp.push_back(q); rv.push_back(mine->m.base + (size_t)sg * mine->m.seg_stride + (size_t)q * ce_per * 8); }
        }
        CKI(sc.exchange(sp, sv, rp, rv, ce_per * 64));
    }
    wf_mat_free(ctx, loc);
    loc = nullptr;
    std::vector<u64> d1;
    if (cnt) CKI(wf_column_degrees(ctx, mine, d1));
    d1.resize(blk, 0);
    std::vector<u64> all((size_t)blk * G), deg1(ncols);
    CKI(sc.gather_host(d1.data(), all.data(), (size_t)blk * 8));
    for (int q = 0; q < G; q++)
        for (u32 j = cs0[q] * 8; j < std::min(ncols, (cs0[q] + cns[q]) * 8); j++) deg1[j] = all[(size_t)q * blk + j - cs0[q] * 8];
    TraceReport rep;
    wf_degree_verdict(air, alde != nullptr, D, log_n, deg1, rep);
    return validation_result(ctx, WF_OK, rep);
}

template <int D>
int prove_sharded(wf_ctx* ctx, const wf_comm* cm, const AirHost& air_in, const AuxBuildHost* aux_build, wf_aux_assertions_fn aux_assertions,
                  void* aux_user, const uint64_t* const* local_cols, const uint64_t* d_local, int mont, u32 log_n, const Options& o,
                  std::vector<u8>& proof_out, double* stats) {
    AirHost air_dyn;
    if (aux_assertions) air_dyn = air_in;
    const AirHost& air = aux_assertions ? air_dyn : air_in;
    ShardCtx sc{ctx, cm, cm->world, cm->rank};
    const int G = sc.G, r = sc.r;
    const int h = o.hash_id;
    const size_t n = (size_t)1 << log_n;
    const u32 log_b = log2_ceil(o.blowup);
    const size_t N = n << log_b, b = o.blowup;
    const u32 c = air.w, aw = air.aw, nsg = (c + 7) / 8;
    const size_t rows_per = N / (size_t)G;
    if (G < 2 || (G & (G - 1)) || r < 0 || r >= G) return wf_fail(ctx, WF_ERR_INVALID, "world size must be a power of two >= 2");
    if (aw && !aux_build) return wf_fail(ctx, WF_ERR_INVALID, "multi-segment AIR needs an aux build description");
    std::vector<u32> seg0(G), segs(G), col0(G), ncol(G);
    for (int q = 0; q < G; q++) {
        shard_segments(c, (u32)G, (u32)q, seg0[q], segs[q]);
        shard_columns(c, (u32)G, (u32)q, col0[q], ncol[q]);
    }
    const u32 cl = ncol[r], fs = seg0[r], nsl = segs[r];
    const u32 maxcl = *std::max_element(ncol.begin(), ncol.end());
    const u32 kc = air.num_comp_cols(n), log_ceb = air.log_ce_blowup();
    const size_t ce = n << log_ceb, ce_per = ce / (size_t)G;
    if (rows_per < 64 * b || ce_per < 64) return wf_fail(ctx, WF_ERR_UNSUPPORTED, "trace too short to shard over %d ranks", G);
    const bool validate = ctx->validate && !air.is_fib;
    Channel ch(h, context_seed(air, n, o));

    wf_mat *polys = nullptr, *lde = nullptr, *shard = nullptr, *mtrace = nullptr, *atrace = nullptr, *apolys = nullptr, *arows = nullptr,
           *comp_l = nullptr, *comp = nullptr, *cpolys = nullptr, *clde = nullptr, *deep = nullptr, *fri_in = nullptr, *tstage = nullptr;
    ShardTree ttree, atree, ctree;
    wf_fri* fri = nullptr;
    ProofScope scope(ctx);
    scope.own({&polys, &lde, &shard, &mtrace, &atrace, &apolys, &arows, &comp_l, &comp, &cpolys, &clde, &deep, &fri_in, &tstage});
    scope.own({&ttree.local, &atree.local, &ctree.local});
    scope.fri = &fri;
    struct SLayer { u64* vals; size_t m_l, m_g; ShardTree tree; };
    std::vector<SLayer> slayers;
    std::vector<void*> owned;
    struct Cleanup {
        wf_ctx* ctx; std::vector<SLayer>& sl; std::vector<void*>& ow;
        ~Cleanup() { for (auto& l : sl) wf_tree_free(ctx, l.tree.local); for (void* p : ow) wf_dev_free(ctx, p); }
    } cleanup{ctx, slayers, owned};

    wf_mark(ctx, "start");
    const size_t nj = n / (size_t)G;
    CKI(wf_mat_alloc_w(ctx, rows_per + b, c, 8, &shard));
    shard->m.rows = rows_per;
    wf_mat*& stage = tstage;
    if (cl) CKI(wf_mat_alloc_w(ctx, N, cl, 8, &lde));
    CKI(wf_mat_alloc_w(ctx, rows_per, c, 8, &stage));
    std::vector<void*> peer_stage;
    const bool push = sc.map_peers(stage->m.base, peer_stage) == WF_OK;
    if (push) {
        for (int i = 0; i < 4; i++) if (!ctx->push_st[i]) CK(cudaStreamCreateWithFlags(&ctx->push_st[i], cudaStreamNonBlocking));
        for (int i = 0; i < 16; i++) if (!ctx->push_ev[i]) CK(cudaEventCreateWithFlags(&ctx->push_ev[i], cudaEventDisableTiming));
    }
    auto lde_block = [&](u32 sg, u32 k, int q) {
        return lde->m.base + (size_t)sg * lde->m.seg_stride + ((size_t)k * n + (size_t)q * nj) * 8;
    };
    const std::function<int(u32)> after_coset = [&](u32 k) -> int {
        if (push) {
            cudaEvent_t ev = ctx->push_ev[k % 16];
            CK(cudaEventRecord(ev, ctx->st));
            for (int dq = 1; dq < G; dq++) {
                const int q = (r + dq) % G;
                cudaStream_t ps = ctx->push_st[dq % 4];
                CK(cudaStreamWaitEvent(ps, ev, 0));
                for (u32 sg = 0; sg < nsl; sg++) {
                    u64* dst = (u64*)peer_stage[q] + (size_t)(fs + sg) * stage->m.seg_stride + (size_t)k * nj * 8;
                    CK(cudaMemcpyAsync(dst, lde_block(sg, k, q), nj * 64, cudaMemcpyDeviceToDevice, ps));
                }
            }
            for (u32 sg = 0; sg < nsl; sg++)
                CK(cudaMemcpyAsync(stage->m.base + (size_t)(fs + sg) * stage->m.seg_stride + (size_t)k * nj * 8, lde_block(sg, k, r), nj * 64,
                                   cudaMemcpyDeviceToDevice, ctx->st));
            sc.bytes_overlapped += (double)(G - 1) * nsl * nj * 64;
            return WF_OK;
        }
        std::vector<int> sp, rp;
        std::vector<const void*> sv;
        std::vector<void*> rv;
        for (u32 sg = 0; sg < nsl; sg++)
            for (int q = 0; q < G; q++) {
                u64* dst = stage->m.base + (size_t)(fs + sg) * stage->m.seg_stride + (size_t)k * nj * 8;
                if (q == r) CK(cudaMemcpyAsync(dst, lde_block(sg, k, q), nj * 64, cudaMemcpyDeviceToDevice, ctx->st));
                else { sp.push_back(q); sv.push_back(lde_block(sg, k, q)); }
            }
        for (int q = 0; q < G; q++)
            for (u32 sg = 0; q != r && sg < segs[q]; sg++) {
                rp.push_back(q);
                rv.push_back(stage->m.base + (size_t)(seg0[q] + sg) * stage->m.seg_stride + (size_t)k * nj * 8);
            }
        CKI(sc.fork());
        return sc.exchange(sp, sv, rp, rv, nj * 64);
    };
    if (cl) CKI(wf_trace_lde_cosetwise(ctx, local_cols, d_local, cl, n, mont, log_b, &polys, &lde, true, &after_coset));
    else for (u32 k = 0; k < (u32)b; k++) CKI(after_coset(k));
    wf_mark(ctx, "trace_lde");
    if (push) {
        for (int i = 0; i < 4; i++) CK(cudaStreamSynchronize(ctx->push_st[i]));
        CKI(sc.host_barrier());
        sc.ncoll += 1;
    } else {
        CKI(sc.join());
    }
    {
        SegMatrix dstv = shard->m;
        dim3 grid((unsigned)((rows_per * 8 + 255) / 256), nsg);
        coset_interleave_kernel<<<grid, 256, 0, ctx->st>>>(stage->m, dstv, nj, (u32)b);
        ctx->launches++;
        CK(cudaGetLastError());
    }
    scope.drop(lde);
    scope.drop(stage);
    CKI(exchange_halo(sc, shard->m, b));
    wf_mark(ctx, "trace_exchange");
    Digest root;
    CKI(wf_commit_rows_partitioned(ctx, h, shard, o.part_words(c, 1), &ttree.local));
    ttree.n_global = N;
    CKI(shard_tree_finish(sc, h, ttree, &root));
    wf_mark(ctx, "trace_commit");
    ch.commit(root.b);

    std::vector<u64> rnd_flat;
    wf_mat aview;
    if (aw) {
        for (u32 i = 0; i < air.nr; i++) { GlExt<D> e = draw_ext<D>(ch.coin); for (int q = 0; q < D; q++) rnd_flat.push_back(e.v[q]); }
        CKI(wf_mat_alloc_w(ctx, n, c, 8, &mtrace));
        if (cl) {
            wf_mat* ev;
            CKI(wf_mat_evaluate(ctx, polys, &ev));
            SegMatrix dv = mtrace->m;
            dv.base += (size_t)fs * dv.seg_stride;
            dv.cols = cl;
            const cudaError_t e = layout_select_cols(ev->m, 0, dv, ctx->st);
            ctx->launches++;
            wf_mat_free(ctx, ev);
            CK(e);
        }
        {
            std::vector<int> sp, rp;
            std::vector<const void*> sv;
            std::vector<void*> rv;
            for (int q = 0; q < G; q++) {
                if (q == r) continue;
                for (u32 sg = 0; sg < nsl; sg++) { sp.push_back(q); sv.push_back(mtrace->m.base + (size_t)(fs + sg) * mtrace->m.seg_stride); }
                for (u32 sg = 0; sg < segs[q]; sg++) { rp.push_back(q); rv.push_back(mtrace->m.base + (size_t)(seg0[q] + sg) * mtrace->m.seg_stride); }
            }
            CKI(sc.exchange(sp, sv, rp, rv, n * 64));
        }
        wf_mark(ctx, "main_trace_gather");
        CKI(wf_aux_build_run(ctx, *aux_build, mtrace, c, air.periodic, rnd_flat.data(), air.nr, D, &atrace));
        if (!validate) scope.drop(mtrace);
        wf_mark(ctx, "aux_build");
        if (aux_assertions) {
            std::vector<u64> rnd_user = rnd_flat;
            if (mont) for (u64& v : rnd_user) v = gl_mul(v, 0xFFFFFFFFULL);
            std::vector<u64> vals = get_aux_assertion_words(air_dyn, D, mont);
            if (aux_assertions(aux_user, rnd_user.data(), vals.data()) != 0) return wf_fail(ctx, WF_ERR_INVALID, "aux assertion callback failed");
            if (!set_aux_assertion_words(air_dyn, vals.data(), D, mont))
                return wf_fail(ctx, WF_ERR_INVALID, "aux assertion value is not a canonical field element");
        }
        CKI(wf_mat_interpolate(ctx, atrace, &apolys));
        if (!validate) scope.drop(atrace);
        CKI(shard_lde_rows(sc, apolys, log_b, true, &arows, aview));
        wf_mark(ctx, "aux_lde");
        CKI(wf_commit_rows_partitioned(ctx, h, &aview, o.part_words(aw, D), &atree.local));
        atree.n_global = N;
        CKI(shard_tree_finish(sc, h, atree, &root));
        wf_mark(ctx, "aux_commit");
        ch.commit(root.b);
    }
    if (validate) {
        CKI(sharded_check_trace<D>(sc, air, polys, mtrace, atrace, rnd_flat, log_n, seg0, segs));
        scope.drop(mtrace);
        scope.drop(atrace);
    }
    std::vector<GlExt<D>> cc = draw_coeffs<D>(ch.coin, o.batch_c, air.num_constraints());
    CKI(eval_constraints<D>(ctx, air, shard, aw ? arows : nullptr, cc, rnd_flat, log_n, log_b, &comp_l, (size_t)r * ce_per, ce_per));
    if (validate) CKI(sharded_check_degrees<D>(sc, air, shard, aw ? arows : nullptr, rnd_flat, log_n, log_b));
    wf_mark(ctx, "constraint_eval");
    CKI(wf_mat_alloc(ctx, ce, D, &comp));
    CKI(sc.all_gather_dev(comp_l->m.base, comp->m.base, ce_per * comp->m.W * 8));
    scope.drop(comp_l);
    CKI(composition_polys(ctx, comp, log_n, D, kc, &cpolys));
    scope.drop(comp);
    wf_mat cview;
    CKI(shard_lde_rows(sc, cpolys, log_b, false, &clde, cview));
    wf_mark(ctx, "composition_lde");
    CKI(wf_commit_rows_partitioned(ctx, h, &cview, o.part_words(kc, D), &ctree.local));
    ctree.n_global = N;
    CKI(shard_tree_finish(sc, h, ctree, &root));
    wf_mark(ctx, "composition_commit");
    ch.commit(root.b);
    GlExt<D> z = draw_ext<D>(ch.coin);
    GlExt<D> zg = ext_mul_base(z, gl_root_of_unity(log_n));
    std::vector<std::vector<GlExt<D>>> ood;
    {
        std::vector<const wf_mat*> mats = {cpolys};
        if (aw) mats.push_back(apolys);
        if (cl) mats.push_back(polys);
        CKI(ood_eval<D>(ctx, mats, z, zg, ood));
    }
    const u32 ct = c + aw;
    std::vector<GlExt<D>> t_cur(c), t_nxt(c);
    {
        std::vector<u64> mine((size_t)maxcl * 2 * D, 0), all((size_t)G * maxcl * 2 * D);
        const size_t mi = aw ? 4 : 2;
        for (u32 j = 0; j < cl; j++)
            for (int q = 0; q < D; q++) { mine[((size_t)j * 2) * D + q] = ood[mi][j].v[q]; mine[((size_t)j * 2 + 1) * D + q] = ood[mi + 1][j].v[q]; }
        CKI(sc.gather_host(mine.data(), all.data(), mine.size() * 8));
        for (int s = 0; s < G; s++)
            for (u32 jl = 0; jl < ncol[s]; jl++) {
                const u32 j = col0[s] + jl;
                const u64* v = &all[((size_t)s * maxcl + jl) * 2 * D];
                for (int q = 0; q < D; q++) { t_cur[j].v[q] = v[q]; t_nxt[j].v[q] = v[D + q]; }
            }
    }
    if (aw) {
        auto a_cur = ext_from_components<D>(ood[2]), a_nxt = ext_from_components<D>(ood[3]);
        t_cur.insert(t_cur.end(), a_cur.begin(), a_cur.end());
        t_nxt.insert(t_nxt.end(), a_nxt.begin(), a_nxt.end());
    }
    std::vector<GlExt<D>> q_cur = ext_from_components<D>(ood[0]), q_nxt = ext_from_components<D>(ood[1]);
    ByteVec ood_t, ood_q;
    ch.coin.reseed(ood_frames<D>(h, t_cur, t_nxt, q_cur, q_nxt, &ood_t, &ood_q));
    wf_mark(ctx, "ood_frames");
    std::vector<GlExt<D>> dc = draw_coeffs<D>(ch.coin, o.batch_d, ct + kc);
    GlExt<D> Sz = ext_zero<D>(), Szg = ext_zero<D>();
    for (u32 j = 0; j < ct; j++) { Sz = ext_add(Sz, ext_mul(dc[j], t_cur[j])); Szg = ext_add(Szg, ext_mul(dc[j], t_nxt[j])); }
    for (u32 j = 0; j < kc; j++) { Sz = ext_add(Sz, ext_mul(dc[ct + j], q_cur[j])); Szg = ext_add(Szg, ext_mul(dc[ct + j], q_nxt[j])); }
    CKI(deep_compose<D>(ctx, shard, aw ? &aview : nullptr, &cview, kc, log_n + log_b, dc, z, zg, Sz, Szg, &deep, (size_t)r * rows_per, rows_per));
    wf_mark(ctx, "deep_composition");
    const u32 nf = o.folding;
    const int ld = deep->m.W;
    const size_t max_rem = (size_t)(o.rem_max_deg + 1) * o.blowup;
    u64* cur = deep->m.base;
    size_t L = N;
    u32 min_log = 17;
    if (const char* e = getenv("WF_SHARD_FRI_MIN_LOG")) min_log = (u32)atoi(e);
    while (L > max_rem && L / (size_t)G >= ((size_t)1 << min_log) && (L / nf) % (size_t)G == 0 && L / nf / (size_t)G >= 2) {
        SLayer sl;
        sl.m_g = L / nf;
        sl.m_l = sl.m_g / (size_t)G;
        void* vp;
        CKI(wf_dev_alloc(ctx, (size_t)nf * sl.m_l * ld * 8, &vp));
        owned.push_back(vp);
        sl.vals = (u64*)vp;
        std::vector<int> sp, rp;
        std::vector<const void*> sv;
        std::vector<void*> rv;
        for (u32 t = 0; t < nf; t++) {
            const size_t P = (size_t)nf * r + t;
            const int owner = (int)(P % (size_t)G);
            const size_t q = P / (size_t)G;
            const u64* src = cur + (size_t)t * sl.m_l * ld;
            if (owner == r) CK(cudaMemcpyAsync(sl.vals + q * sl.m_l * ld, src, sl.m_l * ld * 8, cudaMemcpyDeviceToDevice, ctx->st));
            else { sp.push_back(owner); sv.push_back(src); }
        }
        for (u32 q = 0; q < nf; q++) {
            const size_t P = (size_t)q * G + r;
            const int src_rank = (int)(P / nf);
            if (src_rank != r) { rp.push_back(src_rank); rv.push_back(sl.vals + (size_t)q * sl.m_l * ld); }
        }
        CKI(sc.exchange(sp, sv, rp, rv, sl.m_l * ld * 8));
        CKI(wf_fri_layer_tree(ctx, h, sl.vals, (size_t)nf * sl.m_l, D, ld, (int)nf, &sl.tree.local));
        sl.tree.n_global = sl.m_g;
        slayers.push_back(sl);
        CKI(shard_tree_finish(sc, h, slayers.back().tree, &root));
        ch.commit(root.b);
        GlExt<D> alpha = draw_ext<D>(ch.coin);
        const u32 logL = log2_ceil(L);
        const u64* master;
        CKI(wf_get_twiddles(ctx, logL, &master));
        void* nx;
        CKI(wf_dev_alloc(ctx, sl.m_l * ld * 8, &nx));
        owned.push_back(nx);
        if (ld > D) CK(cudaMemsetAsync(nx, 0, sl.m_l * ld * 8, ctx->st));
        u64 av[3] = {0, 0, 0};
        for (int q = 0; q < D; q++) av[q] = alpha.v[q];
        CK(fri_fold_layer(sl.vals, (size_t)nf * sl.m_l, D, ld, (int)nf, av, master, (u64*)nx, ld, ctx->st, nullptr, (size_t)r * sl.m_l, logL));
        ctx->launches++;
        cur = (u64*)nx;
        L = sl.m_g;
    }
    CKI(wf_mat_alloc(ctx, L, D, &fri_in));
    CKI(sc.all_gather_dev(cur, fri_in->m.base, (L / (size_t)G) * ld * 8));
    scope.drop(deep);
    {
        std::vector<Digest> fri_roots;
        CKI(wf_fri_build_layers_coin(ctx, h, fri_in, D, o.folding, o.rem_max_deg, o.blowup, ch.coin, fri_roots, &fri));
        for (auto& rt : fri_roots) ch.commitments.bytes(rt.b, WF_DIGEST_BYTES(h));
    }
    scope.drop(fri_in);
    wf_mark(ctx, "fri_layers");
    u64 nonce;
    CKI(grind_on_device(ctx, h, ch.coin.seed, o.grinding, &nonce));
    if (ch.coin.check_leading_zeros(nonce) < o.grinding) return wf_fail(ctx, WF_ERR_STATE, "grinding self-check failed");
    std::vector<u64> pos;
    if (!query_positions(ch.coin, o.num_queries, N, nonce, pos)) return wf_fail(ctx, WF_ERR_STATE, "failed to draw query positions");
    wf_mark(ctx, "grinding");
    ByteVec w;
    write_context(w, air, log_n, o);
    w.u8_((u8)pos.size());
    w.u16_((uint16_t)ch.commitments.v.size());
    w.bytes(ch.commitments.v.data(), ch.commitments.v.size());
    GatherBatch gb;
    gb.comm = cm;
    const u64 NONE = ~(u64)0;
    auto owned_rows = [&](const std::vector<u64>& p, size_t per) {
        std::vector<u64> l(p.size(), NONE);
        for (size_t i = 0; i < p.size(); i++) if ((int)(p[i] / per) == r) l[i] = p[i] % per;
        return l;
    };
    std::vector<std::pair<size_t, u64>> top_t, top_a, top_c;
    const std::vector<u64> mine = owned_rows(pos, rows_per);
    size_t tr_rows = gb.add_rows(shard->m, mine), cr_rows = gb.add_rows(cview.m, mine), ar_rows = aw ? gb.add_rows(aview.m, mine) : 0;
    size_t tr_dig, cr_dig, ar_dig = 0;
    CKI(gb.add_opening_sharded(ctx, ttree.local, N, G, r, pos, &tr_dig, &top_t));
    CKI(gb.add_opening_sharded(ctx, ctree.local, N, G, r, pos, &cr_dig, &top_c));
    if (aw) CKI(gb.add_opening_sharded(ctx, atree.local, N, G, r, pos, &ar_dig, &top_a));
    FriProofPlan splan;
    std::vector<std::vector<std::pair<size_t, u64>>> top_f(slayers.size());
    std::vector<u64> fpos = pos;
    for (size_t l = 0; l < slayers.size(); l++) {
        const SLayer& sl = slayers[l];
        fpos = fold_positions(fpos, sl.m_g);
        std::vector<u64> gpos(fpos.size() * nf, NONE);
        for (size_t i = 0; i < fpos.size(); i++)
            if ((int)(fpos[i] / sl.m_l) == r)
                for (u32 j = 0; j < nf; j++) gpos[i * nf + j] = (u64)j * sl.m_l + fpos[i] % sl.m_l;
        SegMatrix lm;
        lm.base = sl.vals; lm.rows = (size_t)nf * sl.m_l; lm.cols = (u32)D; lm.W = ld; lm.seg_stride = lm.rows * ld;
        size_t dig_id;
        splan.row_ids.push_back(gb.add_rows(lm, gpos));
        CKI(gb.add_opening_sharded(ctx, sl.tree.local, sl.m_g, G, r, fpos, &dig_id, &top_f[l]));
        splan.dig_ids.push_back(dig_id);
        splan.nq.push_back(fpos.size());
    }
    FriProofPlan fplan;
    {
        const size_t r0 = gb.rows.size(), d0 = gb.digs.size();
        CKI(wf_fri_queue_proof(ctx, fri, fpos, gb, fplan));
        if (r != 0) {
            for (size_t i = r0; i < gb.rows.size(); i++) std::fill(gb.rows[i].pos.begin(), gb.rows[i].pos.end(), NONE);
            for (size_t i = d0; i < gb.digs.size(); i++) std::fill(gb.digs[i].idx.begin(), gb.digs[i].idx.end(), NONE);
        }
    }
    CKI(gb.run(ctx));
    auto patch = [&](size_t dig_id, const std::vector<std::pair<size_t, u64>>& slots, const ShardTree& t) {
        for (auto& se : slots) memcpy(gb.digest_words(dig_id) + se.first * 4, t.top[se.second].b, 32);
    };
    patch(tr_dig, top_t, ttree);
    patch(cr_dig, top_c, ctree);
    if (aw) patch(ar_dig, top_a, atree);
    for (size_t l = 0; l < slayers.size(); l++) patch(splan.dig_ids[l], top_f[l], slayers[l].tree);
    write_queries(gb, tr_rows, tr_dig, pos.size() * c, w);
    if (aw) write_queries(gb, ar_rows, ar_dig, pos.size() * aw * D, w);
    write_queries(gb, cr_rows, cr_dig, pos.size() * kc * D, w);
    w.u16_((uint16_t)ood_t.v.size()); w.bytes(ood_t.v.data(), ood_t.v.size());
    w.u16_((uint16_t)ood_q.v.size()); w.bytes(ood_q.v.data(), ood_q.v.size());
    wf_fri_finish_proof(fri, gb, fplan, w, &splan);
    w.u64_(nonce);
    wf_mark(ctx, "queries_and_proof");
    proof_out.swap(w.v);
    if (stats) {
        CK(cudaStreamSynchronize(ctx->st));
        stats[0] = sc.bytes_sent; stats[1] = sc.exchange_ms(); stats[2] = sc.ncoll + 1; stats[3] = sc.ms_small;
        for (int i = 4; i < 8; i++) stats[i] = 0;
        stats[4] = (double)slayers.size();
        stats[5] = sc.bytes_overlapped;
        stats[6] = push ? 1.0 : 0.0;
    }
    return WF_OK;
}

}

extern "C" int wf_grind(wf_ctx* ctx, int hash_id, const uint8_t seed[32], uint32_t grinding, uint64_t* nonce) {
    if (!ctx || !seed || !nonce || grinding > 40) return wf_fail(ctx, WF_ERR_INVALID, "bad arguments");
    Digest d;
    memcpy(d.b, seed, 32);
    return grind_on_device(ctx, hash_id, d, grinding, nonce);
}

static int parse_options(wf_ctx* ctx, const uint32_t* opts, Options& o) {
    o = options_from_words(opts);
    if (o.num_partitions > 16) return wf_fail(ctx, WF_ERR_INVALID, "at most 16 partitions (air/src/options.rs:413-414)");
    if (!options_in_range(o) || o.ext < 1 || o.ext > 3) return wf_fail(ctx, WF_ERR_INVALID, "bad proof options");
    if (!WF_HASH_IS_KNOWN(o.hash_id)) return wf_fail(ctx, WF_ERR_UNSUPPORTED, "unknown hash %d", o.hash_id);
    return WF_OK;
}
static int prove_bytes(wf_ctx* ctx, const AirHost& air, const uint64_t* const* trace_cols, const uint64_t* d_trace, int mont,
                       uint32_t log_n, const Options& o, std::vector<u8>& out, wf_aux_builder_fn aux_builder, void* aux_user,
                       wf_aux_assertions_fn aux_assertions, const AuxBuildHost* aux_build) {
    switch (o.ext) {
        case 1: return prove_air<1>(ctx, air, trace_cols, d_trace, mont, log_n, o, aux_builder, aux_user, out, aux_assertions, aux_build);
        case 2: return prove_air<2>(ctx, air, trace_cols, d_trace, mont, log_n, o, aux_builder, aux_user, out, aux_assertions, aux_build);
        case 3: return prove_air<3>(ctx, air, trace_cols, d_trace, mont, log_n, o, aux_builder, aux_user, out, aux_assertions, aux_build);
    }
    return wf_fail(ctx, WF_ERR_UNSUPPORTED, "field extension %u", o.ext);
}
static int prove_dispatch(wf_ctx* ctx, const AirHost& air, const uint64_t* const* trace_cols, const uint64_t* d_trace, int mont,
                          uint32_t log_n, const Options& o, uint8_t* proof, size_t* proof_len, wf_aux_builder_fn aux_builder = nullptr,
                          void* aux_user = nullptr, wf_aux_assertions_fn aux_assertions = nullptr, const AuxBuildHost* aux_build = nullptr) {
    std::vector<u8> out;
    CKI(prove_bytes(ctx, air, trace_cols, d_trace, mont, log_n, o, out, aux_builder, aux_user, aux_assertions, aux_build));
    if (out.size() > *proof_len) return wf_fail(ctx, WF_ERR_INVALID, "proof buffer too small (%zu needed)", out.size());
    memcpy(proof, out.data(), out.size());
    *proof_len = out.size();
    return WF_OK;
}
static int prove_fib_entry(wf_ctx* ctx, const uint64_t* const* trace_cols, const uint64_t* d_trace, int mont, uint32_t k,
                           uint32_t log_n, const uint64_t* results, const uint32_t* opts, uint8_t* proof, size_t* proof_len) {
    if (!ctx || (!trace_cols && !d_trace) || !results || !opts || !proof || !proof_len || k == 0 || 2 * k > 255 || log_n < 3)
        return wf_fail(ctx, WF_ERR_INVALID, "bad arguments");
    Options o;
    CKI(parse_options(ctx, opts, o));
    AirHost air = fib_air_host(k, (size_t)1 << log_n, results);
    return prove_dispatch(ctx, air, trace_cols, d_trace, mont, log_n, o, proof, proof_len);
}
extern "C" int wf_prove_air(wf_ctx* ctx, const uint64_t* air_desc, size_t air_desc_len, const uint64_t* const* trace_cols, int mont,
                            uint32_t log_n, const uint32_t* opts, uint8_t* proof, size_t* proof_len) {
    if (!ctx || !air_desc || !trace_cols || !opts || !proof || !proof_len || log_n < 3)
        return wf_fail(ctx, WF_ERR_INVALID, "bad arguments");
    Options o;
    CKI(parse_options(ctx, opts, o));
    AirHost air;
    if (!parse_air_host(air_desc, air_desc_len, air)) return wf_fail(ctx, WF_ERR_INVALID, "malformed AIR description");
    if (air.aw) return wf_fail(ctx, WF_ERR_INVALID, "multi-segment AIR: use wf_prove_air_aux");
    return prove_dispatch(ctx, air, trace_cols, nullptr, mont, log_n, o, proof, proof_len);
}
extern "C" int wf_prove_air_aux(wf_ctx* ctx, const uint64_t* air_desc, size_t air_desc_len, const uint64_t* const* trace_cols, int mont,
                                uint32_t log_n, const uint32_t* opts, wf_aux_builder_fn aux_builder, void* aux_user, uint8_t* proof,
                                size_t* proof_len) {
    if (!ctx || !air_desc || !trace_cols || !opts || !proof || !proof_len || log_n < 3)
        return wf_fail(ctx, WF_ERR_INVALID, "bad arguments");
    Options o;
    CKI(parse_options(ctx, opts, o));
    AirHost air;
    if (!parse_air_host(air_desc, air_desc_len, air)) return wf_fail(ctx, WF_ERR_INVALID, "malformed AIR description");
    return prove_dispatch(ctx, air, trace_cols, nullptr, mont, log_n, o, proof, proof_len, aux_builder, aux_user);
}
extern "C" int wf_prove_air_aux_dyn(wf_ctx* ctx, const uint64_t* air_desc, size_t air_desc_len, const uint64_t* const* trace_cols, int mont,
                                    uint32_t log_n, const uint32_t* opts, wf_aux_builder_fn aux_builder,
                                    wf_aux_assertions_fn aux_assertions, void* aux_user, uint8_t* proof, size_t* proof_len) {
    if (!ctx || !air_desc || !trace_cols || !opts || !proof || !proof_len || log_n < 3 || !aux_assertions)
        return wf_fail(ctx, WF_ERR_INVALID, "bad arguments");
    Options o;
    CKI(parse_options(ctx, opts, o));
    AirHost air;
    if (!parse_air_host(air_desc, air_desc_len, air)) return wf_fail(ctx, WF_ERR_INVALID, "malformed AIR description");
    return prove_dispatch(ctx, air, trace_cols, nullptr, mont, log_n, o, proof, proof_len, aux_builder, aux_user, aux_assertions);
}

static int parse_aux_build(wf_ctx* ctx, const AirHost& air, const uint64_t* aux_build, size_t aux_build_len, AuxBuildHost& b) {
    if (!air.aw) return wf_fail(ctx, WF_ERR_INVALID, "single-segment AIR: it has no aux segment to build");
    if (const char* why = wf_aux_build_parse(aux_build, aux_build_len, air.w, air.aw, (u32)air.periodic.size(), air.nr, b))
        return wf_fail(ctx, WF_ERR_INVALID, "%s", why);
    return WF_OK;
}
extern "C" int wf_aux_build_check(const uint64_t* air_desc, size_t air_desc_len, const uint64_t* aux_build, size_t aux_build_len,
                                  uint32_t log_n, char* msg, size_t msg_cap) {
    auto say = [&](const char* t) { if (msg && msg_cap) { strncpy(msg, t, msg_cap - 1); msg[msg_cap - 1] = 0; } };
    say("");
    if (!air_desc || !aux_build || log_n < 3 || log_n > 32) { say("bad arguments"); return WF_ERR_INVALID; }
    AirHost air;
    if (!parse_air_host(air_desc, air_desc_len, air)) { say("malformed AIR description"); return WF_ERR_INVALID; }
    wf_ctx note{};
    AuxBuildHost b;
    int r = parse_aux_build(&note, air, aux_build, aux_build_len, b);
    for (auto& col : air.periodic)
        if (r == WF_OK && col.size() > ((size_t)1 << log_n)) r = wf_fail(&note, WF_ERR_INVALID, "periodic column longer than the trace");
    say(note.err.c_str());
    return r;
}
extern "C" int wf_aux_build(wf_ctx* ctx, const uint64_t* air_desc, size_t air_desc_len, const uint64_t* aux_build, size_t aux_build_len,
                            const wf_mat* main_evals, const uint64_t* rand, uint32_t ext, wf_mat** aux) {
    if (!ctx || !air_desc || !aux_build || !main_evals || !aux || ext < 1 || ext > 3) return wf_fail(ctx, WF_ERR_INVALID, "bad arguments");
    AirHost air;
    if (!parse_air_host(air_desc, air_desc_len, air)) return wf_fail(ctx, WF_ERR_INVALID, "malformed AIR description");
    AuxBuildHost b;
    CKI(parse_aux_build(ctx, air, aux_build, aux_build_len, b));
    if (air.nr && !rand) return wf_fail(ctx, WF_ERR_INVALID, "random elements missing");
    return wf_aux_build_run(ctx, b, main_evals, air.w, air.periodic, rand, air.nr, (int)ext, aux);
}
extern "C" int wf_prove_air_aux_built(wf_ctx* ctx, const uint64_t* air_desc, size_t air_desc_len, const uint64_t* aux_build,
                                      size_t aux_build_len, const uint64_t* const* trace_cols, const uint64_t* d_trace, int mont,
                                      uint32_t log_n, const uint32_t* opts, wf_aux_assertions_fn aux_assertions, void* aux_user,
                                      uint8_t* proof, size_t* proof_len) {
    if (!ctx || !air_desc || !aux_build || !opts || !proof || !proof_len || log_n < 3) return wf_fail(ctx, WF_ERR_INVALID, "bad arguments");
    if (!trace_cols == !d_trace) return wf_fail(ctx, WF_ERR_INVALID, "pass exactly one of trace_cols (host) and d_trace (device)");
    Options o;
    CKI(parse_options(ctx, opts, o));
    AirHost air;
    if (!parse_air_host(air_desc, air_desc_len, air)) return wf_fail(ctx, WF_ERR_INVALID, "malformed AIR description");
    AuxBuildHost b;
    CKI(parse_aux_build(ctx, air, aux_build, aux_build_len, b));
    for (auto& col : b.cols)
        for (u32 q = o.ext; q < 3; q++) if (col.init[q]) return wf_fail(ctx, WF_ERR_INVALID, "aux column init has non-zero words beyond the extension degree");
    return prove_dispatch(ctx, air, trace_cols, d_trace, mont, log_n, o, proof, proof_len, nullptr, aux_user, aux_assertions, &b);
}

extern "C" int wf_jit_compile_air(const uint64_t* air_desc, size_t air_desc_len, uint32_t ext, size_t* cubin_bytes, char* log, size_t log_cap) {
    if (!air_desc || ext < 1 || ext > 3) return WF_ERR_INVALID;
    AirHost air;
    if (!parse_air_host(air_desc, air_desc_len, air)) return WF_ERR_INVALID;
    std::vector<char> cubin;
    std::string lg;
    const int rc = wf_jit_compile(wf_jit_source((int)ext, air.w, (u32)air.periodic.size(), air.num_regs, air.prog, air.consts, air.aw, air.nr,
                                                air.aux_num_regs, air.aux_prog), cubin, lg);
    if (log && log_cap) { strncpy(log, lg.c_str(), log_cap - 1); log[log_cap - 1] = 0; }
    if (cubin_bytes) *cubin_bytes = cubin.size();
    if (const char* dump = getenv("WF_JIT_DUMP")) if (rc == 0) { FILE* f = fopen(dump, "wb"); if (f) { fwrite(cubin.data(), 1, cubin.size(), f); fclose(f); } }
    return rc == 0 ? WF_OK : WF_ERR_UNSUPPORTED;
}

extern "C" int wf_air_check(const uint64_t* air_desc, size_t air_desc_len, uint32_t log_n, uint32_t blowup, char* msg, size_t msg_cap) {
    auto say = [&](const char* t) { if (msg && msg_cap) { strncpy(msg, t, msg_cap - 1); msg[msg_cap - 1] = 0; } };
    say("");
    if (!air_desc || log_n < 3 || log_n > 32 || blowup < 2 || blowup > 128 || (blowup & (blowup - 1))) { say("bad arguments"); return WF_ERR_INVALID; }
    AirHost air;
    if (!parse_air_host(air_desc, air_desc_len, air)) { say("malformed AIR description"); return WF_ERR_INVALID; }
    wf_ctx note{};
    const int r = air_check_host(&note, air, log_n, blowup);
    say(note.err.c_str());
    return r;
}

static int air_batch_parse(wf_ctx* ctx, uint32_t batch, const uint64_t* const* air_descs, const size_t* air_desc_lens, uint32_t log_n,
                           uint32_t blowup, std::vector<AirHost>& airs) {
    if (batch == 0 || !air_descs || !air_desc_lens || log_n < 3 || log_n > 32 || blowup < 2 || blowup > 128 || (blowup & (blowup - 1)))
        return wf_fail(ctx, WF_ERR_INVALID, "bad arguments");
    airs.assign(batch, AirHost());
    for (u32 j = 0; j < batch; j++) {
        if (!air_descs[j] || !parse_air_host(air_descs[j], air_desc_lens[j], airs[j]))
            return wf_fail(ctx, WF_ERR_INVALID, "proof %u: malformed AIR description", j);
        if (air_check_host(ctx, airs[j], log_n, blowup) != WF_OK) return wf_fail(ctx, WF_ERR_INVALID, "proof %u: %s", j, std::string(ctx->err).c_str());
        if (const char* why = j ? air_structure_mismatch(airs[0], airs[j]) : nullptr)
            return wf_fail(ctx, WF_ERR_INVALID, "proof %u differs from proof 0 in its %s", j, why);
    }
    return WF_OK;
}
extern "C" int wf_air_batch_check(uint32_t batch, const uint64_t* const* air_descs, const size_t* air_desc_lens, uint32_t log_n,
                                  uint32_t blowup, char* msg, size_t msg_cap) {
    wf_ctx note{};
    std::vector<AirHost> airs;
    const int r = air_batch_parse(&note, batch, air_descs, air_desc_lens, log_n, blowup, airs);
    if (msg && msg_cap) { strncpy(msg, note.err.c_str(), msg_cap - 1); msg[msg_cap - 1] = 0; }
    return r;
}
extern "C" int wf_prove_air_batch(wf_ctx* ctx, uint32_t batch, const uint64_t* const* air_descs, const size_t* air_desc_lens,
                                  const uint64_t* aux_build, size_t aux_build_len, const uint64_t* const* trace_cols, const uint64_t* d_traces,
                                  int mont, uint32_t log_n, const uint32_t* opts, uint8_t* const* proofs, size_t* proof_lens) {
    if (!ctx || !opts || !proofs || !proof_lens) return wf_fail(ctx, WF_ERR_INVALID, "bad arguments");
    if (!trace_cols == !d_traces) return wf_fail(ctx, WF_ERR_INVALID, "pass exactly one of trace_cols (host) and d_traces (device)");
    Options o;
    CKI(parse_options(ctx, opts, o));
    std::vector<AirHost> airs;
    CKI(air_batch_parse(ctx, batch, air_descs, air_desc_lens, log_n, o.blowup, airs));
    for (u32 j = 0; j < batch; j++) if (!proofs[j]) return wf_fail(ctx, WF_ERR_INVALID, "proof %u: no output buffer", j);
    AuxBuildHost b;
    if (aux_build) {
        CKI(parse_aux_build(ctx, airs[0], aux_build, aux_build_len, b));
        for (auto& col : b.cols)
            for (u32 q = o.ext; q < 3; q++) if (col.init[q]) return wf_fail(ctx, WF_ERR_INVALID, "aux column init has non-zero words beyond the extension degree");
    } else if (airs[0].aw) {
        return wf_fail(ctx, WF_ERR_INVALID, "multi-segment AIR: a batch builds its aux segments from aux_build");
    }
    const u32 w = airs[0].w;
    const size_t n = (size_t)1 << log_n;
    std::vector<std::vector<u8>> out(batch);
    for (u32 j = 0; j < batch; j++) {
        const uint64_t* const* cols = trace_cols ? trace_cols + (size_t)j * w : nullptr;
        const uint64_t* dev = d_traces ? d_traces + (size_t)j * w * n : nullptr;
        const int r = prove_bytes(ctx, airs[j], cols, dev, mont, log_n, o, out[j], nullptr, nullptr, nullptr, aux_build ? &b : nullptr);
        if (r != WF_OK) return wf_fail(ctx, r, "proof %u: %s", j, std::string(ctx->err).c_str());
    }
    for (u32 j = 0; j < batch; j++)
        if (out[j].size() > proof_lens[j]) return wf_fail(ctx, WF_ERR_INVALID, "proof %u: proof buffer too small (%zu needed)", j, out[j].size());
    for (u32 j = 0; j < batch; j++) {
        memcpy(proofs[j], out[j].data(), out[j].size());
        proof_lens[j] = out[j].size();
    }
    return WF_OK;
}

extern "C" int wf_trace_validate(wf_ctx* ctx, const uint64_t* air_desc, size_t air_desc_len, const uint64_t* aux_build, size_t aux_build_len,
                                 const uint64_t* const* aux_cols, const uint64_t* const* trace_cols, const uint64_t* d_trace, int mont,
                                 const uint64_t* rand, uint32_t log_n, uint32_t ext, int check_degrees, wf_validation* report,
                                 uint64_t* first_failing_step, uint64_t* expected_degrees, uint64_t* actual_degrees, char* msg, size_t msg_cap) {
    if (msg && msg_cap) msg[0] = 0;
    if (!ctx || !air_desc || !report || log_n < 3 || log_n > 30 || ext < 1 || ext > 3) return wf_fail(ctx, WF_ERR_INVALID, "bad arguments");
    if (!trace_cols == !d_trace) return wf_fail(ctx, WF_ERR_INVALID, "pass exactly one of trace_cols (host) and d_trace (device)");
// ... 344 lines not shown
```

Baseline: 81.72.

## Fuse FRI fold with next-layer Blake3 hashing, skip padded NTT lanes, avoid copies

Adds a fused kernel that folds a FRI layer and hashes the folded rows into leaf digests for the next layer, removing a separate hash pass and a re-read of the folded values. The FRI builder can now take ownership of the input buffer instead of making a device-to-device copy. The zeroing memsets are replaced by in-kernel zero stores of padding columns. A padded NTT pass variant skips loads and butterflies on dead padding lanes in the last segment. Together these touch several subsystems and add complexity in ownership and in padding handling.

After: 80.47 (median of 6 runs). 1.5% less time.

```diff
diff --git a/winterfell_b200/csrc/capi.cu b/winterfell_b200/csrc/capi.cu
--- a/winterfell_b200/csrc/capi.cu
+++ b/winterfell_b200/csrc/capi.cu
@@ -206,6 +206,7 @@
     p.out_W = (u32)out.W;
     p.out_row_mul = 1;
     p.cconst = 1;
+    p.live = (int)(in.cols - (in.nseg() - 1) * (u32)in.W);
 }
 static int split3(wf_ctx* ctx, u32 log_n, u32* lr, u32* lc, u32* lr2, u32* lc2) {
     *lr = (log_n + 2) / 3;
@@ -1073,9 +1074,10 @@
     wf_ctx* ctx;
     wf_fri* f;
     wf_tree* t = nullptr;
+    wf_tree* tn = nullptr;
     DevScratch tmp;
     FriBuild(wf_ctx* c, wf_fri* fr) : ctx(c), f(fr), tmp(c) {}
-    ~FriBuild() { if (t) wf_tree_free(ctx, t); if (f) wf_fri_free(ctx, f); }
+    ~FriBuild() { if (t) wf_tree_free(ctx, t); if (tn) wf_tree_free(ctx, tn); if (f) wf_fri_free(ctx, f); }
 };
 extern "C" {
 int wf_fri_build_layers(wf_ctx* ctx, int hash_id, const wf_mat* evals, int d, uint32_t folding, uint32_t rem_max_deg,
@@ -1113,7 +1115,6 @@
         CKI(wf_get_twiddles(ctx, log2_ceil(len), &master));
         void* nxt;
         CKI(g.tmp.alloc(m * ld * 8, &nxt));
-        if (ld > d) CK(cudaMemsetAsync(nxt, 0, m * ld * 8, ctx->st));
         CK(fri_fold_layer((u64*)cur, len, d, ld, (int)folding, alpha, master, (u64*)nxt, ld, ctx->st));
         ctx->launches++;
         f->layers.push_back(FriLayer{(u64*)g.tmp.keep(cur), len, t});
@@ -1140,8 +1141,8 @@
 }
 
 }
-int wf_fri_build_layers_coin(wf_ctx* ctx, int hash_id, const wf_mat* evals, int d, uint32_t folding, uint32_t rem_max_deg,
-                             uint32_t blowup, PublicCoin& coin, std::vector<Digest>& commitments, wf_fri** out) {
+static int fri_build_layers_coin(wf_ctx* ctx, int hash_id, wf_mat* evals, bool take, int d, uint32_t folding, uint32_t rem_max_deg,
+                                 uint32_t blowup, PublicCoin& coin, std::vector<Digest>& commitments, wf_fri** out) {
     if (!ctx || !evals || !out) return wf_fail(ctx, WF_ERR_INVALID, "bad arguments");
     if (d < 1 || d > 3 || (int)evals->m.cols != d) return wf_fail(ctx, WF_ERR_INVALID, "evaluations must have ext_degree base columns");
     if (folding != 2 && folding != 4 && folding != 8 && folding != 16) return wf_fail(ctx, WF_ERR_UNSUPPORTED, "folding factor %u", folding);
@@ -1157,8 +1158,14 @@
     size_t nlayers = 0;
     for (size_t l = len; l > max_rem; l /= folding) nlayers++;
     void *cur, *dstate, *dalpha, *dlog;
-    CKI(g.tmp.alloc(len * ld * 8, &cur));
-    CK(cudaMemcpyAsync(cur, evals->m.base, len * ld * 8, cudaMemcpyDeviceToDevice, ctx->st));
+    if (take && evals->m.nseg() == 1 && ctx->live.count(evals->m.base)) {
+        cur = evals->m.base;
+        g.tmp.bufs.push_back(cur);
+        evals->m.base = nullptr;
+    } else {
+        CKI(g.tmp.alloc(len * ld * 8, &cur));
+        CK(cudaMemcpyAsync(cur, evals->m.base, len * ld * 8, cudaMemcpyDeviceToDevice, ctx->st));
+    }
     CKI(g.tmp.alloc(8 * 8, &dstate));
     CKI(g.tmp.alloc(8 * 8, &dalpha));
     CKI(g.tmp.alloc(std::max<size_t>(nlayers, 1) * 8 * 8, &dlog));
@@ -1166,24 +1173,34 @@
     memcpy(seed_words, coin.seed.b, 32);
     CK(cudaMemcpyAsync(dstate, seed_words, 32, cudaMemcpyHostToDevice, ctx->st));
     size_t layer = 0;
+    if (len > max_rem) {
+        CKI(tree_alloc(ctx, hash_id, len / folding, &g.t));
+        CK(fri_hash_layer(hash_id, (u64*)cur, len, d, ld, (int)folding, g.t->leaves, ctx->st));
+        ctx->launches++;
+    }
     while (len > max_rem) {
         size_t m = len / folding;
-        wf_tree* t;
-        CKI(tree_alloc(ctx, hash_id, m, &t));
-        g.t = t;
-        CK(fri_hash_layer(hash_id, (u64*)cur, len, d, ld, (int)folding, t->leaves, ctx->st));
+        wf_tree* t = g.t;
         CK(commit_merkle_nodes(hash_id, t->leaves, m, t->nodes, ctx->st));
         CK(fri_coin_step(hash_id, (u64*)dstate, t->nodes + 4, d, (u64*)dalpha, (u64*)dlog + 8 * layer, ctx->st));
-        ctx->launches += 2 + merkle_launches(m);
+        ctx->launches += 1 + merkle_launches(m);
         const u64* master;
         CKI(wf_get_twiddles(ctx, log2_ceil(len), &master));
         void* nxt;
         CKI(g.tmp.alloc(m * ld * 8, &nxt));
-        if (ld > d) CK(cudaMemsetAsync(nxt, 0, m * ld * 8, ctx->st));
-        CK(fri_fold_layer((u64*)cur, len, d, ld, (int)folding, nullptr, master, (u64*)nxt, ld, ctx->st, (const u64*)dalpha));
-        ctx->launches++;
+        if (m > max_rem) {
+            CKI(tree_alloc(ctx, hash_id, m / folding, &g.tn));
+            int nl = 0;
+            CK(fri_fold_hash_layer(hash_id, (u64*)cur, len, d, ld, (int)folding, (const u64*)dalpha, master, (u64*)nxt, ld, g.tn->leaves,
+                                   ctx->st, &nl));
+            ctx->launches += nl;
+        } else {
+            CK(fri_fold_layer((u64*)cur, len, d, ld, (int)folding, nullptr, master, (u64*)nxt, ld, ctx->st, (const u64*)dalpha));
+            ctx->launches++;
+        }
         f->layers.push_back(FriLayer{(u64*)g.tmp.keep(cur), len, t});
-        g.t = nullptr;
+        g.t = g.tn;
+        g.tn = nullptr;
         cur = nxt;
         len = m;
         layer++;
@@ -1217,6 +1234,14 @@
     g.f = nullptr;
     *out = f;
     return WF_OK;
+}
+int wf_fri_build_layers_coin(wf_ctx* ctx, int hash_id, const wf_mat* evals, int d, uint32_t folding, uint32_t rem_max_deg,
+                             uint32_t blowup, PublicCoin& coin, std::vector<Digest>& commitments, wf_fri** out) {
+    return fri_build_layers_coin(ctx, hash_id, const_cast<wf_mat*>(evals), false, d, folding, rem_max_deg, blowup, coin, commitments, out);
+}
+int wf_fri_build_layers_coin_take(wf_ctx* ctx, int hash_id, wf_mat* evals, int d, uint32_t folding, uint32_t rem_max_deg,
+                                  uint32_t blowup, PublicCoin& coin, std::vector<Digest>& commitments, wf_fri** out) {
+    return fri_build_layers_coin(ctx, hash_id, evals, true, d, folding, rem_max_deg, blowup, coin, commitments, out);
 }
 extern "C" {
 
diff --git a/winterfell_b200/csrc/fri.cu b/winterfell_b200/csrc/fri.cu
--- a/winterfell_b200/csrc/fri.cu
+++ b/winterfell_b200/csrc/fri.cu
@@ -61,16 +61,9 @@
 }
 
 template <int D, int LOGNF>
-__global__ void __launch_bounds__(256) fri_fold_kernel(const u64* __restrict__ ev, size_t m, int ld, GlExt<D> alpha,
-                                                       const u64* __restrict__ d_alpha, const u64* __restrict__ master,
-                                                       u32 logL, u64* __restrict__ next, int next_ld, size_t i0) {
+__device__ __forceinline__ GlExt<D> fold_row(const u64* __restrict__ ev, size_t m, int ld, const GlExt<D>& alpha,
+                                             const u64* __restrict__ master, u32 logL, size_t i, size_t i0) {
     constexpr int NF = 1 << LOGNF;
-    size_t i = (size_t)blockIdx.x * blockDim.x + threadIdx.x;
-    if (i >= m) return;
-    if (d_alpha) {
-#pragma unroll
-        for (int c = 0; c < D; c++) alpha.v[c] = d_alpha[c];
-    }
     u64 x[D][NF];
 #pragma unroll
     for (int k = 0; k < NF; k++)
@@ -98,9 +91,65 @@
         acc = ext_add(ext_mul(acc, beta), cj);
     }
     const u64 inv_nf = GL_P - ((GL_P - 1) >> LOGNF);
-    acc = ext_mul_base(acc, inv_nf);
-#pragma unroll
-    for (int c = 0; c < D; c++) next[i * next_ld + c] = acc.v[c];
+    return ext_mul_base(acc, inv_nf);
+}
+
+template <int D>
+__device__ __forceinline__ void store_row(u64* __restrict__ next, int next_ld, size_t i, const GlExt<D>& v) {
+#pragma unroll
+    for (int c = 0; c < D; c++) next[i * next_ld + c] = v.v[c];
+    for (int c = D; c < next_ld; c++) next[i * next_ld + c] = 0;
+}
+
+template <int D, int LOGNF>
+__global__ void __launch_bounds__(256) fri_fold_kernel(const u64* __restrict__ ev, size_t m, int ld, GlExt<D> alpha,
+                                                       const u64* __restrict__ d_alpha, const u64* __restrict__ master,
+                                                       u32 logL, u64* __restrict__ next, int next_ld, size_t i0) {
+    size_t i = (size_t)blockIdx.x * blockDim.x + threadIdx.x;
+    if (i >= m) return;
+    if (d_alpha) {
+#pragma unroll
+        for (int c = 0; c < D; c++) alpha.v[c] = d_alpha[c];
+    }
+    store_row<D>(next, next_ld, i, fold_row<D, LOGNF>(ev, m, ld, alpha, master, logL, i, i0));
+}
+
+template <int D, int LOGNF, int DW>
+__global__ void __launch_bounds__(256) fri_fold_hash_blake3_kernel(const u64* __restrict__ ev, size_t m, int ld,
+                                                                   const u64* __restrict__ d_alpha, const u64* __restrict__ master,
+                                                                   u32 logL, u64* __restrict__ next, int next_ld,
+                                                                   uint4* __restrict__ digests) {
+    constexpr int NF = 1 << LOGNF, NE = NF * D;
+    const size_t mq = m >> LOGNF;
+    const size_t j = (size_t)blockIdx.x * blockDim.x + threadIdx.x;
+    if (j >= mq) return;
+    GlExt<D> alpha;
+#pragma unroll
+    for (int c = 0; c < D; c++) alpha.v[c] = d_alpha[c];
+    u32 cv[8], msg[16];
+    b3_iv(cv);
+#pragma unroll
+    for (int k = 0; k < NF; k++) {
+        const size_t i = j + (size_t)k * mq;
+        const GlExt<D> v = fold_row<D, LOGNF>(ev, m, ld, alpha, master, logL, i, 0);
+        store_row<D>(next, next_ld, i, v);
+#pragma unroll
+        for (int c = 0; c < D; c++) {
+            const int e = k * D + c, slot = e % 8;
+            msg[2 * slot] = (u32)v.v[c];
+            msg[2 * slot + 1] = (u32)(v.v[c] >> 32);
+            if (slot == 7 || e == NE - 1) {
+                const int b = e / 8;
+#pragma unroll
+                for (int z = slot + 1; z < 8; z++) { msg[2 * z] = 0; msg[2 * z + 1] = 0; }
+                const u32 fl = (b == 0 ? B3_CHUNK_START : 0) | (e == NE - 1 ? (B3_CHUNK_END | B3_ROOT) : 0);
+                b3_compress(cv, msg, 0, (u32)(slot + 1) * 8, fl, b3_runtime_one());
+            }
+        }
+    }
+    if (DW == 6) { cv[6] = 0; cv[7] = 0; }
+    digests[2 * j] = make_uint4(cv[0], cv[1], cv[2], cv[3]);
+    digests[2 * j + 1] = make_uint4(cv[4], cv[5], cv[6], cv[7]);
 }
 
 cudaError_t fri_hash_layer(int hash_id, const u64* evals, size_t len, int d, int ld, int nf, u64* digests,
@@ -136,6 +185,46 @@
     return cudaGetLastError();
 }
 
+template <int D, int DW>
+static cudaError_t fold_hash_dispatch(const u64* evals, size_t len, int ld, int nf, const u64* d_alpha, const u64* master,
+                                      u64* next, int next_ld, u64* digests, cudaStream_t st) {
+    const size_t mq = len / nf / nf;
+    const u32 logL = log2_ceil(len);
+    const unsigned blocks = (unsigned)((mq + 255) / 256);
+    uint4* dg = reinterpret_cast<uint4*>(digests);
+    const size_t m = len / nf;
+    switch (nf) {
+        case 2: fri_fold_hash_blake3_kernel<D, 1, DW><<<blocks, 256, 0, st>>>(evals, m, ld, d_alpha, master, logL, next, next_ld, dg); break;
+        case 4: fri_fold_hash_blake3_kernel<D, 2, DW><<<blocks, 256, 0, st>>>(evals, m, ld, d_alpha, master, logL, next, next_ld, dg); break;
+        case 8: fri_fold_hash_blake3_kernel<D, 3, DW><<<blocks, 256, 0, st>>>(evals, m, ld, d_alpha, master, logL, next, next_ld, dg); break;
+        case 16: fri_fold_hash_blake3_kernel<D, 4, DW><<<blocks, 256, 0, st>>>(evals, m, ld, d_alpha, master, logL, next, next_ld, dg); break;
+        default: return cudaErrorInvalidValue;
+    }
+    return cudaGetLastError();
+}
+template <int DW>
+static cudaError_t fold_hash_d(const u64* evals, size_t len, int d, int ld, int nf, const u64* d_alpha, const u64* master,
+                               u64* next, int next_ld, u64* digests, cudaStream_t st) {
+    switch (d) {
+        case 1: return fold_hash_dispatch<1, DW>(evals, len, ld, nf, d_alpha, master, next, next_ld, digests, st);
+        case 2: return fold_hash_dispatch<2, DW>(evals, len, ld, nf, d_alpha, master, next, next_ld, digests, st);
+        case 3: return fold_hash_dispatch<3, DW>(evals, len, ld, nf, d_alpha, master, next, next_ld, digests, st);
+        default: return cudaErrorInvalidValue;
+    }
+}
+cudaError_t fri_fold_hash_layer(int hash_id, const u64* evals, size_t len, int d, int ld, int nf, const u64* d_alpha,
+                                const u64* master, u64* next, int next_ld, u64* digests, cudaStream_t st, int* launches) {
+    if (WF_HASH_IS_BLAKE3(hash_id)) {
+        *launches = 1;
+        return WF_DIGEST_WORDS32(hash_id) == 6 ? fold_hash_d<6>(evals, len, d, ld, nf, d_alpha, master, next, next_ld, digests, st)
+                                               : fold_hash_d<8>(evals, len, d, ld, nf, d_alpha, master, next, next_ld, digests, st);
+    }
+    *launches = 2;
+    cudaError_t e = fri_fold_layer(evals, len, d, ld, nf, nullptr, master, next, next_ld, st, d_alpha);
+    if (e != cudaSuccess) return e;
+    return fri_hash_layer(hash_id, next, len / nf, d, next_ld, nf, digests, st);
+}
+
 cudaError_t fri_fold_layer(const u64* evals, size_t len, int d, int ld, int nf, const u64* alpha, const u64* master,
                            u64* next, int next_ld, cudaStream_t st, const u64* d_alpha, size_t i0, u32 logL_global) {
     switch (d) {
diff --git a/winterfell_b200/csrc/fri.cuh b/winterfell_b200/csrc/fri.cuh
--- a/winterfell_b200/csrc/fri.cuh
+++ b/winterfell_b200/csrc/fri.cuh
@@ -8,4 +8,6 @@
 cudaError_t fri_fold_layer(const u64* evals, size_t len, int d, int ld, int nf, const u64* alpha,
                            const u64* master, u64* next, int next_ld, cudaStream_t st, const u64* d_alpha = nullptr,
                            size_t i0 = 0, u32 logL_global = 0);
+cudaError_t fri_fold_hash_layer(int hash_id, const u64* evals, size_t len, int d, int ld, int nf, const u64* d_alpha,
+                                const u64* master, u64* next, int next_ld, u64* digests, cudaStream_t st, int* launches);
 cudaError_t fri_coin_step(int hash_id, u64* state, const u64* root, int d, u64* alpha_out, u64* log_entry, cudaStream_t st);
diff --git a/winterfell_b200/csrc/internal.hpp b/winterfell_b200/csrc/internal.hpp
--- a/winterfell_b200/csrc/internal.hpp
+++ b/winterfell_b200/csrc/internal.hpp
@@ -145,6 +145,8 @@
 struct wf_fri;
 int wf_fri_build_layers_coin(wf_ctx* ctx, int hash_id, const wf_mat* evals, int d, uint32_t folding, uint32_t rem_max_deg,
                              uint32_t blowup, PublicCoin& coin, std::vector<Digest>& commitments, wf_fri** out);
+int wf_fri_build_layers_coin_take(wf_ctx* ctx, int hash_id, wf_mat* evals, int d, uint32_t folding, uint32_t rem_max_deg,
+                                  uint32_t blowup, PublicCoin& coin, std::vector<Digest>& commitments, wf_fri** out);
 int wf_get_twiddles(wf_ctx* ctx, u32 log_n, const u64** out);
 struct wf_tree;
 int wf_fri_layer_tree(wf_ctx* ctx, int hash_id, const u64* vals, size_t len, int d, int ld, int nf, wf_tree** out);
diff --git a/winterfell_b200/csrc/ntt.cuh b/winterfell_b200/csrc/ntt.cuh
--- a/winterfell_b200/csrc/ntt.cuh
+++ b/winterfell_b200/csrc/ntt.cuh
@@ -41,6 +41,7 @@
     int vec_in, vec_out;
     const u64* ctab;
     u64 cconst;
+    int live;
 };
 
 enum { NTT_STRIDED = 0, NTT_CONTIG = 1 };
diff --git a/winterfell_b200/csrc/ntt2.cu b/winterfell_b200/csrc/ntt2.cu
--- a/winterfell_b200/csrc/ntt2.cu
+++ b/winterfell_b200/csrc/ntt2.cu
@@ -83,9 +83,9 @@
         asm volatile("{\n\t.reg .pred p;\n\tmbarrier.try_wait.parity.shared::cta.b64 p, [%1], 0;\n\tselp.u32 %0, 1, 0, p;\n\t}" : "=r"(done) : "r"(mb) : "memory");
 }
 
-__device__ __forceinline__ void cp_async16(void* smem_dst, const void* gsrc, bool ok) {
+__device__ __forceinline__ void cp_async16(void* smem_dst, const void* gsrc, u32 bytes) {
     const u32 dst = (u32)__cvta_generic_to_shared(smem_dst);
-    asm volatile("cp.async.cg.shared.global [%0], [%1], 16, %2;" ::"r"(dst), "l"(gsrc), "r"(ok ? 16 : 0) : "memory");
+    asm volatile("cp.async.cg.shared.global [%0], [%1], 16, %2;" ::"r"(dst), "l"(gsrc), "r"(bytes) : "memory");
 }
 __device__ __forceinline__ void cp_async8(void* smem_dst, const void* gsrc, bool ok) {
     const u32 dst = (u32)__cvta_generic_to_shared(smem_dst);
@@ -94,18 +94,21 @@
 __device__ __forceinline__ void cp_async_commit() { asm volatile("cp.async.commit_group;" ::: "memory"); }
 __device__ __forceinline__ void cp_async_wait_all() { asm volatile("cp.async.wait_group 0;" ::: "memory"); }
 
-template <int LOGS, int K>
-__device__ __forceinline__ void tile_round(u64* __restrict__ s, const u64* __restrict__ tw, const u64* __restrict__ pre, int tid) {
+__host__ __device__ constexpr u32 div16_magic(u32 n) { return (65536u + n - 1) / n; }
+template <int LOGS, int K, bool PAD>
+__device__ __forceinline__ void tile_round(u64* __restrict__ s, const u64* __restrict__ tw, const u64* __restrict__ pre, int tid, u32 nl) {
     constexpr int LANES = Plan<LOGS>::lanes, LK = LANES == 8 ? 1 : 2;
     constexpr int R = plan_radix<LOGS>(K), ST = plan_stage<LOGS>(K);
     constexpr int LOGSPAN = LOGS - ST - R;
     constexpr u32 SPAN = 1u << LOGSPAN;
     constexpr bool LAST = LOGSPAN == 0;
     constexpr u32 TASKS = (1u << LOGS) * LANES / 16;
+    static_assert(TASKS <= 1024, "task index bound of div16_magic");
     if (R == 4) {
+        const u32 tasks = PAD ? (1u << LOGS) / 16 * nl : TASKS, mag = div16_magic(nl);
 #pragma unroll 1
-        for (u32 task = tid; task < TASKS; task += NTT2_THREADS) {
-            const u32 lane = task % LANES, bf = task / LANES;
+        for (u32 task = tid; task < tasks; task += NTT2_THREADS) {
+            const u32 bf = PAD ? (task * mag) >> 16 : task / LANES, lane = PAD ? task - bf * nl : task % LANES;
             const u32 lo = bf & (SPAN - 1), base = ((bf >> LOGSPAN) << (LOGSPAN + 4)) + lo;
             const u32 bh = base ^ swz_hash<LK>(base);
             u64* pr[1 << LK];
@@ -133,9 +136,10 @@
         }
     } else {
         constexpr int LP = LANES / 2;
+        const u32 np = (nl + 1) / 2, tasks = PAD ? (1u << LOGS) / 8 * np : TASKS, mag = div16_magic(np);
 #pragma unroll 1
-        for (u32 task = tid; task < TASKS; task += NTT2_THREADS) {
-            const u32 lp = task % LP, bf = task / LP;
+        for (u32 task = tid; task < tasks; task += NTT2_THREADS) {
+            const u32 bf = PAD ? (task * mag) >> 16 : task / LP, lp = PAD ? task - bf * np : task % LP;
             const u32 lo = bf & (SPAN - 1), base = ((bf >> LOGSPAN) << (LOGSPAN + 3)) + lo;
             const u32 bh = base ^ swz_hash<LK>(base);
             ulonglong2* pr[1 << LK];
@@ -174,8 +178,8 @@
     }
 }
 
-template <int MODE, int LOGS>
-__global__ void __launch_bounds__(NTT2_THREADS, NTT2_MINB) ntt2_pass_kernel(const NttPassParams p) {
+template <int MODE, int LOGS, bool PAD>
+__device__ __forceinline__ void ntt2_pass(const NttPassParams& p) {
     extern __shared__ __align__(16) u64 smem[];
     constexpr int LANES = Plan<LOGS>::lanes, LK = LANES == 8 ? 1 : 2, LP = LANES / 2;
     constexpr u32 S = 1u << LOGS;
@@ -194,6 +198,8 @@
     const u32 g = ymap ? blockIdx.z : blockIdx.y, b = ymap ? blockIdx.x : blockIdx.z;
     const u32 R = 1u << p.logR, C = 1u << p.logC;
     const u32 ncols = MODE == NTT_STRIDED ? C : R;
+    const u32 lw = (PAD && g + 1 == (ymap ? gridDim.z : gridDim.y)) ? (u32)p.live : (u32)W;
+    const u32 nl = PAD && W >= LANES ? (u32)min(max((int)lw - (int)q0, 0), LANES) : (u32)LANES;
 
     {
         const u64* in = p.in + (size_t)g * p.in_seg_stride + (size_t)b * p.in_batch_stride;
@@ -202,7 +208,7 @@
         const u32 t0 = W >= LANES ? 0 : (l0 >> logW), t1 = W >= LANES ? 0 : ((l0 + 1) >> logW);
         const u32 w0 = W >= LANES ? q0 + l0 : (l0 & (W - 1)), w1 = W >= LANES ? q0 + l0 + 1 : ((l0 + 1) & (W - 1));
         const u32 c0 = tile * T + t0, c1 = tile * T + t1;
-        const bool ok0 = c0 < ncols, ok1 = c1 < ncols;
+        const bool ok0 = c0 < ncols && (!PAD || w0 < lw), ok1 = c1 < ncols && (!PAD || w1 < lw);
         const bool yin = MODE == NTT_CONTIG && ymap;
         const u64 istride = MODE == NTT_STRIDED ? ((u64)W << p.logC) : (yin ? ((u64)p.out_row_mul << p.logR) * p.out_W : (u64)W);
         const u64* a0 = MODE == NTT_STRIDED ? in + (size_t)c0 * W + w0
@@ -220,7 +226,7 @@
         for (u32 i = tid / LP; i < S; i += ROWS_PER_IT) {
             u64* dst = s + prow<LK>(i) * LANES + l0;
             if (vec) {
-                cp_async16(dst, a0 + i * s0, ok0);
+                cp_async16(dst, a0 + i * s0, ok0 ? (!PAD || ok1 ? 16 : 8) : 0);
             } else {
                 cp_async8(dst, a0 + i * s0, ok0);
                 cp_async8(dst + 1, a1 + i * s1, ok1);
@@ -270,16 +276,18 @@
     bulk_wait(mbar);
     __syncthreads();
 
-    tile_round<LOGS, 0>(s, rtw, p.pre_tab ? p.pre_tab + (size_t)b * p.pre_batch_stride : nullptr, tid);
-    __syncthreads();
-    if (Plan<LOGS>::rounds == 3) {
-        tile_round<LOGS, 1>(s, rtw + Plan<LOGS>::tw0_entries, nullptr, tid);
+    if (!PAD || nl) {
+        tile_round<LOGS, 0, PAD>(s, rtw, p.pre_tab ? p.pre_tab + (size_t)b * p.pre_batch_stride : nullptr, tid, nl);
         __syncthreads();
-        tile_round<LOGS, 2>(s, nullptr, nullptr, tid);
-    } else {
-        tile_round<LOGS, 1>(s, nullptr, nullptr, tid);
-    }
-    __syncthreads();
+        if (Plan<LOGS>::rounds == 3) {
+            tile_round<LOGS, 1, PAD>(s, rtw + Plan<LOGS>::tw0_entries, nullptr, tid, nl);
+            __syncthreads();
+            tile_round<LOGS, 2, PAD>(s, nullptr, nullptr, tid, nl);
+        } else {
+            tile_round<LOGS, 1, PAD>(s, nullptr, nullptr, tid, nl);
+        }
+        __syncthreads();
+    }
 
     u64* out = p.out + (size_t)g * p.out_seg_stride + (size_t)b * p.out_batch_stride;
     {
@@ -350,6 +358,11 @@
     }
 }
 
+template <int MODE, int LOGS>
+__global__ void __launch_bounds__(NTT2_THREADS, NTT2_MINB) ntt2_pass_kernel(const NttPassParams p) { ntt2_pass<MODE, LOGS, false>(p); }
+template <int MODE, int LOGS>
+__global__ void __launch_bounds__(NTT2_THREADS, NTT2_MINB) ntt2_pad_pass_kernel(const NttPassParams p) { ntt2_pass<MODE, LOGS, true>(p); }
+
 template <int LOGS>
 __global__ void ntt2_build_tw_kernel(u64* out, u64 w_s) {
     const u32 idx = blockIdx.x * blockDim.x + threadIdx.x;
@@ -376,9 +389,10 @@
     const size_t smem = smem_bytes_t<LOGS>(p);
     const u32 tiles = ((ncols + T - 1) / T) * chunks;
     const dim3 grid = p.y_in_out ? dim3(n_batch, tiles, n_segments) : dim3(tiles, n_segments, n_batch);
-    cudaError_t e = cudaFuncSetAttribute(ntt2_pass_kernel<MODE, LOGS>, cudaFuncAttributeMaxDynamicSharedMemorySize, (int)smem);
+    auto kernel = (p.live && p.live < p.W) ? ntt2_pad_pass_kernel<MODE, LOGS> : ntt2_pass_kernel<MODE, LOGS>;
+    cudaError_t e = cudaFuncSetAttribute(kernel, cudaFuncAttributeMaxDynamicSharedMemorySize, (int)smem);
     if (e != cudaSuccess) return e;
-    ntt2_pass_kernel<MODE, LOGS><<<grid, NTT2_THREADS, smem, st>>>(p);
+    kernel<<<grid, NTT2_THREADS, smem, st>>>(p);
     return cudaGetLastError();
 }
 template <int MODE>
diff --git a/winterfell_b200/csrc/prover.cu b/winterfell_b200/csrc/prover.cu
--- a/winterfell_b200/csrc/prover.cu
+++ b/winterfell_b200/csrc/prover.cu
@@ -1222,7 +1222,7 @@
     wf_mark(ctx, "deep_composition");
     {
         std::vector<Digest> fri_roots;
-        CKI(wf_fri_build_layers_coin(ctx, h, deep, D, o.folding, o.rem_max_deg, o.blowup, ch.coin, fri_roots, &fri));
+        CKI(wf_fri_build_layers_coin_take(ctx, h, deep, D, o.folding, o.rem_max_deg, o.blowup, ch.coin, fri_roots, &fri));
         for (auto& r : fri_roots) ch.commitments.bytes(r.b, WF_DIGEST_BYTES(h));
     }
     scope.drop(deep);
@@ -1874,7 +1874,6 @@
         void* nx;
         CKI(wf_dev_alloc(ctx, sl.m_l * ld * 8, &nx));
         owned.push_back(nx);
-        if (ld > D) CK(cudaMemsetAsync(nx, 0, sl.m_l * ld * 8, ctx->st));
         u64 av[3] = {0, 0, 0};
         for (int q = 0; q < D; q++) av[q] = alpha.v[q];
         CK(fri_fold_layer(sl.vals, (size_t)nf * sl.m_l, D, ld, (int)nf, av, master, (u64*)nx, ld, ctx->st, nullptr, (size_t)r * sl.m_l, logL));
@@ -1887,7 +1886,7 @@
     scope.drop(deep);
     {
         std::vector<Digest> fri_roots;
-        CKI(wf_fri_build_layers_coin(ctx, h, fri_in, D, o.folding, o.rem_max_deg, o.blowup, ch.coin, fri_roots, &fri));
+        CKI(wf_fri_build_layers_coin_take(ctx, h, fri_in, D, o.folding, o.rem_max_deg, o.blowup, ch.coin, fri_roots, &fri));
         for (auto& rt : fri_roots) ch.commitments.bytes(rt.b, WF_DIGEST_BYTES(h));
     }
     scope.drop(fri_in);
```
